# yuhogun0908/MISOnet

Measured on AMD Instinct MI355X. Metric: utterances/sec MISO1->MVDR->MISO3, 6-mic 16kHz 4s, higher is better.
Workload: dtype f32w; 1 GPU; BASELINE configs[3]: synthetic 6-mic 16 kHz 4 s, full MISO1x6 -> align -> MVDRx2 -> MISO3x2; batch_per_gpu=16, global_batch=16, frames=1001, freq_bins=129, parallelism=utterance-shard x1

## Files before the change

include/misonet.h:

```cpp
#ifndef MISONET_H_
#define MISONET_H_

#ifdef __cplusplus
extern "C" {
#endif

typedef struct misonet_net misonet_net;
typedef struct misonet_pipeline misonet_pipeline;
typedef void* misonet_stream;

enum {
  MISONET_OK = 0,
  MISONET_EINVAL = -1,
  MISONET_ESTATE = -2,
  MISONET_EHIP = -3,
  MISONET_ENOMEM = -4,
  MISONET_ENAN = -5
};

typedef struct {
  int in_ch;
  int out_ch;
  int en_ch[7];
  int de_ch[7];
  int n_freq;
  int tcn_norm;
} misonet_cfg;

const char* misonet_strerror(int code);
const char* misonet_last_error(void);
int misonet_version(void);

int misonet_net_create(const misonet_cfg* cfg, misonet_net** out);
int misonet_net_destroy(misonet_net* net);
int misonet_net_num_tensors(const misonet_net* net);
const char* misonet_net_tensor_name(const misonet_net* net, int i);
long long misonet_net_tensor_numel(const misonet_net* net, int i);
int misonet_net_set_tensor(misonet_net* net, const char* key, const float* host_data, long long numel);
int misonet_net_commit(misonet_net* net);

int misonet_net_set_precision(misonet_net* net, int mode);
int misonet_net_get_precision(const misonet_net* net);

long long misonet_net_workspace_bytes(const misonet_net* net, int n_samples, int n_frames);

int misonet_net_forward(misonet_net* net, int n_seg, const void* const* seg_dev, const int* seg_ch,
                        int B, int T, void* out_dev, void* ws_dev, long long ws_bytes, misonet_stream stream);
int misonet_net_check(misonet_net* net, const void* ws_dev, misonet_stream stream);

int misonet_net_keep_activations(misonet_net* net, int keep);
int misonet_net_buffer_plan(const misonet_net* net, int n_frames, int max_buffers, long long* offset_bytes,
                            long long* size_bytes, int* first_step, int* last_step);
int misonet_net_conv_plan(const misonet_net* net, int mode, int max_layers, int* kind);
int misonet_net_tap_shape(const misonet_net* net, const char* name, int* C, int* F);
int misonet_net_tap(misonet_net* net, const char* name, const void* ws_dev, int B, int T, float* dst_dev,
                    misonet_stream stream);

long long misonet_mvdr_workspace_bytes(int B, int F, int M);
int misonet_mvdr(const void* src_dev, const void* mix_dev, int B, int F, int M, int T, float epsi,
                 void* out_dev, void* ws_dev, long long ws_bytes, misonet_stream stream);
int misonet_mvdr_debug(const void* ws_dev, int B, int F, int M, void* steer_c128_dev, void* w_c128_dev,
                       misonet_stream stream);

typedef struct {
  int kind;
  int noise;
  double condition;
  int trace_normalize;
  float epsi;
  int ban;
  int ref_ch;
} misonet_bf_opts;
int misonet_bf_opts_default(misonet_bf_opts* opts);
long long misonet_beamform_workspace_bytes(int B, int F, int M, const misonet_bf_opts* opts);
int misonet_beamform(const void* src_dev, const void* mix_dev, int B, int F, int M, int T, const misonet_bf_opts* opts,
                     void* out_dev, void* ws_dev, long long ws_bytes, misonet_stream stream);
int misonet_beamform_debug(const void* ws_dev, int B, int F, int M, const misonet_bf_opts* opts, void* w_c128_dev,
                           double* lambda_dev, misonet_stream stream);

typedef struct {
  int taps;
  int delay;
  int iterations;
  double diag_load;
  double power_floor;
} misonet_wpe_opts;
int misonet_wpe_opts_default(misonet_wpe_opts* opts);
long long misonet_wpe_workspace_bytes(int B, int M, int T, int F, const misonet_wpe_opts* opts);
int misonet_wpe(const void* mix_dev, const float* power_dev, int B, int M, int T, int F, const misonet_wpe_opts* opts,
                void* out_dev, void* ws_dev, long long ws_bytes, misonet_stream stream);
int misonet_wpe_debug(const void* ws_dev, int B, int M, int F, const misonet_wpe_opts* opts, void* g_c128_dev, int* fail_dev,
                      misonet_stream stream);

typedef struct {
  int taps;
  int delay;
  double diag_load;
  double power_floor;
  int ref_ch;
} misonet_wpd_opts;
int misonet_wpd_opts_default(misonet_wpd_opts* opts);
long long misonet_wpd_workspace_bytes(int B, int F, int M, const misonet_wpd_opts* opts);
int misonet_wpd(const void* src_dev, const void* mix_dev, int B, int F, int M, int T, const misonet_wpd_opts* opts,
                void* out_dev, void* ws_dev, long long ws_bytes, misonet_stream stream);
int misonet_wpd_debug(const void* ws_dev, int B, int F, int M, const misonet_wpd_opts* opts, void* wbar_c128_dev, int* fail_dev,
                      misonet_stream stream);

typedef struct {
  int iterations;
  int prior;
  double diag_load;
  double prior_floor;
} misonet_cacgmm_opts;
int misonet_cacgmm_opts_default(misonet_cacgmm_opts* opts);
long long misonet_cacgmm_workspace_bytes(int B, int K, int F, int M);
int misonet_cacgmm(const void* mix_dev, const float* init_masks_dev, int B, int K, int F, int M, int T,
                   const misonet_cacgmm_opts* opts, float* masks_out_dev, void* images_out_dev, void* ws_dev, long long ws_bytes,
                   misonet_stream stream);
int misonet_cacgmm_debug(const void* ws_dev, int B, int K, int F, int M, void* bk_c128_dev, double* pi_dev, double* ll_dev,
                         int* fail_dev, misonet_stream stream);
int misonet_masks_from_estimates(const void* est_dev, const void* mix_dev, int B, int S, int F, int M, int T,
                                 float* masks_out_dev, misonet_stream stream);

typedef struct {
  int kind;
  int noise;
  int rtf;
  double mu;
  double diag_load;
  int ref_ch;
} misonet_jbf_opts;
int misonet_jbf_opts_default(misonet_jbf_opts* opts);
long long misonet_beamform_joint_workspace_bytes(int B, int S, int F, int M, const misonet_jbf_opts* opts);
int misonet_beamform_joint(const void* src_dev, const void* mix_dev, int B, int S, int F, int M, int T,
                           const misonet_jbf_opts* opts, void* out_dev, void* ws_dev, long long ws_bytes, misonet_stream stream);
int misonet_beamform_joint_debug(const void* ws_dev, int B, int S, int F, int M, const misonet_jbf_opts* opts, void* w_c128_dev,
                                 void* rtf_c128_dev, int* fail_dev, misonet_stream stream);

typedef struct {
  int iterations;
  int model;
  int channels;
  int ref_ch;
  double floor;
} misonet_iva_opts;
int misonet_iva_opts_default(misonet_iva_opts* opts);
long long misonet_auxiva_workspace_bytes(int B, int S, int K, int F, int M, int T);
int misonet_auxiva_resident_frames(int K);
int misonet_auxiva(const void* mix_dev, int B, int S, int F, int M, int T, const misonet_iva_opts* opts, void* images_out_dev,
                   int* order_out_dev, void* ws_dev, long long ws_bytes, misonet_stream stream);
int misonet_auxiva_debug(const void* ws_dev, int B, int K, int F, int M, int T, void* y_c128_dev, void* a_c128_dev,
                         void* evec_c128_dev, double* power_dev, int* fail_dev, misonet_stream stream);

long long misonet_pit_scratch_bytes(int B, int S, int F);
int misonet_pit_select(const void* anchor_dev, const void* cand_dev, int B, int S, int T, int F,
                       int* sel_dev, double* dist_dev, long long dist_bytes, misonet_stream stream);

long long misonet_css_scratch_bytes(int K, int S, int F);
int misonet_css_align(const void* est_dev, int K, int S, int T, int F, int hop_frames, const int* perm0_dev,
                      int* perm_dev, double* dist_dev, long long dist_bytes, misonet_stream stream);
int misonet_css_stitch(const float* y_dev, const int* perm_dev, int K, int S, int W, int hop, int first,
                       long long n_out, short* out_i16_dev, float* out_f32_dev, misonet_stream stream);

long long misonet_score_scratch_bytes(int B, int E, int R, long long n_or_F);
int misonet_score_wave(const void* est_dev, int est_is_i16, long long est_sb, long long est_ss, long long est_st,
                       const float* ref_dev, long long ref_sb, long long ref_ss, long long ref_st, int B, int E, int R,
                       long long n, const int* n_valid_dev, double* stats_dev, void* scratch_dev,
                       long long scratch_bytes, misonet_stream stream);
int misonet_score_spec(const void* est_dev, long long est_sb, long long est_ss, long long est_st, const void* ref_dev,
                       long long ref_sb, long long ref_ss, long long ref_st, int B, int E, int R, int T, int F,
                       double* pair_dev, int* perm_dev, double* upit_dev, void* scratch_dev, long long scratch_bytes,
                       misonet_stream stream);

long long misonet_bss_scratch_bytes(int B, int E, int R, long long n, int Q);
int misonet_bss_corr(const void* est_dev, int est_is_i16, long long est_sb, long long est_ss, long long est_st,
                     const float* ref_dev, long long ref_sb, long long ref_ss, long long ref_st, int B, int E, int R,
                     long long n, const int* n_valid_dev, int Q, double* Rrr_dev, double* Rre_dev, double* Eee_dev,
                     void* scratch_dev, long long scratch_bytes, misonet_stream stream);
int misonet_bss_solve(const double* Rrr_dev, const double* Rre_dev, const double* Eee_dev, int B, int E, int R, int Q,
                      double* T_dev, double* A_dev, int* info_dev, void* scratch_dev, long long scratch_bytes,
                      misonet_stream stream);

long long misonet_stoi_resampled_len(long long n, int fs);
int misonet_stoi_taps(int fs, double* taps_host);
long long misonet_stoi_scratch_bytes(int B, int NS, int R, long long n10);
int misonet_stoi_resample(const void* est_dev, int est_is_i16, long long est_sb, long long est_ss, long long est_st,
                          const float* ref_dev, long long ref_sb, long long ref_ss, long long ref_st, const float* mix_dev,
                          long long mix_sb, long long mix_st, int B, int E, int R, long long n, const int* n_valid_dev, int fs,
                          double* x10_dev, int* len10_dev, misonet_stream stream);
int misonet_stoi_measure(const double* x10_dev, const int* len10_dev, int B, int NS, int R, long long n10, double* out_dev,
                         int* frames_dev, void* scratch_dev, long long scratch_bytes, misonet_stream stream);

int misonet_resample_ratio(int fs_in, int fs_out, int* p, int* q);
long long misonet_resampled_len(long long n, int fs_in, int fs_out);
int misonet_resample_taps(int fs_in, int fs_out, double* out_host, int cap);
int misonet_resample_tile(void);
int misonet_resample(const void* src_dev, int src_kind, long long src_sb, long long src_sc, long long src_st, int B, int M,
                     long long n, const int* n_valid_dev, int fs_in, int fs_out, void* dst_dev, int dst_kind, long long dst_sb,
                     long long dst_sc, long long dst_st, misonet_stream stream);

long long misonet_resample_stream_carry(long long fs_in, long long fs_out);
long long misonet_resample_stream_state_bytes(int B, int M, long long fs_in, long long fs_out);
long long misonet_resample_stream_outputs(long long n_seen, long long n_new, int flush, long long fs_in, long long fs_out);
int misonet_resample_stream_tile(void);
int misonet_resample_stream_reset(void* state_dev, int B, int M, long long fs_in, long long fs_out, misonet_stream stream);
int misonet_resample_stream(const void* src_dev, int src_i16, long long src_sb, long long src_sc, long long src_st, int B, int M,
// ... 147 lines not shown
```

misonet_amd/_lib.py:

```python
from __future__ import annotations

import ctypes as C
import os

_HERE = os.path.dirname(os.path.abspath(__file__))
LIB_PATH = os.environ.get("MISONET_LIB_PATH") or os.path.join(_HERE, "libmisonet_hip.so")

OK, EINVAL, ESTATE, EHIP, ENOMEM, ENAN = 0, -1, -2, -3, -4, -5


class MisonetError(RuntimeError):
    def __init__(self, code, detail):
        super().__init__(f"libmisonet_hip error {code}: {detail}")
        self.code = code


class Cfg(C.Structure):
    _fields_ = [("in_ch", C.c_int), ("out_ch", C.c_int), ("en_ch", C.c_int * 7), ("de_ch", C.c_int * 7),
                ("n_freq", C.c_int), ("tcn_norm", C.c_int)]


class BfOpts(C.Structure):
    _fields_ = [("kind", C.c_int), ("noise", C.c_int), ("condition", C.c_double), ("trace_normalize", C.c_int),
                ("epsi", C.c_float), ("ban", C.c_int), ("ref_ch", C.c_int)]


class WpeOpts(C.Structure):
    _fields_ = [("taps", C.c_int), ("delay", C.c_int), ("iterations", C.c_int), ("diag_load", C.c_double),
                ("power_floor", C.c_double)]


class OwpeOpts(C.Structure):
    _fields_ = [("taps", C.c_int), ("delay", C.c_int), ("context", C.c_int), ("alpha", C.c_double),
                ("power_floor", C.c_double), ("init", C.c_double)]


class OivaOpts(C.Structure):
    _fields_ = [("model", C.c_int), ("ref_ch", C.c_int), ("alpha", C.c_double), ("floor", C.c_double), ("init", C.c_double)]


class ObfOpts(C.Structure):
    _fields_ = [("noise", C.c_int), ("ref_ch", C.c_int), ("alpha", C.c_double), ("mu", C.c_double), ("diag_load", C.c_double),
                ("epsi", C.c_double), ("init", C.c_double)]


class WpdOpts(C.Structure):
    _fields_ = [("taps", C.c_int), ("delay", C.c_int), ("diag_load", C.c_double), ("power_floor", C.c_double),
                ("ref_ch", C.c_int)]


class CacgmmOpts(C.Structure):
    _fields_ = [("iterations", C.c_int), ("prior", C.c_int), ("diag_load", C.c_double), ("prior_floor", C.c_double)]


class JbfOpts(C.Structure):
    _fields_ = [("kind", C.c_int), ("noise", C.c_int), ("rtf", C.c_int), ("mu", C.c_double), ("diag_load", C.c_double),
                ("ref_ch", C.c_int)]


class DoaOpts(C.Structure):
    _fields_ = [("kind", C.c_int), ("num_src", C.c_int), ("block", C.c_int), ("hop", C.c_int), ("f_lo", C.c_int),
                ("f_hi", C.c_int), ("min_sep", C.c_double)]


class IvaOpts(C.Structure):
    _fields_ = [("iterations", C.c_int), ("model", C.c_int), ("channels", C.c_int), ("ref_ch", C.c_int), ("floor", C.c_double)]


SIGNATURES = {
    "misonet_strerror": (C.c_char_p, [C.c_int]),
    "misonet_last_error": (C.c_char_p, []),
    "misonet_version": (C.c_int, []),
    "misonet_net_create": (C.c_int, [C.POINTER(Cfg), C.POINTER(C.c_void_p)]),
    "misonet_net_destroy": (C.c_int, [C.c_void_p]),
    "misonet_net_num_tensors": (C.c_int, [C.c_void_p]),
    "misonet_net_tensor_name": (C.c_char_p, [C.c_void_p, C.c_int]),
    "misonet_net_tensor_numel": (C.c_longlong, [C.c_void_p, C.c_int]),
    "misonet_net_set_tensor": (C.c_int, [C.c_void_p, C.c_char_p, C.c_void_p, C.c_longlong]),
    "misonet_net_commit": (C.c_int, [C.c_void_p]),
    "misonet_net_set_precision": (C.c_int, [C.c_void_p, C.c_int]),
    "misonet_net_get_precision": (C.c_int, [C.c_void_p]),
    "misonet_net_keep_activations": (C.c_int, [C.c_void_p, C.c_int]),
    "misonet_net_buffer_plan": (C.c_int, [C.c_void_p, C.c_int, C.c_int, C.POINTER(C.c_longlong), C.POINTER(C.c_longlong),
                                          C.POINTER(C.c_int), C.POINTER(C.c_int)]),
    "misonet_net_conv_plan": (C.c_int, [C.c_void_p, C.c_int, C.c_int, C.POINTER(C.c_int)]),
    "misonet_net_workspace_bytes": (C.c_longlong, [C.c_void_p, C.c_int, C.c_int]),
    "misonet_net_forward": (C.c_int, [C.c_void_p, C.c_int, C.POINTER(C.c_void_p), C.POINTER(C.c_int), C.c_int, C.c_int,
                                      C.c_void_p, C.c_void_p, C.c_longlong, C.c_void_p]),
    "misonet_net_check": (C.c_int, [C.c_void_p, C.c_void_p, C.c_void_p]),
    "misonet_net_tap_shape": (C.c_int, [C.c_void_p, C.c_char_p, C.POINTER(C.c_int), C.POINTER(C.c_int)]),
    "misonet_net_tap": (C.c_int, [C.c_void_p, C.c_char_p, C.c_void_p, C.c_int, C.c_int, C.c_void_p, C.c_void_p]),
    "misonet_mvdr_workspace_bytes": (C.c_longlong, [C.c_int, C.c_int, C.c_int]),
    "misonet_mvdr": (C.c_int, [C.c_void_p, C.c_void_p, C.c_int, C.c_int, C.c_int, C.c_int, C.c_float, C.c_void_p,
                               C.c_void_p, C.c_longlong, C.c_void_p]),
    "misonet_mvdr_debug": (C.c_int, [C.c_void_p, C.c_int, C.c_int, C.c_int, C.c_void_p, C.c_void_p, C.c_void_p]),
    "misonet_bf_opts_default": (C.c_int, [C.POINTER(BfOpts)]),
    "misonet_beamform_workspace_bytes": (C.c_longlong, [C.c_int, C.c_int, C.c_int, C.POINTER(BfOpts)]),
    "misonet_beamform": (C.c_int, [C.c_void_p, C.c_void_p, C.c_int, C.c_int, C.c_int, C.c_int, C.POINTER(BfOpts), C.c_void_p,
                                   C.c_void_p, C.c_longlong, C.c_void_p]),
    "misonet_beamform_debug": (C.c_int, [C.c_void_p, C.c_int, C.c_int, C.c_int, C.POINTER(BfOpts), C.c_void_p, C.c_void_p,
                                         C.c_void_p]),
    "misonet_pipeline_set_beamformer": (C.c_int, [C.c_void_p, C.POINTER(BfOpts)]),
    "misonet_wpe_opts_default": (C.c_int, [C.POINTER(WpeOpts)]),
    "misonet_wpe_workspace_bytes": (C.c_longlong, [C.c_int, C.c_int, C.c_int, C.c_int, C.POINTER(WpeOpts)]),
    "misonet_wpe": (C.c_int, [C.c_void_p, C.c_void_p, C.c_int, C.c_int, C.c_int, C.c_int, C.POINTER(WpeOpts), C.c_void_p,
                              C.c_void_p, C.c_longlong, C.c_void_p]),
    "misonet_wpe_debug": (C.c_int, [C.c_void_p, C.c_int, C.c_int, C.c_int, C.POINTER(WpeOpts), C.c_void_p, C.c_void_p,
                                    C.c_void_p]),
    "misonet_owpe_opts_default": (C.c_int, [C.POINTER(OwpeOpts)]),
    "misonet_owpe_state_bytes": (C.c_longlong, [C.c_int, C.c_int, C.c_int, C.POINTER(OwpeOpts)]),
    "misonet_owpe_lds_bytes": (C.c_int, [C.c_int, C.POINTER(OwpeOpts)]),
    "misonet_owpe_reset": (C.c_int, [C.c_void_p, C.c_int, C.c_int, C.c_int, C.POINTER(OwpeOpts), C.c_void_p]),
    "misonet_owpe": (C.c_int, [C.c_void_p, C.c_int, C.c_int, C.c_int, C.c_int, C.POINTER(OwpeOpts), C.c_void_p, C.c_void_p,
                               C.c_longlong, C.c_void_p]),
    "misonet_owpe_debug": (C.c_int, [C.c_void_p, C.c_int, C.c_int, C.c_int, C.POINTER(OwpeOpts), C.c_void_p, C.c_void_p,
                                     C.c_void_p, C.c_void_p, C.c_void_p]),
    "misonet_wpd_opts_default": (C.c_int, [C.POINTER(WpdOpts)]),
    "misonet_wpd_workspace_bytes": (C.c_longlong, [C.c_int, C.c_int, C.c_int, C.POINTER(WpdOpts)]),
    "misonet_wpd": (C.c_int, [C.c_void_p, C.c_void_p, C.c_int, C.c_int, C.c_int, C.c_int, C.POINTER(WpdOpts), C.c_void_p,
                              C.c_void_p, C.c_longlong, C.c_void_p]),
    "misonet_wpd_debug": (C.c_int, [C.c_void_p, C.c_int, C.c_int, C.c_int, C.POINTER(WpdOpts), C.c_void_p, C.c_void_p,
                                    C.c_void_p]),
    "misonet_pipeline_set_wpd": (C.c_int, [C.c_void_p, C.POINTER(WpdOpts)]),
    "misonet_cacgmm_opts_default": (C.c_int, [C.POINTER(CacgmmOpts)]),
    "misonet_cacgmm_workspace_bytes": (C.c_longlong, [C.c_int, C.c_int, C.c_int, C.c_int]),
    "misonet_cacgmm": (C.c_int, [C.c_void_p, C.c_void_p, C.c_int, C.c_int, C.c_int, C.c_int, C.c_int, C.POINTER(CacgmmOpts),
                                 C.c_void_p, C.c_void_p, C.c_void_p, C.c_longlong, C.c_void_p]),
    "misonet_cacgmm_debug": (C.c_int, [C.c_void_p, C.c_int, C.c_int, C.c_int, C.c_int, C.c_void_p, C.c_void_p, C.c_void_p,
                                       C.c_void_p, C.c_void_p]),
    "misonet_masks_from_estimates": (C.c_int, [C.c_void_p, C.c_void_p, C.c_int, C.c_int, C.c_int, C.c_int, C.c_int, C.c_void_p,
                                               C.c_void_p]),
    "misonet_pipeline_set_refine": (C.c_int, [C.c_void_p, C.POINTER(CacgmmOpts)]),
    "misonet_jbf_opts_default": (C.c_int, [C.POINTER(JbfOpts)]),
    "misonet_beamform_joint_workspace_bytes": (C.c_longlong, [C.c_int, C.c_int, C.c_int, C.c_int, C.POINTER(JbfOpts)]),
    "misonet_beamform_joint": (C.c_int, [C.c_void_p, C.c_void_p, C.c_int, C.c_int, C.c_int, C.c_int, C.c_int, C.POINTER(JbfOpts),
                                         C.c_void_p, C.c_void_p, C.c_longlong, C.c_void_p]),
    "misonet_beamform_joint_debug": (C.c_int, [C.c_void_p, C.c_int, C.c_int, C.c_int, C.c_int, C.POINTER(JbfOpts), C.c_void_p,
                                               C.c_void_p, C.c_void_p, C.c_void_p]),
    "misonet_pipeline_set_joint": (C.c_int, [C.c_void_p, C.POINTER(JbfOpts)]),
    "misonet_iva_opts_default": (C.c_int, [C.POINTER(IvaOpts)]),
    "misonet_auxiva_workspace_bytes": (C.c_longlong, [C.c_int, C.c_int, C.c_int, C.c_int, C.c_int, C.c_int]),
    "misonet_auxiva_resident_frames": (C.c_int, [C.c_int]),
    "misonet_auxiva": (C.c_int, [C.c_void_p, C.c_int, C.c_int, C.c_int, C.c_int, C.c_int, C.POINTER(IvaOpts), C.c_void_p,
                                 C.c_void_p, C.c_void_p, C.c_longlong, C.c_void_p]),
    "misonet_auxiva_debug": (C.c_int, [C.c_void_p, C.c_int, C.c_int, C.c_int, C.c_int, C.c_int, C.c_void_p, C.c_void_p,
                                       C.c_void_p, C.c_void_p, C.c_void_p, C.c_void_p]),
    "misonet_oiva_opts_default": (C.c_int, [C.POINTER(OivaOpts)]),
    "misonet_oiva_state_bytes": (C.c_longlong, [C.c_int, C.c_int, C.c_int]),
    "misonet_oiva_bins_per_pass": (C.c_int, [C.c_int]),
    "misonet_oiva_reset": (C.c_int, [C.c_void_p, C.c_int, C.c_int, C.c_int, C.POINTER(OivaOpts), C.c_void_p]),
    "misonet_oiva": (C.c_int, [C.c_void_p, C.c_int, C.c_int, C.c_int, C.c_int, C.POINTER(OivaOpts), C.c_void_p, C.c_void_p,
                               C.c_void_p, C.c_longlong, C.c_void_p]),
    "misonet_oiva_debug": (C.c_int, [C.c_void_p, C.c_int, C.c_int, C.c_int, C.c_void_p, C.c_void_p, C.c_void_p, C.c_void_p,
                                     C.c_void_p]),
    "misonet_obf_opts_default": (C.c_int, [C.POINTER(ObfOpts)]),
    "misonet_obf_state_bytes": (C.c_longlong, [C.c_int, C.c_int, C.c_int, C.c_int]),
    "misonet_obf_cells_per_block": (C.c_int, [C.c_int]),
    "misonet_obf_reset": (C.c_int, [C.c_void_p, C.c_int, C.c_int, C.c_int, C.c_int, C.POINTER(ObfOpts), C.c_void_p]),
    "misonet_obf": (C.c_int, [C.c_void_p, C.c_void_p, C.c_int, C.c_int, C.c_int, C.c_int, C.c_int, C.POINTER(ObfOpts), C.c_void_p,
                              C.c_void_p, C.c_longlong, C.c_void_p]),
    "misonet_obf_debug": (C.c_int, [C.c_void_p, C.c_int, C.c_int, C.c_int, C.c_int, C.c_void_p, C.c_void_p, C.c_void_p, C.c_void_p,
                                    C.c_void_p, C.c_void_p]),
    "misonet_pit_scratch_bytes": (C.c_longlong, [C.c_int, C.c_int, C.c_int]),
    "misonet_pit_select": (C.c_int, [C.c_void_p, C.c_void_p, C.c_int, C.c_int, C.c_int, C.c_int, C.c_void_p, C.c_void_p,
                                     C.c_longlong, C.c_void_p]),
    "misonet_css_scratch_bytes": (C.c_longlong, [C.c_int, C.c_int, C.c_int]),
    "misonet_css_align": (C.c_int, [C.c_void_p, C.c_int, C.c_int, C.c_int, C.c_int, C.c_int, C.c_void_p, C.c_void_p,
                                    C.c_void_p, C.c_longlong, C.c_void_p]),
    "misonet_css_stitch": (C.c_int, [C.c_void_p, C.c_void_p, C.c_int, C.c_int, C.c_int, C.c_int, C.c_int, C.c_longlong,
                                     C.c_void_p, C.c_void_p, C.c_void_p]),
    "misonet_score_scratch_bytes": (C.c_longlong, [C.c_int, C.c_int, C.c_int, C.c_longlong]),
    "misonet_score_wave": (C.c_int, [C.c_void_p, C.c_int, C.c_longlong, C.c_longlong, C.c_longlong, C.c_void_p, C.c_longlong,
                                     C.c_longlong, C.c_longlong, C.c_int, C.c_int, C.c_int, C.c_longlong, C.c_void_p,
                                     C.c_void_p, C.c_void_p, C.c_longlong, C.c_void_p]),
    "misonet_score_spec": (C.c_int, [C.c_void_p, C.c_longlong, C.c_longlong, C.c_longlong, C.c_void_p, C.c_longlong,
                                     C.c_longlong, C.c_longlong, C.c_int, C.c_int, C.c_int, C.c_int, C.c_int, C.c_void_p,
                                     C.c_void_p, C.c_void_p, C.c_void_p, C.c_longlong, C.c_void_p]),
    "misonet_bss_scratch_bytes": (C.c_longlong, [C.c_int, C.c_int, C.c_int, C.c_longlong, C.c_int]),
    "misonet_bss_corr": (C.c_int, [C.c_void_p, C.c_int, C.c_longlong, C.c_longlong, C.c_longlong, C.c_void_p, C.c_longlong,
                                   C.c_longlong, C.c_longlong, C.c_int, C.c_int, C.c_int, C.c_longlong, C.c_void_p, C.c_int,
                                   C.c_void_p, C.c_void_p, C.c_void_p, C.c_void_p, C.c_longlong, C.c_void_p]),
    "misonet_bss_solve": (C.c_int, [C.c_void_p, C.c_void_p, C.c_void_p, C.c_int, C.c_int, C.c_int, C.c_int, C.c_void_p,
                                    C.c_void_p, C.c_void_p, C.c_void_p, C.c_longlong, C.c_void_p]),
    "misonet_stoi_resampled_len": (C.c_longlong, [C.c_longlong, C.c_int]),
    "misonet_stoi_taps": (C.c_int, [C.c_int, C.POINTER(C.c_double)]),
    "misonet_stoi_scratch_bytes": (C.c_longlong, [C.c_int, C.c_int, C.c_int, C.c_longlong]),
    "misonet_stoi_resample": (C.c_int, [C.c_void_p, C.c_int, C.c_longlong, C.c_longlong, C.c_longlong, C.c_void_p,
                                        C.c_longlong, C.c_longlong, C.c_longlong, C.c_void_p, C.c_longlong, C.c_longlong,
                                        C.c_int, C.c_int, C.c_int, C.c_longlong, C.c_void_p, C.c_int, C.c_void_p, C.c_void_p,
                                        C.c_void_p]),
    "misonet_stoi_measure": (C.c_int, [C.c_void_p, C.c_void_p, C.c_int, C.c_int, C.c_int, C.c_longlong, C.c_void_p,
                                       C.c_void_p, C.c_void_p, C.c_longlong, C.c_void_p]),
    "misonet_resample_ratio": (C.c_int, [C.c_int, C.c_int, C.POINTER(C.c_int), C.POINTER(C.c_int)]),
    "misonet_resampled_len": (C.c_longlong, [C.c_longlong, C.c_int, C.c_int]),
    "misonet_resample_taps": (C.c_int, [C.c_int, C.c_int, C.POINTER(C.c_double), C.c_int]),
    "misonet_resample_tile": (C.c_int, []),
    "misonet_resample": (C.c_int, [C.c_void_p, C.c_int, C.c_longlong, C.c_longlong, C.c_longlong, C.c_int, C.c_int, C.c_longlong,
                                   C.c_void_p, C.c_int, C.c_int, C.c_void_p, C.c_int, C.c_longlong, C.c_longlong, C.c_longlong,
                                   C.c_void_p]),
    "misonet_resample_stream_carry": (C.c_longlong, [C.c_longlong, C.c_longlong]),
    "misonet_resample_stream_state_bytes": (C.c_longlong, [C.c_int, C.c_int, C.c_longlong, C.c_longlong]),
    "misonet_resample_stream_outputs": (C.c_longlong, [C.c_longlong, C.c_longlong, C.c_int, C.c_longlong, C.c_longlong]),
    "misonet_resample_stream_tile": (C.c_int, []),
    "misonet_resample_stream_reset": (C.c_int, [C.c_void_p, C.c_int, C.c_int, C.c_longlong, C.c_longlong, C.c_void_p]),
    "misonet_resample_stream": (C.c_int, [C.c_void_p, C.c_int, C.c_longlong, C.c_longlong, C.c_longlong, C.c_int, C.c_int,
                                          C.c_longlong, C.c_longlong, C.c_int, C.c_longlong, C.c_longlong, C.c_void_p, C.c_int,
                                          C.c_longlong, C.c_longlong, C.c_longlong, C.c_void_p, C.c_longlong, C.c_void_p]),
    "misonet_room_tile": (C.c_int, []),
    "misonet_room_rir_len": (C.c_longlong, [C.c_int, C.c_int, C.c_int, C.c_int]),
    "misonet_room_mix_len": (C.c_longlong, [C.c_longlong, C.c_int]),
    "misonet_room_rir": (C.c_int, [C.c_void_p, C.c_void_p, C.c_void_p, C.c_void_p, C.c_int, C.c_int, C.c_int, C.c_double,
                                   C.c_double, C.c_int, C.c_int, C.c_void_p, C.c_void_p, C.c_void_p]),
    "misonet_room_mix": (C.c_int, [C.c_void_p, C.c_longlong, C.c_longlong, C.c_longlong, C.c_void_p, C.c_void_p, C.c_int, C.c_int,
                                   C.c_int, C.c_longlong, C.c_int, C.c_longlong, C.c_void_p, C.c_void_p, C.c_void_p, C.c_void_p]),
    "misonet_doa_opts_default": (C.c_int, [C.POINTER(DoaOpts)]),
    "misonet_doa_tile": (C.c_int, []),
    "misonet_doa_bin_chunk": (C.c_int, []),
    "misonet_doa_blocks": (C.c_int, [C.c_int, C.c_int, C.c_int]),
    "misonet_doa_workspace_bytes": (C.c_longlong, [C.c_int, C.c_int, C.c_int, C.c_int, C.c_int, C.c_int, C.POINTER(DoaOpts)]),
    "misonet_doa": (C.c_int, [C.c_void_p, C.c_void_p, C.c_void_p, C.c_int, C.c_void_p, C.c_int, C.c_int, C.c_int, C.c_int,
                              C.c_int, C.c_int, C.c_double, C.POINTER(DoaOpts), C.c_void_p, C.c_void_p, C.c_void_p, C.c_void_p,
                              C.c_void_p, C.c_longlong, C.c_void_p]),
    "misonet_doa_debug": (C.c_int, [C.c_void_p, C.c_int, C.c_int, C.c_int, C.c_int, C.c_int, C.c_int, C.POINTER(DoaOpts),
                                    C.c_void_p, C.c_void_p, C.c_void_p, C.c_void_p]),
    "misonet_reverb_frames": (C.c_longlong, [C.c_longlong, C.c_int]),
    "misonet_reverb_scratch_bytes": (C.c_longlong, [C.c_int, C.c_int, C.c_int, C.c_longlong, C.c_int]),
    "misonet_reverb_measure": (C.c_int, [C.c_void_p, C.c_int, C.c_longlong, C.c_longlong, C.c_longlong, C.c_void_p,
                                         C.c_longlong, C.c_longlong, C.c_longlong, C.c_void_p, C.c_longlong, C.c_longlong,
                                         C.c_int, C.c_int, C.c_int, C.c_longlong, C.c_void_p, C.c_int, C.c_void_p, C.c_void_p,
                                         C.c_void_p, C.c_void_p, C.c_longlong, C.c_void_p]),
    "misonet_srmr_frames": (C.c_longlong, [C.c_longlong, C.c_int]),
    "misonet_srmr_scratch_bytes": (C.c_longlong, [C.c_int, C.c_int, C.c_longlong, C.c_int]),
    "misonet_srmr_chunk": (C.c_int, []),
    "misonet_srmr_measure": (C.c_int, [C.c_void_p, C.c_int, C.c_longlong, C.c_longlong, C.c_longlong, C.c_void_p, C.c_longlong,
                                       C.c_longlong, C.c_int, C.c_int, C.c_longlong, C.c_void_p, C.c_int, C.c_void_p, C.c_void_p,
                                       C.c_void_p, C.c_void_p, C.c_longlong, C.c_void_p]),
    "misonet_pipeline_create": (C.c_int, [C.c_void_p, C.c_void_p, C.c_int, C.c_int, C.c_int, C.c_float,
                                          C.POINTER(C.c_void_p)]),
# ... 62 lines not shown
```

misonet_amd/csrc/conv_select.hpp:

```cpp
#pragma once
#include "kernels.hpp"

#ifdef MISONET_EXPERIMENTS
#define MN_ALT_MODES 1
#else
#define MN_ALT_MODES 0
#endif

namespace mn {

constexpr int CONV_NMODES = 7;
inline bool conv_mode_built(int mode) {
  return mode == 0 || mode == 3 || mode == 5 || (MN_ALT_MODES && mode >= 1 && mode < CONV_NMODES);
}

enum class ConvKind : int {
  DIRECT = 0,
  W1D,
  FEW,
  WINO,
  X6_FIRST,
  X6,
  BF16,
  BF16_DMA,
  WINO6,
};
constexpr int CONV_NKIND = 9;

struct ConvShape {
  int Cin, Cout, Fin, Fout;
  int sf, padf, tr2, act;
  bool transposed;
  int ident_c;
  bool net_input;
  int in_oct, out_oct;
};
inline ConvShape conv_shape(const ConvArgs& a, bool net_input = false) {
  return {a.Cin, a.Cout, a.Fin, a.Fout, a.sf, a.padf, a.tr2, a.act, a.padf == 2, a.ident_c, net_input, a.in_oct, a.out_oct};
}

bool conv_w1d_ok(const ConvShape& s);
bool conv_few_ok(const ConvShape& s);
bool conv_wino_ok(const ConvShape& s);
bool conv_x6_first_ok(const ConvShape& s);
bool conv_wino6_ok(const ConvShape& s);

inline ConvKind conv_select(const ConvShape& s, int mode) {
  const bool planar = mode == 0 || mode == 5 || mode == 6;
  if (s.out_oct == 3 && conv_x6_first_ok(s)) return ConvKind::X6_FIRST;
  if (s.in_oct == 3) return ConvKind::X6;
#if MN_ALT_MODES
  if (s.in_oct) return ConvKind::BF16_DMA;
  if (mode == 1 || mode == 2) return ConvKind::BF16;
  if (mode == 6 && conv_wino6_ok(s)) return ConvKind::WINO6;
#endif
  if (planar && conv_few_ok(s)) return ConvKind::FEW;
  if (mode == 5 && conv_wino_ok(s)) return ConvKind::WINO;
  if (mode == 5 && conv_w1d_ok(s)) return ConvKind::W1D;
  return ConvKind::DIRECT;
}

struct ConvWeights {
  const float* W;
  int Cin, Cout;
  bool transposed;
  int cop, ncg;
};
long long conv_image_floats(ConvKind k, const ConvWeights& c);
void conv_image_pack(ConvKind k, const ConvWeights& c, float* img);
inline long long conv_wino_ww16_at(int Cin, int Cout) { return (long long)((Cout + 31) / 32) * (Cin / 8) * 16 * 8 * 32; }
float conv_f16_wscale(const float* W, long long n);

}
```

misonet_amd/csrc/conv_weights.hip:

```cpp
#include "conv_select.hpp"

#include <math.h>
#include <cmath>
#include <algorithm>
#include <string.h>

namespace mn {

static inline float tap(const ConvWeights& c, int co, int ci, int kt, int kf) {
  return c.transposed ? c.W[(((long long)ci * c.Cout + co) * 3 + (2 - kt)) * 3 + (2 - kf)]
                      : c.W[(((long long)co * c.Cin + ci) * 3 + kt) * 3 + kf];
}
static const double WINO_G[4][3] = {{1, 0, 0}, {0.5, 0.5, 0.5}, {0.5, -0.5, 0.5}, {0, 0, 1}};
static inline double wino_u(const ConvWeights& c, int co, int ci, int xi, int nu) {
  double u = 0.0;
  for (int kt = 0; kt < 3; ++kt)
    for (int kf = 0; kf < 3; ++kf) u += WINO_G[xi][kf] * WINO_G[nu][kt] * (double)tap(c, co, ci, kt, kf);
  return u;
}

static void direct_image(const ConvWeights& c, float* w) {
  const int nchunk = (c.Cin + CK - 1) / CK, COP = c.cop;
  for (int cg = 0; cg < c.ncg; ++cg)
    for (int kc = 0; kc < nchunk; ++kc)
      for (int kt = 0; kt < 3; ++kt)
        for (int kf = 0; kf < 3; ++kf)
          for (int cil = 0; cil < CK; ++cil)
            for (int col = 0; col < COP; ++col) {
              const int ci = kc * CK + cil, co = cg * COP + col;
              w[((((long long)cg * nchunk + kc) * 9 + (kt * 3 + kf)) * CK + cil) * COP + col] =
                  (ci < c.Cin && co < c.Cout) ? tap(c, co, ci, kt, kf) : 0.f;
            }
}

static inline unsigned short f32_to_bf16_rne(float f) {
  unsigned int u;
  memcpy(&u, &f, 4);
  u += 0x7fffu + ((u >> 16) & 1u);
  return (unsigned short)(u >> 16);
}
static inline float bf16_to_f32(unsigned short h) {
  unsigned int u = (unsigned int)h << 16;
  float f;
  memcpy(&f, &u, 4);
  return f;
}

float conv_f16_wscale(const float* W, long long n) {
  float m = 0.f;
  for (long long i = 0; i < n; ++i) m = std::max(m, fabsf(W[i]));
  return (m > 0.f && std::isfinite(m)) ? exp2f(floorf(log2f(64.f / m))) : 1.f;
}

static void bf16_image(const ConvWeights& c, float* dst, bool pieces) {
  const int nchunk = (c.Cin + 15) / 16;
  const int COP = 32;
  const int ncg16 = (c.Cout + 31) / 32;
  unsigned short* w = reinterpret_cast<unsigned short*>(dst);
  const long long img = 9LL * 2 * COP * 8;
  for (int cg = 0; cg < ncg16; ++cg)
    for (int kc = 0; kc < nchunk; ++kc)
      for (int kt = 0; kt < 3; ++kt)
        for (int kf = 0; kf < 3; ++kf)
          for (int h = 0; h < 2; ++h)
            for (int col = 0; col < COP; ++col)
              for (int e = 0; e < 8; ++e) {
                const int ci = kc * 16 + 8 * h + e, co = cg * COP + col;
                const float v = (ci < c.Cin && co < c.Cout) ? tap(c, co, ci, kt, kf) : 0.f;
                const long long idx = ((((long long)(kt * 3 + kf)) * 2 + h) * COP + col) * 8 + e;
                if (pieces) {
                  const unsigned short hi = f32_to_bf16_rne(v);
                  const long long base = ((long long)cg * nchunk + kc) * 2 * img;
                  w[base + idx] = hi;
                  w[base + img + idx] = f32_to_bf16_rne(v - bf16_to_f32(hi));
                } else {
                  dst[((long long)cg * nchunk + kc) * img + idx] = v;
                }
              }
}

static void wf6_image(const ConvWeights& c, float* wf) {
  const int nchunk = (c.Cin + 7) / 8;
  const int ncg = (c.Cout + 31) / 32;
  for (int cg = 0; cg < ncg; ++cg)
    for (int kc = 0; kc < nchunk; ++kc)
      for (int kt = 0; kt < 3; ++kt)
        for (int kf = 0; kf < 3; ++kf)
          for (int col = 0; col < 32; ++col)
            for (int e = 0; e < 8; ++e) {
              const int ci = kc * 8 + e, co = cg * 32 + col;
              wf[((((long long)cg * nchunk + kc) * 9 + (kt * 3 + kf)) * 32 + col) * 8 + e] =
                  (ci < c.Cin && co < c.Cout) ? tap(c, co, ci, kt, kf) : 0.f;
            }
}

static void w6s_image(const ConvWeights& c, float* dst) {
  const int nchunk = (c.Cin + 7) / 8;
  unsigned short* img = reinterpret_cast<unsigned short*>(dst);
  for (int kc = 0; kc < nchunk; ++kc)
    for (int kt = 0; kt < 3; ++kt)
      for (int kf = 0; kf < 3; ++kf)
        for (int co = 0; co < 32; ++co)
          for (int e = 0; e < 8; ++e) {
            const int ci = kc * 8 + e;
            const float v = (ci < c.Cin && co < c.Cout) ? tap(c, co, ci, kt, kf) : 0.f;
            const unsigned short h = f32_to_bf16_rne(v);
            const float r1 = v - bf16_to_f32(h);
            const unsigned short m = f32_to_bf16_rne(r1);
            const unsigned short l = f32_to_bf16_rne(r1 - bf16_to_f32(m));
            const unsigned short part[3] = {h, m, l};
            for (int p = 0; p < 3; ++p) {
              const long long unit = kt < 2 ? ((kf * 3 + p) * 2 + kt) * 32 + co : 576 + (kf * 3 + p) * 32 + co;
              img[((long long)kc * 864 + unit) * 8 + e] = part[p];
            }
          }
}

static void few_image(const ConvWeights& c, float* img) {
  for (int ci = 0; ci < c.Cin; ++ci)
    for (int kt = 0; kt < 3; ++kt)
      for (int kf = 0; kf < 3; ++kf)
        for (int co = 0; co < 4; ++co) img[((long long)ci * 9 + (kt * 3 + kf)) * 4 + co] = co < c.Cout ? tap(c, co, ci, kt, kf) : 0.f;
}

static void w1d_image(const ConvWeights& c, float* img) {
  const int nchunk = (c.Cin + CK - 1) / CK, ncg = (c.Cout + 31) / 32;
  for (int cg = 0; cg < ncg; ++cg)
    for (int kc = 0; kc < nchunk; ++kc)
      for (int nu = 0; nu < 4; ++nu)
        for (int kf = 0; kf < 3; ++kf)
          for (int cil = 0; cil < CK; ++cil)
            for (int col = 0; col < 32; ++col) {
              const int ci = kc * CK + cil, co = cg * 32 + col;
              double u = 0.0;
              if (ci < c.Cin && co < c.Cout)
                for (int kt = 0; kt < 3; ++kt) u += WINO_G[nu][kt] * (double)tap(c, co, ci, kt, kf);
              img[((((long long)cg * nchunk + kc) * 12 + (nu * 3 + kf)) * CK + cil) * 32 + col] = (float)u;
            }
}

static inline bool wino_minus(int xi, int nu) { return (nu == 2) != ((nu == 3) != (xi == 3)); }
static void wino_image(const ConvWeights& c, float* img) {
  const int nchunk = c.Cin / 8, ncg = (c.Cout + 31) / 32;
  for (int cg = 0; cg < ncg; ++cg)
    for (int kc = 0; kc < nchunk; ++kc)
      for (int cil = 0; cil < 8; ++cil)
        for (int col = 0; col < 32; ++col) {
          const int ci = kc * 8 + cil, co = cg * 32 + col;
          for (int pos = 0; pos < 16; ++pos) {
            const int xi = pos >> 2, nu = pos & 3;
            const double u = co < c.Cout ? wino_u(c, co, ci, xi, nu) : 0.0;
            img[(((((long long)cg * nchunk + kc) * 4 + (pos >> 2)) * 8 + cil) * 32 + col) * 4 + (pos & 3)] = (float)(wino_minus(xi, nu) ? -u : u);
          }
        }
}
static void wino_image16(const ConvWeights& c, int co0, float* img) {
  const int nchunk = c.Cin / 8;
  for (int kc = 0; kc < nchunk; ++kc)
    for (int cil = 0; cil < 8; ++cil)
      for (int col = 0; col < 16; ++col) {
        const int ci = kc * 8 + cil, co = co0 + col;
        for (int pos = 0; pos < 16; ++pos) {
          const int xi = pos >> 2, nu = pos & 3;
          const double u = wino_u(c, co, ci, xi, nu);
          const int s = cil >> 2, kk = cil & 3;
          img[((((((long long)kc * 2 + s) * 4 + (pos >> 2)) * 4 + kk) * 16 + col) * 4) + (pos & 3)] = (float)(wino_minus(xi, nu) ? -u : u);
        }
      }
}

static void wino6_image(const ConvWeights& c, float* dst) {
  const int nk = (c.Cin + 15) / 16, ncg = (c.Cout + 31) / 32;
  unsigned short* img = reinterpret_cast<unsigned short*>(dst);
  auto top16 = [](float x) { unsigned u; memcpy(&u, &x, 4); return (unsigned short)(u >> 16); };
  for (int cg = 0; cg < ncg; ++cg)
    for (int kk = 0; kk < nk; ++kk)
      for (int pos = 0; pos < 16; ++pos)
        for (int col = 0; col < 32; ++col)
          for (int cil = 0; cil < 16; ++cil) {
            const int ci = kk * 16 + cil, co = cg * 32 + col, xi = pos >> 2, nu = pos & 3;
            const float v = (float)((co < c.Cout && ci < c.Cin) ? wino_u(c, co, ci, xi, nu) : 0.0);
            unsigned vb; memcpy(&vb, &v, 4);
            unsigned hb = vb & 0xffff0000u, wb = vb & 0xffffff00u;
            float h, w; memcpy(&h, &hb, 4); memcpy(&w, &wb, 4);
            const float m = w - h, l = v - w;
            const int lane = col + 32 * (cil >> 3), j = cil & 7;
            const long long q = (((long long)cg * nk + kk) * 4 + xi) * (3 * 4 * 64 * 8);
            img[q + ((long long)(nu * 3 + 0) * 64 + lane) * 8 + j] = top16(h);
            img[q + ((long long)(nu * 3 + 1) * 64 + lane) * 8 + j] = top16(m);
            img[q + ((long long)(nu * 3 + 2) * 64 + lane) * 8 + j] = top16(l);
          }
}

long long conv_image_floats(ConvKind k, const ConvWeights& c) {
  const long long g32 = (c.Cout + 31) / 32, k8 = (c.Cin + 7) / 8, k16 = (c.Cin + 15) / 16;
  switch (k) {
    case ConvKind::DIRECT: return (long long)c.ncg * ((c.Cin + CK - 1) / CK) * 9 * CK * c.cop;
    case ConvKind::W1D: return g32 * ((c.Cin + CK - 1) / CK) * 12 * CK * 32;
    case ConvKind::FEW: return (long long)c.Cin * 36;
    case ConvKind::WINO: return conv_wino_ww16_at(c.Cin, c.Cout) + ((c.Cout & 31) == 16 ? (long long)(c.Cin / 8) * 2048 : 0);
    case ConvKind::X6_FIRST: return k8 * 864 * 4;
    case ConvKind::X6: return g32 * k8 * 9 * 32 * 8;
    case ConvKind::BF16: return g32 * k16 * 2 * 9 * 2 * 32 * 8 / 2;
    case ConvKind::BF16_DMA: return g32 * k16 * 9 * 2 * 32 * 8;
    case ConvKind::WINO6: return g32 * k16 * (16 * 3 * 64 * 16 / 4);
  }
  return 0;
}

void conv_image_pack(ConvKind k, const ConvWeights& c, float* img) {
  switch (k) {
    case ConvKind::DIRECT: direct_image(c, img); break;
    case ConvKind::W1D: w1d_image(c, img); break;
    case ConvKind::FEW: few_image(c, img); break;
    case ConvKind::WINO:
      wino_image(c, img);
      if ((c.Cout & 31) == 16) wino_image16(c, c.Cout - 16, img + conv_wino_ww16_at(c.Cin, c.Cout));
      break;
    case ConvKind::X6_FIRST: w6s_image(c, img); break;
    case ConvKind::X6: wf6_image(c, img); break;
#if MN_ALT_MODES
    case ConvKind::BF16: bf16_image(c, img, true); break;
    case ConvKind::BF16_DMA: bf16_image(c, img, false); break;
    case ConvKind::WINO6: wino6_image(c, img); break;
#else
    default: break;
#endif
  }
}

}
```

misonet_amd/csrc/conv_wino.hip:

```cpp
#include "conv_select.hpp"
#include "conv_epilogue.hpp"
#include "wino_regs.hpp"
#include <stdio.h>
#include <stdlib.h>
#include <utility>

namespace mn {

typedef float wf16 __attribute__((ext_vector_type(16)));
typedef float wf4 __attribute__((ext_vector_type(4)));
typedef float wf2 __attribute__((ext_vector_type(2)));
typedef unsigned int wu2 __attribute__((ext_vector_type(2)));
#define MN_WLDS(p) ((__attribute__((address_space(3))) void*)(p))

constexpr int WCK = 8;
constexpr int WTT = 64;
constexpr int WFT = 8;
constexpr int WNR = 10;
constexpr int WTW = 66;
constexpr int WIN_FLOATS = WCK * WNR * WTW;
constexpr int WW_FLOATS = 16 * WCK * 32;
constexpr int WSTAGE_FLOATS = WIN_FLOATS + WW_FLOATS;
constexpr int WNSTAGE = 3;
constexpr int WNRM_MAX = 192;
constexpr int WCO_MAX = 64;

template <int P, bool Z = false>
__device__ __forceinline__ void wino_mfma(float uu, float vv) {
  if (Z) asm volatile("v_mfma_f32_32x32x2_f32 a[%0:%1], %2, %3, 0" ::"n"(16 * P), "n"(16 * P + 15), "v"(uu), "v"(vv) : W_ACLOB);
  else asm volatile("v_mfma_f32_32x32x2_f32 a[%0:%1], %2, %3, a[%0:%1]" ::"n"(16 * P), "n"(16 * P + 15), "v"(uu), "v"(vv) : W_ACLOB);
}
template <int B, bool Z = false>
__device__ __forceinline__ void wino_mfma16(float uu, float vv) {
  if (Z) asm volatile("v_mfma_f32_16x16x4_f32 a[%0:%1], %2, %3, 0" ::"n"(4 * B), "n"(4 * B + 3), "v"(uu), "v"(vv) : W_ACLOB);
  else asm volatile("v_mfma_f32_16x16x4_f32 a[%0:%1], %2, %3, a[%0:%1]" ::"n"(4 * B), "n"(4 * B + 3), "v"(uu), "v"(vv) : W_ACLOB);
}
__device__ __forceinline__ wf2 pk_add(wf2 a, wf2 b) { wf2 d; asm volatile("v_pk_add_f32 %0, %1, %2" : "=v"(d) : "v"(a), "v"(b)); return d; }
__device__ __forceinline__ wf2 pk_sub(wf2 a, wf2 b) { wf2 d; asm volatile("v_pk_add_f32 %0, %1, %2 neg_lo:[0,1] neg_hi:[0,1]" : "=v"(d) : "v"(a), "v"(b)); return d; }
__device__ __forceinline__ wf2 pk_t01(wf2 a, wf2 b) { wf2 d; asm volatile("v_pk_add_f32 %0, %1, %2 op_sel:[0,0] op_sel_hi:[1,0] neg_lo:[0,1] neg_hi:[0,0]" : "=v"(d) : "v"(a), "v"(b)); return d; }
__device__ __forceinline__ wf2 pk_t23(wf2 a, wf2 b) { wf2 d; asm volatile("v_pk_add_f32 %0, %1, %2 op_sel:[1,0] op_sel_hi:[1,1] neg_lo:[0,1] neg_hi:[0,1]" : "=v"(d) : "v"(a), "v"(b)); return d; }
__device__ __forceinline__ wf2 pk_spm(wf2 a) { wf2 d; asm volatile("v_pk_add_f32 %0, %1, %1 op_sel:[0,1] op_sel_hi:[0,1] neg_lo:[0,0] neg_hi:[0,1]" : "=v"(d) : "v"(a)); return d; }
__device__ __forceinline__ wf2 pk_add_nh(wf2 a, wf2 b) { wf2 d; asm volatile("v_pk_add_f32 %0, %1, %2 neg_lo:[0,0] neg_hi:[0,1]" : "=v"(d) : "v"(a), "v"(b)); return d; }
__device__ __forceinline__ wf2 pk_mul(wf2 a, wf2 b) { wf2 d; asm volatile("v_pk_mul_f32 %0, %1, %2" : "=v"(d) : "v"(a), "v"(b)); return d; }
__device__ __forceinline__ wf2 pk_fma(wf2 a, wf2 b, wf2 c) { wf2 d; asm volatile("v_pk_fma_f32 %0, %1, %2, %3" : "=v"(d) : "v"(a), "v"(b), "v"(c)); return d; }
__device__ __forceinline__ float exp2_ws(float x) {
  float r;
  asm volatile("v_exp_f32 %0, %1\n\ts_nop 0" : "=v"(r) : "v"(x));
  return r;
}
__device__ __forceinline__ float elu_pick(float y, float neg, float pos) {
  return __builtin_bit_cast(int, y) < 0 ? neg : pos;
}
template <int OFF>
__device__ __forceinline__ void lds_write_f32(unsigned addr, float v) {
  asm volatile("ds_write_b32 %0, %1 offset:%2" ::"v"(addr), "v"(v), "n"(OFF) : "memory");
}
__device__ __forceinline__ wf2 pk_nrm(wf2 x, wf2 nr) { wf2 d; asm volatile("v_pk_fma_f32 %0, %1, %2, %2 op_sel:[0,0,1] op_sel_hi:[1,0,1]" : "=v"(d) : "v"(x), "v"(nr)); return d; }
constexpr int WRAW_FLOATS = WCK * WNR * WTT + 256;
constexpr unsigned WRAW_B = (unsigned)(WNSTAGE * WSTAGE_FLOATS) * 4u;
constexpr unsigned WNRM_B = WRAW_B + 2u * WRAW_FLOATS * 4u;
constexpr unsigned WZERO_B = WNRM_B + 2u * WNRM_MAX * 8u;
constexpr unsigned WRED_B = WZERO_B + WNRM_MAX * 8u;
constexpr unsigned WDUMMY_B = WRED_B + 4u * 64u * 4u;
constexpr unsigned WBIAS_B = WDUMMY_B + 64u * 4u;
constexpr size_t WINO_LDS = WBIAS_B + WCO_MAX * 24;
static_assert(WINO_LDS <= 160 * 1024, "one workgroup per CU: at most 160 KB of LDS");

template <int DBG, bool G16 = false>
__global__ __launch_bounds__(256, 1) void conv3x3_wino_f32(const ConvArgs a) {
  extern __shared__ __align__(16) float smem[];
  char* const smem_c = reinterpret_cast<char*>(smem);
  wf2* s_nrm = reinterpret_cast<wf2*>(smem_c + WNRM_B);
  wf2* s_zero = reinterpret_cast<wf2*>(smem_c + WZERO_B);

  const int tid = threadIdx.x;
  const int lane = tid & 63;
  const int wave = __builtin_amdgcn_readfirstlane(tid >> 6);
  const int half = lane >> 5, l31 = lane & 31;
  const int kk = lane >> 4, nn = lane & 15;
  const int T = a.T, Tp = a.Tp, F = a.Fin, Cin = a.Cin;
  const int nchunk = Cin / WCK;
  constexpr unsigned WIMG_B = G16 ? 2u * 4u * 4u * 16u * 16u : (unsigned)(WW_FLOATS * 4);

  const unsigned tps = (unsigned)(a.ntx * a.nty * a.ncg);
  unsigned q0, qstep, Q, xcd_id = 0;
  if (a.xcd) {
    xcd_id = blockIdx.x & 7u;
    q0 = blockIdx.x >> 3;
    qstep = gridDim.x >> 3;
    Q = (unsigned)(a.nsamp >> 3) * tps;
  } else {
    q0 = blockIdx.x;
    qstep = gridDim.x;
    Q = (unsigned)a.nsamp * tps;
  }
  if (q0 >= Q) return;
  const unsigned ntile = (Q - q0 + qstep - 1) / qstep;
  for (int i = tid; i < WNRM_MAX; i += 256) s_zero[i] = wf2{0.f, 0.f};
  if (tid < WCO_MAX) {
    const float b = tid < a.ncg * 32 ? a.bias[tid] : 0.f;
    const float c = elu_fast(b);
    wf2* tb = reinterpret_cast<wf2*>(smem_c + WBIAS_B + tid * 24);
    tb[0] = wf2{b, b}; tb[1] = wf2{-c, -c}; tb[2] = wf2{-1.f - c, -1.f - c};
  }

  const unsigned row_e = (unsigned)Tp;
  const unsigned plane_b = (unsigned)F * row_e * 4u;

  const int sq = tid & 15, scr = tid >> 4;
  int sch[5];
#pragma unroll
  for (int i = 0; i < 5; ++i) sch[i] = (scr + 16 * i) / WNR;
  const bool hrole = tid < 2 * WCK * WNR;
  const int hit = hrole ? tid >> 1 : 0, hside = tid & 1;
  const int hch = hit / WNR, hrow = hit - hch * WNR;
  const unsigned lds0 = (unsigned)(unsigned long long)MN_WLDS(smem);
  constexpr unsigned STAGE_B = (unsigned)WSTAGE_FLOATS * 4u, STEP_B = (unsigned)((G16 ? 4 : 2) * WNR * WTW) * 4u;
  const unsigned dbase = G16 ? lds0 + (unsigned)((kk * WNR + 2 * wave) * WTW + 2 * nn) * 4u
                             : lds0 + (unsigned)((half * WNR + 2 * wave) * WTW + 2 * l31) * 4u;
  unsigned d1 = launder(dbase + STEP_B), d2 = launder(dbase + 2 * STEP_B), d3 = launder(dbase + 3 * STEP_B);
  unsigned d0n = launder(dbase + STAGE_B);
  unsigned uc = launder(lds0 + (unsigned)WIN_FLOATS * 4u + (unsigned)(G16 ? kk * 16 + nn : half * 32 + l31) * 16u);
  unsigned un = launder(uc + STAGE_B);
  unsigned cn = launder(lds0 + STAGE_B + (unsigned)(scr * WTW + 1 + 4 * sq) * 4u);
  unsigned hn = launder(lds0 + (hrole ? STAGE_B + (unsigned)(hit * WTW + (hside ? WTT + 1 : 0)) * 4u : WDUMMY_B + (unsigned)(tid & 63) * 4u));
#define W_LP(TYPE, ADDR) (reinterpret_cast<__attribute__((address_space(3))) TYPE*>(ADDR))
  const unsigned rofs0 = lds0 + WRAW_B + (unsigned)(scr * WTT + 4 * sq) * 4u;
  const unsigned rhofs0 = lds0 + WRAW_B + (unsigned)(WCK * WNR * WTT + tid) * 4u;
  const unsigned rdma0 = WRAW_B + (unsigned)wave * 1024u;
  const unsigned rhdma0 = WRAW_B + (unsigned)(WCK * WNR * WTT) * 4u + (unsigned)wave * 256u;
  const unsigned wdma0 = (unsigned)(WIN_FLOATS * 4) + (unsigned)wave * 1024u;
  const __amdgpu_buffer_rsrc_t rs_w = make_rsrc_e(reinterpret_cast<unsigned long long>(a.ww),
                                                   (unsigned)(a.ncg * nchunk) * WIMG_B);
  unsigned wvo[4];
#pragma unroll
  for (int j = 0; j < 4; ++j) wvo[j] = (unsigned)(tid + 256 * (G16 ? (j & 1) : j)) * 16u;

  unsigned ql = q0;
  int kl = 0;
  int Ln = -1, Lpar = 1, Lcg = 0;
  int lslot = 0;
  unsigned Lgoff[5], Lhoff = 0;
  unsigned Lnr[6];
  bool Lfull = false;
  unsigned Lmask = 0;
  __amdgpu_buffer_rsrc_t rs_l;
  unsigned Cnr[6];
  bool Cfull = false;
  unsigned Cmask = 0;
  unsigned Dwso = 0;
  int cslot = 0;
#pragma unroll
  for (int i = 0; i < 6; ++i) { Lnr[i] = lds0 + WZERO_B; Cnr[i] = lds0 + WZERO_B; }

#define W_DECODE(Q, TT_, FT_, N_, CG_)                                                                \
  {                                                                                                   \
    const unsigned q_ = __builtin_amdgcn_readfirstlane(Q);                                            \
    const unsigned j_ = q_ / tps;                                                                     \
    unsigned r_ = q_ - j_ * tps;                                                                      \
    N_ = (int)(a.xcd ? j_ * 8u + xcd_id : j_);                                                        \
    CG_ = (int)(r_ % (unsigned)a.ncg);                                                                \
    r_ /= (unsigned)a.ncg;                                                                            \
    TT_ = (int)(r_ % (unsigned)a.ntx);                                                                \
    FT_ = (int)(r_ / (unsigned)a.ntx);                                                                \
  }

#define W_LOAD_SETUP(Q)                                                                               \
  {                                                                                                   \
    int tt_, ft_, n_, cg_;                                                                            \
    W_DECODE(Q, tt_, ft_, n_, cg_)                                                                    \
    const int t0_ = tt_ * WTT, fin0_ = ft_ * WFT - 1;                                                 \
    if (n_ != Ln) {                             \
      Ln = n_;                                                                                        \
      Lpar ^= 1;                                                                                      \
      for (int c = tid; c < Cin; c += 256) {                                                          \
        float mean = 0.f, rstd = 1.f;                                                                 \
        if (c >= a.ident_c) {                                                                         \
          const dstat_t* st_ = a.in_stats + ((long long)n_ * a.in_sstride + a.in_c0 + c) * (2 * DS_NL); \
          const double cnt = (double)F * (double)T;                                                   \
          const double m = dstat_read(st_) / cnt;                                                     \
          double var = dstat_read(st_ + DS_NL) / cnt - m * m;                                         \
          var = var > 0.0 ? var : 0.0;                                                                \
          mean = (float)m;                                                                            \
          rstd = (float)(1.0 / sqrt(var + (double)IN_EPS));                                           \
        }                                                                                             \
        s_nrm[Lpar * WNRM_MAX + c] = wf2{rstd, -mean * rstd};                                         \
      }                                                                                               \
      const float* in_n_ = a.in + (long long)n_ * a.in_bstride + (long long)a.in_c0 * F * Tp;         \
      rs_l = make_rsrc_e(reinterpret_cast<unsigned long long>(in_n_), (unsigned)Cin * plane_b);       \
    }                                                                                                 \
    Lcg = cg_;                                                                                        \
    const int tg_ = t0_ + 4 * sq;                                                                     \
    const int tge_ = tg_ + 4 <= Tp ? tg_ : Tp - 4;                                                    \
    Lfull = t0_ + WTT <= T;                                                                           \
    Lmask = (tg_ < T ? 1u : 0u) | (tg_ + 1 < T ? 2u : 0u) | (tg_ + 2 < T ? 4u : 0u) | (tg_ + 3 < T ? 8u : 0u); \
    _Pragma("unroll") for (int i = 0; i < 5; ++i) {                                                   \
      int fin = fin0_ + (scr + 16 * i) - sch[i] * WNR;                                                \
      Lnr[i] = lds0 + ((fin >= 0 && fin < F) ? WNRM_B + (unsigned)(Lpar * WNRM_MAX + sch[i]) * 8u : WZERO_B); \
      fin = fin < 0 ? 0 : (fin >= F ? F - 1 : fin);                                                   \
      Lgoff[i] = (unsigned)sch[i] * plane_b + (unsigned)((fin * (int)row_e + tge_) * 4);              \
    }                                                                                                 \
    {                                                                                                 \
      const int htg_ = hside ? t0_ + WTT : t0_ - 1;                                                   \
      int fin = fin0_ + hrow;                                                                         \
      const bool hok_ = hrole && fin >= 0 && fin < F && htg_ >= 0 && htg_ < T;                        \
      Lnr[5] = lds0 + (hok_ ? WNRM_B + (unsigned)(Lpar * WNRM_MAX + hch) * 8u : WZERO_B);             \
      fin = fin < 0 ? 0 : (fin >= F ? F - 1 : fin);                                                   \
      const int th_ = (htg_ < 0 || htg_ >= T) ? 0 : htg_;    \
      Lhoff = (unsigned)hch * plane_b + (unsigned)((fin * (int)row_e + th_) * 4);                     \
    }                                                                                                 \
  }

#define W_LATCH                                                                                       \
  {                                                                                                   \
    Dwso = (unsigned)(Lcg * nchunk + kl) * WIMG_B;                                                    \
  }
#define W_ADVANCE                                                                                     \
  {                                                                                                   \
    lslot ^= 1;                                                                                       \
    if (++kl == nchunk) {                                                                             \
      if (ql + qstep < Q) { kl = 0; ql += qstep; W_LOAD_SETUP(ql) }                                             \
      else kl = nchunk - 1;                     \
    }                                                                                                 \
  }

  wf4 rwa, rwb;
  float rh = 0.f;
  wf2 nra, nrb;
  wf2 cva[2], cvb[2];
  float chv = 0.f;
  unsigned rofs = rofs0, rhofs = rhofs0;

#define W_CB ((unsigned)kl * (unsigned)WCK * plane_b)
#define W_ISSUE_I(I)                                                                                  \
  __builtin_amdgcn_raw_ptr_buffer_load_lds(rs_l, MN_WLDS(smem_c + rdma0 + lslot * (WRAW_FLOATS * 4) + (I) * 4096), 16, Lgoff[I], W_CB, 0, 0);
#define W_ISSUE_H                                                                                     \
  __builtin_amdgcn_raw_ptr_buffer_load_lds(rs_l, MN_WLDS(smem_c + rhdma0 + lslot * (WRAW_FLOATS * 4)), 4, Lhoff, W_CB, 0, 0);
#define W_ISSUE_W(J, ST, WSO)                                                                         \
  __builtin_amdgcn_raw_ptr_buffer_load_lds(rs_w, MN_WLDS(smem_c + (ST) * (WSTAGE_FLOATS * 4) + wdma0 + (G16 ? ((J) & 1) : (J)) * 4096), 16, wvo[J], WSO, 0, 0);
#define W_WSO_L ((unsigned)(Lcg * nchunk + kl) * WIMG_B)
#define W_VMCNT(N) asm volatile("s_waitcnt vmcnt(" #N ")" ::: "memory");
#define W_NR(DST, I) DST = *W_LP(const wf2, Cnr[I]);
#define W_RR(DST, I) DST = *W_LP(const wf4, rofs + (I) * 4096);
#define W_RRH rh = *W_LP(const float, rhofs);
#define W_CC(CV, RW, NR)                                                                              \
  {                                                                                                   \
    CV[0] = pk_nrm(wf2{RW.x, RW.y}, NR);                                                              \
    CV[1] = pk_nrm(wf2{RW.z, RW.w}, NR);                                                              \
    if (RAG) {                                                                                        \
      CV[0].x = (Cmask & 1u) ? CV[0].x : 0.f; CV[0].y = (Cmask & 2u) ? CV[0].y : 0.f;                 \
      CV[1].x = (Cmask & 4u) ? CV[1].x : 0.f; CV[1].y = (Cmask & 8u) ? CV[1].y : 0.f;                 \
    }                                                                                                 \
  }
#define W_CCH(NR) chv = fmaf(rh, NR.x, NR.y);
#define W_DSW(ADDR, VAL, OFF) asm volatile("ds_write_b32 %0, %1 offset:%2" ::"v"(ADDR), "v"(VAL), "n"(OFF) : "memory");
#define W_CW(CV, I)                                                                                   \
  {                                                                                                   \
    W_DSW(cn, CV[0].x, (I) * (16 * WTW * 4))                                                          \
    W_DSW(cn, CV[0].y, (I) * (16 * WTW * 4) + 4)                                                      \
    W_DSW(cn, CV[1].x, (I) * (16 * WTW * 4) + 8)                                                      \
    W_DSW(cn, CV[1].y, (I) * (16 * WTW * 4) + 12)                                                     \
  }
#define W_CWH W_DSW(hn, chv, 0)
#define W_BARRIER { asm volatile("s_waitcnt lgkmcnt(0)" ::: "memory"); __builtin_amdgcn_s_barrier(); asm volatile("" ::: "memory"); }

  wf2 dd16[2][4][2];
  wf2 vp16[2][4][2];
  wf2 dd[4][2];
  wf4 u[4];
  wf2 vp[4][2];
#define W_FD(I0, DREG)                                                                                \
  {                                                                                                   \
    const unsigned si_ = DREG;                                                                        \
    dd[I0][0] = *W_LP(const wf2, si_ + (I0) * (WTW * 4));                                             \
    dd[I0][1] = *W_LP(const wf2, si_ + (I0) * (WTW * 4) + 8);                                         \
    dd[I0 + 1][0] = *W_LP(const wf2, si_ + ((I0) + 1) * (WTW * 4));                                   \
    dd[I0 + 1][1] = *W_LP(const wf2, si_ + ((I0) + 1) * (WTW * 4) + 8);                               \
  }
#define W_FU(Q, UREG, S) u[Q] = *W_LP(const wf4, UREG + ((S) * 64 + (Q) * 256) * 16);
#define W_TRANSFORM                                                                                   \
  if (!(DBG & 4)) {                                                                                   \
    const wf2 c0a = pk_sub(dd[0][0], dd[2][0]), c0b = pk_sub(dd[0][1], dd[2][1]);                     \
    const wf2 c1a = pk_add(dd[1][0], dd[2][0]), c1b = pk_add(dd[1][1], dd[2][1]);                     \
    const wf2 c2a = pk_sub(dd[2][0], dd[1][0]), c2b = pk_sub(dd[2][1], dd[1][1]);                     \
    const wf2 c3a = pk_sub(dd[1][0], dd[3][0]), c3b = pk_sub(dd[1][1], dd[3][1]);                     \
    vp[0][0] = pk_t01(c0a, c0b); vp[0][1] = pk_t23(c0a, c0b);                                         \
    vp[1][0] = pk_t01(c1a, c1b); vp[1][1] = pk_t23(c1a, c1b);                                         \
    vp[2][0] = pk_t01(c2a, c2b); vp[2][1] = pk_t23(c2a, c2b);                                         \
    vp[3][0] = pk_t01(c3a, c3b); vp[3][1] = pk_t23(c3a, c3b);                                         \
  }

#define W_SB __builtin_amdgcn_sched_barrier(0);
#ifdef MISONET_EXPERIMENTS
  unsigned long long* const tl_buf = (blockIdx.x == 8 && wave == 1) ? a.dbg_buf : nullptr;
  int tl_n = 0;
#define W_STAMP(ID) if (tl_buf && tl_n < 250) { if (lane == 0) { tl_buf[2 * tl_n] = (ID); tl_buf[2 * tl_n + 1] = __builtin_readcyclecounter(); } ++tl_n; }
#else
#define W_STAMP(ID)
#endif
#define W_MF(P, CS) wino_mfma<P, (POST == 2 && (CS) == 0)>(u[(P) >> 2][(P) & 3], vp[(P) >> 2][((P) & 3) >> 1][(P) & 1]);
#define W_NONE
#define W_X(...) if (!(DBG & (1 | 32))) { __VA_ARGS__ }
#define W_XL(...) if (!(DBG & (1 | 16))) { __VA_ARGS__ }
#define W_XW(...) if (!(DBG & (1 | 8))) { __VA_ARGS__ }
#define W_STEP(CS, FD_, FU_, FS, X1, X2, X3, XB, X4, X5, X6, X7, X8, X9, X10, X11, X13, X14, XG)      \
  W_MF(0, CS) W_FU(3, uc, CS) W_SB                                                                    \
  W_MF(1, CS) X1 W_SB                                                                                 \
  W_MF(2, CS) X2 W_SB                                                                                 \
  W_MF(3, CS) X3 W_SB                                                                                 \
  XB                                                                                                  \
  W_MF(4, CS) W_FU(0, FU_, FS) X4 W_SB                                                                \
  W_MF(5, CS) W_FD(0, FD_) X5 W_SB                                                                    \
  W_MF(6, CS) W_FD(2, FD_) X6 W_SB                                                                    \
  W_MF(7, CS) X7 W_SB                                                                                 \
  W_MF(8, CS) W_FU(1, FU_, FS) X8 W_SB                                                                \
  W_MF(9, CS) X9 W_SB                                                                                 \
  W_MF(10, CS) X10 W_SB                                                                               \
  W_MF(11, CS) X11 W_SB                                                                               \
  W_MF(12, CS) W_FU(2, FU_, FS) W_SB                                                                  \
  W_MF(13, CS) X13 W_SB                                                                               \
  W_MF(14, CS) X14 W_SB                                                                               \
  W_MF(15, CS) W_SB                                                                                   \
  W_TRANSFORM XG W_SB

  constexpr int W_NDMA_W = 4, W_NDMA_I = 6, W_NSTORE = 16;
  static_assert(W_NDMA_W * 256 * 16 == WW_FLOATS * 4, "U image = 4 pieces of 256 threads x 16 bytes");
  static_assert(5 * 256 * 16 == WCK * WNR * WTT * 4 && 2 * WCK * WNR <= 256, "raw input = 5 pieces of 256 x 16 bytes + one 4-byte halo piece");
  static_assert(W_NDMA_W + W_NDMA_I == 10 && W_NDMA_I == 6 && 10 + W_NSTORE == 26 && 6 + W_NSTORE == 22,
                "the s_waitcnt vmcnt immediates of W_CHUNK_ (10 / 26 in step 0, 6 / 22 in front of the barrier)");
#define W_BK_S1  \
  const bool nxt0_ = (kc + 2 == nchunk);                                                              \
  Cfull = nxt0_ ? Lfull : Cfull;                                                                      \
  Dwso = (unsigned)(Lcg * nchunk + kl) * WIMG_B;
#define W_BK_S2  \
  lslot ^= 1; ++kl;
#define W_BK_S3                                                \
  const unsigned dl_n_ = (ph3 == 1) ? 0u - 2u * STAGE_B : STAGE_B;       \
  ph3 = ph3 == 2 ? 0 : ph3 + 1;                                                                       \
  post = post > 0 ? post - 1 : 0;                                                                     \
  cslot ^= 1;                                                                                         \
  stnn = ph3 == 0 ? 2 : ph3 - 1;                            \
  const unsigned rsl_ = cslot ? (unsigned)(WRAW_FLOATS * 4) : 0u;
#define W_BK_V                                                                                        \
  if (__builtin_expect(nxt0_, 0)) {                                                                   \
    _Pragma("unroll") for (int i = 0; i < 6; ++i) Cnr[i] = Lnr[i];                                    \
    Cmask = Lmask;                                                                                    \
  } else {                                                                                            \
    _Pragma("unroll") for (int i = 0; i < 6; ++i) Cnr[i] += (unsigned)(WCK * 8);                      \
  }                                                                                                   \
  d1 = d0n + STEP_B; d2 = d0n + 2 * STEP_B; d3 = d0n + 3 * STEP_B;                                    \
  uc = un;                                                                                            \
  d0n += dl_n_; un += dl_n_; cn += dl_n_;                                                             \
  hn += hrole ? dl_n_ : 0u;                                                                           \
  rofs = rofs0 + rsl_; rhofs = rhofs0 + rsl_;
#define W_CHUNK_                                                                                      \
  W_STEP(0, d1, uc, 1, W_NONE, W_NONE, W_NONE, W_NONE, W_NONE, W_NONE, W_NONE,                        \
         W_X(W_STAMP(1) if (POST) { W_VMCNT(26) } else { W_VMCNT(10) } W_STAMP(2) W_RR(rwa, 0)), W_NONE, W_X(W_RR(rwb, 1)), W_X(W_NR(nra, 0)), W_X(W_NR(nrb, 1)), W_NONE, W_NONE, \
         W_X(W_CC(cva, rwa, nra) W_CC(cvb, rwb, nrb)))                                                \
  W_STEP(1, d2, uc, 2, W_X(W_CW(cva, 0)), W_X(W_CW(cvb, 1)), W_NONE, W_NONE, W_NONE, W_NONE, W_NONE,  \
         W_X(W_RR(rwa, 2)), W_NONE, W_X(W_RR(rwb, 3)), W_X(W_NR(nra, 2)), W_X(W_NR(nrb, 3)), W_NONE, W_NONE,  \
         W_X(W_CC(cva, rwa, nra) W_CC(cvb, rwb, nrb)))                                                \
  W_STEP(2, d3, uc, 3, W_X(W_CW(cva, 2)), W_X(W_CW(cvb, 3)), W_NONE, W_NONE, W_NONE, W_NONE, W_NONE,  \
         W_X(W_RR(rwa, 4)), W_NONE, W_X(W_RRH), W_X(W_NR(nra, 4)), W_X(W_NR(nrb, 5)), W_NONE, W_NONE, \
         W_X(W_CC(cva, rwa, nra) W_CCH(nrb)))                                                         \
  W_STEP(3, d0n, un, 0, W_X(W_CW(cva, 4)), W_X(W_CWH), W_NONE,                                        \
         W_STAMP(3) W_XW(if (POST == 2) { W_VMCNT(22) } else { W_VMCNT(6) }) W_STAMP(4) W_BARRIER W_STAMP(5), \
         W_XW(W_ISSUE_W(0, stnn, Dwso)), W_XW(W_ISSUE_W(1, stnn, Dwso)), W_XW(W_ISSUE_W(2, stnn, Dwso)), W_XW(W_ISSUE_W(3, stnn, Dwso)), \
         W_XL(W_ISSUE_I(0)), W_XL(W_ISSUE_I(1)), W_XL(W_ISSUE_I(2)), W_XL(W_ISSUE_I(3)), W_XL(W_ISSUE_I(4)),  \
         W_XL(W_ISSUE_H) W_BK_S1 W_BK_S2 W_BK_S3, W_BK_V)

#define W_FD16(G, I0, DREG)                                                                           \
  {                                                                                                   \
    const unsigned si_ = (DREG) + (G) * 128u;                                                         \
    dd16[G][I0][0] = *W_LP(const wf2, si_ + (I0) * (WTW * 4));                                        \
    dd16[G][I0][1] = *W_LP(const wf2, si_ + (I0) * (WTW * 4) + 8);                                    \
    dd16[G][I0 + 1][0] = *W_LP(const wf2, si_ + ((I0) + 1) * (WTW * 4));                              \
    dd16[G][I0 + 1][1] = *W_LP(const wf2, si_ + ((I0) + 1) * (WTW * 4) + 8);                          \
  }
#define W_FU16(Q, UREG, S) u[Q] = *W_LP(const wf4, UREG + ((S) * 4 + (Q)) * 1024);
#define W_TRANSFORM16(G)                                                                              \
  {                                                                                                   \
    const wf2 c0a = pk_sub(dd16[G][0][0], dd16[G][2][0]), c0b = pk_sub(dd16[G][0][1], dd16[G][2][1]); \
    const wf2 c1a = pk_add(dd16[G][1][0], dd16[G][2][0]), c1b = pk_add(dd16[G][1][1], dd16[G][2][1]); \
    const wf2 c2a = pk_sub(dd16[G][2][0], dd16[G][1][0]), c2b = pk_sub(dd16[G][2][1], dd16[G][1][1]); \
    const wf2 c3a = pk_sub(dd16[G][1][0], dd16[G][3][0]), c3b = pk_sub(dd16[G][1][1], dd16[G][3][1]); \
    vp16[G][0][0] = pk_t01(c0a, c0b); vp16[G][0][1] = pk_t23(c0a, c0b);                               \
    vp16[G][1][0] = pk_t01(c1a, c1b); vp16[G][1][1] = pk_t23(c1a, c1b);                               \
    vp16[G][2][0] = pk_t01(c2a, c2b); vp16[G][2][1] = pk_t23(c2a, c2b);                               \
    vp16[G][3][0] = pk_t01(c3a, c3b); vp16[G][3][1] = pk_t23(c3a, c3b);                               \
  }
#define W_MF16(I, CS) wino_mfma16<(I), (POST == 2 && (CS) == 0)>(u[(I) >> 3][((I) >> 1) & 3], vp16[(I) & 1][(I) >> 3][(((I) >> 1) & 3) >> 1][((I) >> 1) & 1]);
#define W_S16(I, CS, ...) W_MF16(I, CS) __VA_ARGS__ W_SB
#define W_CHUNK16_                                                                                    \
    \
  W_S16(0, 0, W_FU16(3, uc, 0))                                                                       \
  W_S16(1, 0, W_X(if (POST) { W_VMCNT(26) } else { W_VMCNT(10) } W_RR(rwa, 0)))                       \
  W_S16(2, 0, W_X(W_RR(rwb, 1)))                                                                      \
  W_S16(3, 0, W_X(W_NR(nra, 0)))                                                                      \
  W_S16(4, 0, W_X(W_NR(nrb, 1)))                                                                      \
  W_S16(5, 0) W_S16(6, 0)                                                                             \
  W_S16(7, 0, W_X(W_CC(cva, rwa, nra) W_CC(cvb, rwb, nrb)))                                           \
  W_S16(8, 0, W_FU16(0, uc, 1) W_X(W_CW(cva, 0)))                                                     \
  W_S16(9, 0, W_X(W_CW(cvb, 1)))                                                                      \
  W_S16(10, 0, W_FD16(0, 0, d1) W_X(W_RR(rwa, 2)))                                                    \
  W_S16(11, 0, W_FD16(0, 2, d1) W_X(W_RR(rwb, 3)))                                                    \
  W_S16(12, 0, W_FD16(1, 0, d1) W_X(W_NR(nra, 2)))                                                    \
  W_S16(13, 0, W_FD16(1, 2, d1) W_X(W_NR(nrb, 3)))                                                    \
  W_S16(14, 0) W_S16(15, 0)                                                                           \
  W_S16(16, 0, W_FU16(1, uc, 1))                                                                      \
  W_S16(17, 0) W_S16(18, 0)                                                                           \
  W_S16(19, 0, W_X(W_CC(cva, rwa, nra) W_CC(cvb, rwb, nrb)))                                          \
  W_S16(20, 0, W_X(W_CW(cva, 2)))                                                                     \
  W_S16(21, 0, W_X(W_CW(cvb, 3)))                                                                     \
  W_S16(22, 0, W_X(W_RR(rwa, 4)))                                                                     \
  W_S16(23, 0, W_X(W_RRH))                                                                            \
  W_S16(24, 0, W_FU16(2, uc, 1) W_X(W_NR(nra, 4)))                                                    \
  W_S16(25, 0, W_X(W_NR(nrb, 5)))                                                                     \
  W_S16(26, 0) W_S16(27, 0) W_S16(28, 0) W_S16(29, 0) W_S16(30, 0) W_S16(31, 0)                       \
  W_TRANSFORM16(0) W_TRANSFORM16(1) W_X(W_CC(cva, rwa, nra) W_CCH(nrb)) W_SB                          \
   \
  W_S16(0, 1, W_FU16(3, uc, 1) W_X(W_CW(cva, 4)))                                                     \
  W_S16(1, 1, W_X(W_CWH))                                                                             \
  W_S16(2, 1) W_S16(3, 1)                                                                             \
  W_XW(if (POST == 2) { W_VMCNT(22) } else { W_VMCNT(6) }) W_BARRIER                                  \
  W_S16(4, 1, W_XW(W_ISSUE_W(0, stnn, Dwso)))                                                         \
  W_S16(5, 1, W_XW(W_ISSUE_W(1, stnn, Dwso)))                                                         \
  W_S16(6, 1, W_XW(W_ISSUE_W(2, stnn, Dwso)))                                                         \
  W_S16(7, 1, W_XW(W_ISSUE_W(3, stnn, Dwso)))                                                         \
  W_S16(8, 1, W_FU16(0, un, 0) W_XL(W_ISSUE_I(0)))                                                    \
  W_S16(9, 1, W_XL(W_ISSUE_I(1)))                                                                     \
  W_S16(10, 1, W_FD16(0, 0, d0n) W_XL(W_ISSUE_I(2)))                                                  \
  W_S16(11, 1, W_FD16(0, 2, d0n) W_XL(W_ISSUE_I(3)))                                                  \
  W_S16(12, 1, W_FD16(1, 0, d0n) W_XL(W_ISSUE_I(4)))                                                  \
  W_S16(13, 1, W_FD16(1, 2, d0n) W_XL(W_ISSUE_H))                                                     \
  W_S16(14, 1) W_S16(15, 1)                                                                           \
  W_S16(16, 1, W_FU16(1, un, 0))                                                                      \
  W_S16(17, 1) W_S16(18, 1) W_S16(19, 1) W_S16(20, 1) W_S16(21, 1) W_S16(22, 1) W_S16(23, 1)          \
  W_S16(24, 1, W_FU16(2, un, 0))                                                                      \
  W_S16(25, 1) W_S16(26, 1) W_S16(27, 1) W_S16(28, 1) W_S16(29, 1)                                    \
  W_S16(30, 1, W_BK_S1 W_BK_S2 W_BK_S3)                                                               \
  W_S16(31, 1)                                                                                        \
  W_TRANSFORM16(0) W_TRANSFORM16(1) W_BK_V W_SB
#define W_BODY_ if constexpr (G16) { W_CHUNK16_ } else { W_CHUNK_ }

  constexpr bool RAG = true;
  W_LOAD_SETUP(ql)
#pragma unroll
  for (int i = 0; i < 6; ++i) Cnr[i] = Lnr[i];
  Cmask = Lmask; Cfull = Lfull;
  __syncthreads();
  W_ISSUE_W(0, 0, W_WSO_L) W_ISSUE_W(1, 0, W_WSO_L) W_ISSUE_W(2, 0, W_WSO_L) W_ISSUE_W(3, 0, W_WSO_L)
  W_ISSUE_I(0) W_ISSUE_I(1) W_ISSUE_I(2) W_ISSUE_I(3) W_ISSUE_I(4) W_ISSUE_H
  W_LATCH
  W_ADVANCE
  W_ISSUE_W(0, 1, W_WSO_L) W_ISSUE_W(1, 1, W_WSO_L) W_ISSUE_W(2, 1, W_WSO_L) W_ISSUE_W(3, 1, W_WSO_L)
  W_ISSUE_I(0) W_ISSUE_I(1) W_ISSUE_I(2) W_ISSUE_I(3) W_ISSUE_I(4) W_ISSUE_H
  W_LATCH
  W_ADVANCE
  W_VMCNT(0)
  cn -= STAGE_B;
  if (hrole) hn -= STAGE_B;
  W_RR(rwa, 0) W_NR(nra, 0) W_CC(cva, rwa, nra) W_CW(cva, 0)
  W_RR(rwa, 1) W_NR(nra, 1) W_CC(cva, rwa, nra) W_CW(cva, 1)
  W_RR(rwa, 2) W_NR(nra, 2) W_CC(cva, rwa, nra) W_CW(cva, 2)
  W_RR(rwa, 3) W_NR(nra, 3) W_CC(cva, rwa, nra) W_CW(cva, 3)
  W_RR(rwa, 4) W_NR(nra, 4) W_CC(cva, rwa, nra) W_CW(cva, 4)
  W_RRH W_NR(nrb, 5) W_CCH(nrb) W_CWH
#pragma unroll
  for (int i = 0; i < 6; ++i) Cnr[i] += (unsigned)(WCK * 8);
  cn += STAGE_B;
  if (hrole) hn += STAGE_B;
  asm volatile("s_waitcnt lgkmcnt(0)" ::: "memory");
  W_ISSUE_I(0) W_ISSUE_I(1) W_ISSUE_I(2) W_ISSUE_I(3) W_ISSUE_I(4) W_ISSUE_H
  W_LATCH
  W_ADVANCE
  cslot = 1;
  rofs = rofs0 + WRAW_FLOATS * 4;
  rhofs = rhofs0 + WRAW_FLOATS * 4;
  W_BARRIER
  if constexpr (G16) {
    W_FD16(0, 0, dbase) W_FD16(0, 2, dbase) W_FD16(1, 0, dbase) W_FD16(1, 2, dbase) W_FU16(0, uc, 0) W_FU16(1, uc, 0) W_FU16(2, uc, 0)
    W_TRANSFORM16(0) W_TRANSFORM16(1)
  } else {
    W_FD(0, dbase) W_FD(2, dbase) W_FU(0, uc, 0) W_FU(1, uc, 0) W_FU(2, uc, 0)
    W_TRANSFORM
  }
  wfor<256>([&](auto i) __attribute__((always_inline)) { agpr_zero<decltype(i)::value>(); });
  asm volatile("s_nop 4");

  unsigned qc = q0;
  int kc = 0;
  int ph3 = 0;
  int post = 0;
  const unsigned G = ntile * (unsigned)nchunk;
  int stnn = 2;
  for (unsigned g = 0; g < G; ++g) {
    if (Cfull) {
      constexpr bool RAG = false;
      if (post == 0) { constexpr int POST = 0; W_BODY_ } else if (post == 1) { constexpr int POST = 1; W_BODY_ } else { constexpr int POST = 2; W_BODY_ }
    } else {
      constexpr bool RAG = true;
      if (post == 0) { constexpr int POST = 0; W_BODY_ } else if (post == 1) { constexpr int POST = 1; W_BODY_ } else { constexpr int POST = 2; W_BODY_ }
    }
    if (++kc == nchunk) {
      asm volatile("s_nop 15\n\ts_nop 7");
      W_STAMP(10)
      if (!(DBG & 2)) {
      int tt_, ft_, n, cg;
      W_DECODE(qc, tt_, ft_, n, cg)
      const int t0 = tt_ * WTT, f0 = ft_ * WFT;
      const int cbase = cg * 32;
      const int fa = f0 + 2 * wave;
      const bool r0ok = fa < F, r1ok = fa + 1 < F;
      const unsigned P4 = (unsigned)F * (unsigned)Tp * 4u;
      const float* ob_ = a.out + (long long)n * a.out_bstride + (long long)a.out_c0 * F * Tp;
      const __amdgpu_buffer_rsrc_t rs_out = make_rsrc_e(reinterpret_cast<unsigned long long>(ob_), (unsigned)a.Cout * P4);
      const unsigned red_a = lds0 + WRED_B;
      wf2 l2e = {1.44269504088896341f, 1.44269504088896341f};
      asm volatile("" : "+v"(l2e));
      auto epi_item = [&](auto getm, unsigned tabp, unsigned voff, bool evl, const wf2& mt, const wf2& mb, float& o1, float& o2) __attribute__((always_inline)) {
        const wf2 bb = *W_LP(const wf2, tabp);
        wf2 E[4];
        wfor<4>([&](auto xc) __attribute__((always_inline)) {
          constexpr int x = decltype(xc)::value;
          const float m0 = getm(xc, std::integral_constant<int, 0>{}), m1 = getm(xc, std::integral_constant<int, 1>{});
          const float m2 = getm(xc, std::integral_constant<int, 2>{}), m3 = getm(xc, std::integral_constant<int, 3>{});
          E[x] = wf2{m1 + m2, m1 - m2} + wf2{m0, m3};
        });
        wf2 yt = (E[0] + E[1]) + (E[2] + bb);
        wf2 yb = (E[1] - E[2]) + (bb + E[3]);
        if (!(DBG & 256)) {
          const wf2 ncr = *W_LP(const wf2, tabp + 8), nc1 = *W_LP(const wf2, tabp + 16);
          const wf2 xt = yt * l2e, xb = yb * l2e;
          const wf2 et = wf2{__builtin_amdgcn_exp2f(xt.x), __builtin_amdgcn_exp2f(xt.y)} + nc1;
          const wf2 eb = wf2{__builtin_amdgcn_exp2f(xb.x), __builtin_amdgcn_exp2f(xb.y)} + nc1;
          const wf2 at = yt + ncr, ab = yb + ncr;
          yt = wf2{elu_pick(yt.x, et.x, at.x), elu_pick(yt.y, et.y, at.y)};
          yb = wf2{elu_pick(yb.x, eb.x, ab.x), elu_pick(yb.y, eb.y, ab.y)};
        }
        if (!(DBG & 64)) {
          const float n00 = dpp_get<0xB1>(yt.x), n01 = dpp_get<0xB1>(yt.y), n10 = dpp_get<0xB1>(yb.x), n11 = dpp_get<0xB1>(yb.y);
          const wf4 o = {evl ? yt.x : n10, evl ? yt.y : n11, evl ? n00 : yb.x, evl ? n01 : yb.y};
          __builtin_amdgcn_raw_buffer_store_b128(__builtin_bit_cast(u32x4_t, o), rs_out, (DBG & 512) ? 0x80000000u : voff, 0, 2);
        }
        const wf2 zt = yt * mt, zb = yb * mb;
        const wf2 zs = zt + zb, zq = __builtin_elementwise_fma(zb, zb, zt * zt);
        o1 = zs.x + zs.y;
        o2 = zq.x + zq.y;
      };
      auto dummy_store = [&]() __attribute__((always_inline)) {
        if (!(DBG & 64)) __builtin_amdgcn_raw_buffer_store_b128(u32x4_t{0u, 0u, 0u, 0u}, rs_out, 0x80000000u, 0, 2);
      };
      if constexpr (G16) {
        const bool ev = (nn & 1) == 0;
        const unsigned tab16 = launder(lds0 + WBIAS_B + (unsigned)(cbase + 4 * kk) * 24u);
        float s1g[8], s2g[8];
        wfor<2>([&](auto gc) __attribute__((always_inline)) {
          constexpr int g = decltype(gc)::value;
          const int t = t0 + 2 * (nn + 16 * g);
          const bool c0ok = t < T, c1ok = t + 1 < T;
          const unsigned vbase = (unsigned)(fa * Tp + t) * 4u + (unsigned)(cbase + 4 * kk) * P4;
          const unsigned vo_x = ev ? ((r0ok && c0ok) ? vbase : 0x80000000u)
                                   : ((r1ok && t - 2 < T) ? vbase + (unsigned)Tp * 4u - 8u : 0x80000000u);
          wf2 mt = {(r0ok && c0ok) ? 1.f : 0.f, (r0ok && c1ok) ? 1.f : 0.f}, mb = {(r1ok && c0ok) ? 1.f : 0.f, (r1ok && c1ok) ? 1.f : 0.f};
          asm volatile("" : "+v"(mt), "+v"(mb));
          wfor<4>([&](auto rc) __attribute__((always_inline)) {
            constexpr int r = decltype(rc)::value;
            epi_item([&](auto xc, auto nc) __attribute__((always_inline)) { return agpr_get<((4 * decltype(xc)::value + decltype(nc)::value) * 2 + g) * 4 + r>(); },
                     tab16 + r * 24, vo_x + (unsigned)r * P4, ev, mt, mb, s1g[4 * g + r], s2g[4 * g + r]);
          });
        });
        wfor<8>([&](auto) __attribute__((always_inline)) { dummy_store(); });
        W_STAMP(11)
        if (!(DBG & 128)) {
          wfor<4>([&](auto rc) __attribute__((always_inline)) {
            constexpr int r = decltype(rc)::value;
            float x1 = s1g[r] + s1g[4 + r], x2 = s2g[r] + s2g[4 + r];
            x1 += dpp_get<0xB1>(x1); x2 += dpp_get<0xB1>(x2);
            x1 += dpp_get<0x4E>(x1); x2 += dpp_get<0x4E>(x2);
            x1 += dpp_get<0x141>(x1); x2 += dpp_get<0x141>(x2);
            x1 += dpp_get<0x140>(x1); x2 += dpp_get<0x140>(x2);
            if (nn == 0) {
              const unsigned ra_ = red_a + (unsigned)((wave * 32 + 4 * kk + r) * 2) * 4u;
              lds_write_f32<0>(ra_, x1);
              lds_write_f32<4>(ra_, x2);
            }
          });
        }
      } else {
      const int t = t0 + 2 * l31;
      const bool c0ok = t < T, c1ok = t + 1 < T;
      const unsigned vbase = (unsigned)(fa * Tp + t) * 4u + (unsigned)(4 * half) * P4;
      const bool ev = (l31 & 1) == 0;
      const unsigned vo_x = ev ? ((r0ok && c0ok) ? vbase : 0x80000000u)
                               : ((r1ok && t - 2 < T) ? vbase + (unsigned)Tp * 4u - 8u : 0x80000000u);
      const unsigned tab_a = launder(lds0 + WBIAS_B + (unsigned)(cbase + 4 * half) * 24u);
      wf2 mt = {(r0ok && c0ok) ? 1.f : 0.f, (r0ok && c1ok) ? 1.f : 0.f}, mb = {(r1ok && c0ok) ? 1.f : 0.f, (r1ok && c1ok) ? 1.f : 0.f};
      asm volatile("" : "+v"(mt), "+v"(mb));
      float s1[16], s2[16];
      const int nquad = (a.Cout - cbase + 7) >> 3;
      wfor<4>([&](auto qc_) __attribute__((always_inline)) {
        constexpr int qd = decltype(qc_)::value;
        if (__builtin_expect(qd >= nquad, 0)) {
          wfor<4>([&](auto r4) __attribute__((always_inline)) {
            constexpr int r = 4 * qd + decltype(r4)::value;
            dummy_store();
            s1[r] = 0.f; s2[r] = 0.f;
          });
          return;
        }
        wfor<4>([&](auto r4) __attribute__((always_inline)) {
          constexpr int r = 4 * qd + decltype(r4)::value;
          constexpr int kr = (r & 3) + 8 * (r >> 2);
          epi_item([&](auto xc, auto nc) __attribute__((always_inline)) { return agpr_get<(4 * decltype(xc)::value + decltype(nc)::value) * 16 + r>(); },
                   tab_a + kr * 24, vo_x + (unsigned)(cbase + kr) * P4, ev, mt, mb, s1[r], s2[r]);
        });
      });
      W_STAMP(11)
      if (!(DBG & 128)) {
        const float x1 = reduce16_halfwave(s1, lane);
        const float x2 = reduce16_halfwave(s2, lane);
        if ((lane & 16) == 0) {
          const int q = lane & 15;
          const int co_l = (q & 3) + 8 * (q >> 2) + 4 * half;
          W_DSW(red_a + (unsigned)((wave * 32 + co_l) * 2) * 4u, x1, 0)
          W_DSW(red_a + (unsigned)((wave * 32 + co_l) * 2) * 4u, x2, 4)
        }
      }
      }
      if (!(DBG & 128)) {
        W_BARRIER
        if (lane < 16) {
          const int pr = wave * 16 + lane;
          const int co_l = pr >> 1, which = pr & 1;
          const int co = cbase + co_l;
          if (co < a.Cout) {
            float tot = 0.f;
            for (int w = 0; w < 4; ++w)
              if (f0 + 2 * w < F) tot += *W_LP(const float, red_a + (unsigned)((w * 32 + co_l) * 2 + which) * 4u);
            dstat_add(a.out_stats + (((long long)n * a.out_sstride + a.out_c0 + co) * 2 + which) * DS_NL, (double)tot);
          }
        }
      }
      }
      W_STAMP(12)
      if (DBG & (2 | 64)) {
        wfor<256>([&](auto i) __attribute__((always_inline)) { agpr_zero<decltype(i)::value>(); });
        asm volatile("s_nop 4");
      }
      W_STAMP(13)
      kc = 0;
      qc += qstep;
      post = (DBG & (2 | 64)) ? 0 : 2;
    }
    if (kl == nchunk) {
      if (ql + qstep < Q) { kl = 0; ql += qstep; W_LOAD_SETUP(ql) }
      else kl = nchunk - 1;
    }
  }
}

bool conv_wino_ok(const ConvShape& s) {
  return s.act && s.Cin >= 3 * WCK && s.Cout <= WCO_MAX && s.sf == 1 && s.padf == 1 && !s.tr2 && s.Fin == s.Fout && (s.Cin % WCK) == 0 && s.Cin <= WNRM_MAX && !s.in_oct &&
         !s.out_oct;
}

#ifdef MISONET_EXPERIMENTS
static int wino_dbg_env() {
  static const int v = exp_env("MISONET_WINO_DBG", 0);
  return v;
}
#endif

hipError_t conv_wino_init() {
  hipError_t e = hipFuncSetAttribute(reinterpret_cast<const void*>(&conv3x3_wino_f32<0>), hipFuncAttributeMaxDynamicSharedMemorySize,
                                     (int)WINO_LDS);
  if (e == hipSuccess)
    e = hipFuncSetAttribute(reinterpret_cast<const void*>(&conv3x3_wino_f32<0, true>), hipFuncAttributeMaxDynamicSharedMemorySize, (int)WINO_LDS);
#ifdef MISONET_EXPERIMENTS
#define W_ATTR(D) if (e == hipSuccess) e = hipFuncSetAttribute(reinterpret_cast<const void*>(&conv3x3_wino_f32<D>), hipFuncAttributeMaxDynamicSharedMemorySize, (int)WINO_LDS);
  W_ATTR(1) W_ATTR(2) W_ATTR(3) W_ATTR(4) W_ATTR(7) W_ATTR(10) W_ATTR(18) W_ATTR(34) W_ATTR(64) W_ATTR(128) W_ATTR(256) W_ATTR(448) W_ATTR(512)
#undef W_ATTR
#endif
  return e;
}

static hipError_t launch_wino_groups(ConvArgs a, int n_samples, hipStream_t s, bool g16);

hipError_t launch_conv_wino(const ConvArgs& a_in, int n_samples, hipStream_t s) {
  if (!conv_wino_ok(conv_shape(a_in)) || !a_in.ww) return hipErrorInvalidValue;
  if ((a_in.Cout & 31) == 16 && a_in.ww16 != nullptr) {
    const int c32 = a_in.Cout - 16;
    if (c32 > 0) {
      ConvArgs a = a_in;
      a.Cout = c32;
      const hipError_t e = launch_wino_groups(a, n_samples, s, false);
      if (e != hipSuccess) return e;
    }
    ConvArgs b = a_in;
    b.Cout = 16;
    b.out_c0 = a_in.out_c0 + c32;
    b.bias = a_in.bias + c32;
    b.ww = a_in.ww16;
    return launch_wino_groups(b, n_samples, s, true);
  }
  return launch_wino_groups(a_in, n_samples, s, false);
}

static hipError_t launch_wino_groups(ConvArgs a, int n_samples, hipStream_t s, bool g16) {
  a.cop = 32;
  a.ncg = g16 ? 1 : (a.Cout + 31) / 32;
  const int cus = device_cus();
  if (cus <= 0) return hipErrorInvalidDevice;
  (void)conv_grid(a, n_samples, WTT, WFT, (n_samples % 8 == 0 && cus % 8 == 0) ? conv_xcd_env() : 0);
  const long long tiles = (long long)n_samples * a.ntx * a.nty * a.ncg;
  const unsigned grid = (unsigned)(tiles < cus ? tiles : cus);
  const dim3 g(a.xcd ? (unsigned)cus : grid);
  if (g16) {
    hipLaunchKernelGGL((conv3x3_wino_f32<0, true>), g, dim3(256), WINO_LDS, s, a);
    return hipGetLastError();
  }
#ifdef MISONET_EXPERIMENTS
  {
    static const int tl_cin = exp_env("MISONET_WINO_TIMELINE", 0);
    static unsigned long long* tl_dev = nullptr;
    static int tl_done = 0;
    if (tl_cin && a.Cin == tl_cin && a.Fin == 63 && n_samples == 96 && tl_done < 2) {
      if (!tl_dev) (void)hipMalloc(reinterpret_cast<void**>(&tl_dev), 512 * 8);
      (void)hipMemsetAsync(tl_dev, 0, 512 * 8, s);
      a.dbg_buf = tl_dev;
      hipLaunchKernelGGL(conv3x3_wino_f32<0>, g, dim3(256), WINO_LDS, s, a);
      (void)hipStreamSynchronize(s);
      unsigned long long h[512];
      (void)hipMemcpy(h, tl_dev, sizeof(h), hipMemcpyDeviceToHost);
      if (++tl_done == 2) {
        fprintf(stderr, "[wino timeline] Cin=%d nchunk=%d: id, cycles since previous stamp\n", a.Cin, a.Cin / 8);
        for (int i = 0; i < 250 && h[2 * i]; ++i)
          fprintf(stderr, "  %2llu %8lld\n", h[2 * i], i ? (long long)(h[2 * i + 1] - h[2 * i - 1]) : 0ll);
      }
      return hipGetLastError();
    }
  }
  switch (wino_dbg_env()) {
#define W_CASE(D) case D: hipLaunchKernelGGL(conv3x3_wino_f32<D>, g, dim3(256), WINO_LDS, s, a); return hipGetLastError();
    W_CASE(1) W_CASE(2) W_CASE(3) W_CASE(4) W_CASE(7) W_CASE(10) W_CASE(18) W_CASE(34) W_CASE(64) W_CASE(128) W_CASE(256) W_CASE(448) W_CASE(512)
#undef W_CASE
    default: break;
  }
#endif
  hipLaunchKernelGGL(conv3x3_wino_f32<0>, g, dim3(256), WINO_LDS, s, a);
  return hipGetLastError();
}

}
```

misonet_amd/csrc/kernels.hpp:

```cpp
#pragma once
#include <hip/hip_runtime.h>
#include <stdint.h>
#include <stdlib.h>
#include "det_stats.hpp"
#include "sig_view.hpp"

namespace mn {

constexpr int CK = 8;
constexpr int TT = 128;
constexpr int TW = 136;
constexpr int FT = 4;
constexpr float IN_EPS = 1e-5f;
constexpr float GLN_EPS = 1e-8f;

#ifdef MISONET_EXPERIMENTS
inline int exp_env(const char* name, int dflt) { const char* e = getenv(name); return e ? atoi(e) : dflt; }
#else
constexpr int exp_env(const char*, int dflt) { return dflt; }
#endif

inline int round_up(int x, int m) { return (x + m - 1) / m * m; }
inline int frames_pitch(int T) { return round_up(T, 32); }

struct ConvArgs {
  const float* in;
  const dstat_t* in_stats;
  float* out;
  dstat_t* out_stats;
  const float* w;
  const float* bias;
  const unsigned short* w16;
  const void* ww6;
  const float* wsm;
  const float* ww16;
  const float* w1d;
  const float* ww;
  long long in_bstride;
  long long out_bstride;
  int in_sstride, out_sstride;
  int in_c0, Cin, Fin;
  int ident_c;
  int out_c0, Cout, Fout;
  int T, Tp;
  int sf;
  int padf;
  int tr2;
  int act;
  int NR;
  int ncg;
  int cop;
  int in_oct, out_oct;
  float wscale, descale;
  const void* wps;
  long long wps_nstride;
  const float* btab;
  long long btab_nstride;
  int xcd;
  int ntx, nty, nsamp;
  unsigned long long* dbg_buf;
  int dbg;
};
struct ConvTile { int t_tile, f_tile, n, cg; bool valid; };
__device__ __forceinline__ ConvTile conv_tile(const ConvArgs& a) {
  ConvTile r;
  if (a.xcd) {
    const unsigned id = blockIdx.x;
    const unsigned xcd = id & 7u, k = id >> 3;
    const unsigned per = (unsigned)(a.ntx * a.nty * a.ncg);
    const unsigned grp = k / per;
    unsigned tile = k - grp * per;
    r.n = (int)(grp * 8u + xcd);
    r.t_tile = (int)(tile % (unsigned)a.ntx);
    tile /= (unsigned)a.ntx;
    r.cg = (int)(tile % (unsigned)a.ncg);
    r.f_tile = (int)(tile / (unsigned)a.ncg);
    r.valid = r.n < a.nsamp;
  } else {
    r.t_tile = blockIdx.x; r.f_tile = blockIdx.y;
    r.n = blockIdx.z / a.ncg; r.cg = blockIdx.z - r.n * a.ncg;
    r.valid = true;
  }
  return r;
}
inline dim3 conv_grid(ConvArgs& a, int n_samples, int tt, int ft, int xcd) {
  a.ntx = (a.T + tt - 1) / tt; a.nty = (a.Fout + ft - 1) / ft; a.nsamp = n_samples; a.xcd = xcd;
  if (xcd) return dim3((unsigned)(8 * ((n_samples + 7) / 8) * a.ntx * a.nty * a.ncg), 1, 1);
  return dim3(a.ntx, a.nty, n_samples * a.ncg);
}
int conv_xcd_env();
int device_cus();
int conv_cop(int Cout);
int conv_rows(int sf, int tr2);
hipError_t launch_conv(const ConvArgs& a, int n_samples, hipStream_t s);
hipError_t launch_conv_w1d(const ConvArgs& a, int n_samples, hipStream_t s);
hipError_t conv_init();
hipError_t launch_conv_wino(const ConvArgs& a, int n_samples, hipStream_t s);
hipError_t conv_wino_init();
hipError_t launch_conv_few(const ConvArgs& a, int n_samples, hipStream_t s);
hipError_t conv_few_init();
hipError_t launch_conv_wino6(const ConvArgs& a, int n_samples, hipStream_t s);
hipError_t conv_wino6_init();
hipError_t launch_conv_bf16(const ConvArgs& a, int n_samples, hipStream_t s);
hipError_t conv_bf16_init();
hipError_t launch_conv_bf16_dma(const ConvArgs& a, int n_samples, hipStream_t s);
hipError_t launch_conv_wprep(const ConvArgs& a, const float* wf, int n_samples, hipStream_t s);
hipError_t conv_bf16_dma_init();
hipError_t launch_conv_bf16x6(const ConvArgs& a, int n_samples, hipStream_t s);
hipError_t launch_conv_wprep6(const ConvArgs& a, const float* wf6, int n_samples, hipStream_t s);
hipError_t conv_bf16x6_init();
long long conv_bf16x6_wps_bytes(int Cin, int Cout);
hipError_t launch_conv_x6_first(const ConvArgs& a, const void* wimg, int n_samples, hipStream_t s);

int tcn_part_slots(int T);
hipError_t launch_tcn_prepare(const float* raw, long long raw_bstride, int raw_c0, const dstat_t* raw_stats, int raw_sstride,
                              float* x, double2* x_part, int C, int T, int Tp, int n_samples, hipStream_t s,
                              int raw_oct3 = 0);
hipError_t launch_tcn_dw(const float* x, const double2* x_part, int x_np, const float* wdw , const float* prelu ,
                         float* d, double2* gln_part , int C, int T, int Tp, int dilation, int n_samples, hipStream_t s,
                         int norm_kind = 0, const float* nsc = nullptr, const float* nsh = nullptr, const float2* fstat = nullptr);
hipError_t launch_tcn_cln_stats(const float* x, float2* fstat, int C, int T, int Tp, int n_samples, hipStream_t s);
hipError_t launch_tcn_pw(const float* d, const double2* gln_part, const float* gamma, const float* beta,
                         const float* wpw , const float* residual ,
                         float* y, long long y_bstride, int y_c0, double2* y_part , int C, int T, int Tp,
                         int n_samples, hipStream_t s,
                         int y_oct3_cbuf = 0, int x6 = 0);

hipError_t launch_pack(const float2* src, int B, int Mseg, int T, int F, float* dst, long long dst_bstride, int Tp,
                       int c_re, int c_im, int nshift, hipStream_t s);
hipError_t launch_unpack(const float* src, long long src_bstride, int Tp, int S, int T, int F, float2* dst, int n_samples,
                         int* nan_flag, hipStream_t s);
hipError_t launch_export(const float* src, long long src_bstride, int c0, int C, int Fq, int T, int Tp,
                         const dstat_t* stats, int sstride, int ident_c, float* dst, int n_samples, hipStream_t s,
                         int oct = 0);
hipError_t launch_unpack_ex(const float* src, long long src_bstride, int Tp, int S, int T, int F, int c_re0, int c_im0, int mode,
                            int M, const int* sel, float2* dst, int n_out, int* nan_flag, hipStream_t s);
hipError_t launch_compose_sel(const int* shift_sel, const int* clean_sel, int B, int M, int S, int* out, hipStream_t s);
hipError_t launch_assemble3(const float* in1, long long in1_bstride, const float* out1, long long out1_bstride,
                            const int* sel, int B, int M, int S, int ref_ch, int F, int Tp, float* in3,
                            long long in3_bstride, hipStream_t s);

hipError_t launch_stft_pack(const float* wav, int B, int L, int Mw, int T, const float* twid, float* dst,
                            long long dst_bstride, int Tp, int F, int c_re, int c_im, int nshift, hipStream_t s);
hipError_t stft_init();
void stft_build_twiddles(float* tw);
int stft_twiddle_count();
hipError_t launch_istft(const void* spec, int N, int T, const float* itw, short* out_i16, float* out_f32, hipStream_t s);
hipError_t istft_init();
void istft_build_twiddles(float* tw);
int istft_twiddle_count();
long long stft_stream_state_bytes(long long BM);
long long istft_stream_state_bytes(long long R);
hipError_t stft_stream_init();
hipError_t launch_stft_stream(const float* wav, int B, int n, int Mw, int Tn, int off0, int update, const float* twid,
                              float2* out, float* tail, hipStream_t s);
hipError_t launch_istft_stream(const void* spec, int R, int Tn, int lead, int fr0, int H, int update, const float* itw,
                               short* out_i16, float* out_f32, void* carry, hipStream_t s);

struct CView {
  const float* re; const float* im;
  long long sb, sf, sm; int st;
};
enum { BF_MVDR = 0, BF_SOUDEN = 1, BF_GEV = 2 };
struct MvdrArgs {
  CView mix;
  const float* est;
  long long est_bstride;
  const int* sel;
  CView src;
  int S;
  int B, F, M, T, Tp;
  float epsi;
  int kind = BF_MVDR;
  int noise_mix = 0;
  int trace_norm = 0;
  int ban = 0;
  int bf_ref = 0;
  double condition = 0.0;
};
long long mvdr_ws_bytes(int B, int S, int F, int M);
long long bf_ws_bytes(int B, int S, int F, int M, int kind);
struct COut { float* re; float* im; long long ob, os, ot, of; };
hipError_t launch_mvdr(const MvdrArgs& a, const COut& out, void* ws, hipStream_t s);
hipError_t launch_mvdr_debug(const void* ws, int B, int S, int F, int M, double* steer, double* w, hipStream_t s);
hipError_t launch_bf_debug(const void* ws, int B, int S, int F, int M, double* w, double* lam, hipStream_t s);

struct PitArgs {
  CView a, b;
// ... 229 lines not shown
```

misonet_amd/csrc/net.hip:

```cpp
#include "net.hpp"

#include <math.h>
#include <cmath>
#include <algorithm>
#include <stdarg.h>
#include <stdio.h>
#include <stdlib.h>
#include <string.h>

using namespace mn;

static thread_local char g_err[512] = "";
int mn::fail(int code, const char* fmt, ...) {
  va_list ap;
  va_start(ap, fmt);
  vsnprintf(g_err, sizeof(g_err), fmt, ap);
  va_end(ap);
  return code;
}

Prof mn::g_profs[MAX_DEV];
std::atomic<int> mn::g_prof_any{0};

static int find_tensor(const misonet_net* n, const std::string& name) {
// ... 117 lines not shown
      snprintf(nm, sizeof(nm), "decoders.%d.0", i);
      add_dense(n, n->dec, nm, buf, cin, cin / 2, cin, 0, B_X2 + (i - 2), 0);
      snprintf(nm, sizeof(nm), i == 6 ? "decoders.%d.1.deconv2d" : "decoders.%d.1.net.0", i);
      n->dec.push_back(make_conv(n, nm, B_X2 + (i - 2), 0, cin, 0, obuf, 0, cout, i == 6 ? 1 : 2, 0, true, i == 6 ? 0 : 1));
    } else {
      snprintf(nm, sizeof(nm), "decoders.%d.0.net.0", i);
      n->dec.push_back(make_conv(n, nm, buf, 0, cin, i == 0 ? de[0] : 0, obuf, 0, cout, i == 0 ? 1 : 2, 0, true, 1));
    }
  }
  for (int r = 0; r < 2; ++r)
    for (int x = 0; x < 7; ++x) {
      TcnBlock tb;
      tb.dilation = 1 << x;
      for (int h = 0; h < 2; ++h) {
        if (c.tcn_norm) {
          snprintf(nm, sizeof(nm), "TCN.temporal_conv_net.%d.%d.net.%d", r, x, h == 0 ? 0 : 3);
          const std::string q(nm);
          if (c.tcn_norm == 3) {
            tb.h[h].on[0] = add_tensor(n, q + ".weight", 128);
            tb.h[h].on[1] = add_tensor(n, q + ".bias", 128);
            tb.h[h].on[2] = add_tensor(n, q + ".running_mean", 128);
            tb.h[h].on[3] = add_tensor(n, q + ".running_var", 128);
          } else {
            tb.h[h].on[0] = add_tensor(n, q + ".gamma", 128);
            tb.h[h].on[1] = add_tensor(n, q + ".beta", 128);
          }
        }
        snprintf(nm, sizeof(nm), "TCN.temporal_conv_net.%d.%d.net.%d.net", r, x, h == 0 ? 2 : 5);
        const std::string p(nm);
        tb.h[h].dw = add_tensor(n, p + ".0.weight", 128 * 3);
        tb.h[h].prelu = add_tensor(n, p + ".1.weight", 1);
        tb.h[h].gamma = add_tensor(n, p + ".2.gamma", 128);
        tb.h[h].beta = add_tensor(n, p + ".2.beta", 128);
        tb.h[h].pw = add_tensor(n, p + ".3.weight", 128 * 128);
      }
      n->tcn.push_back(tb);
    }
  n->taps.push_back({"enc0_conv", B_E0, 0, en[0], false});
  for (int b = 0; b < 7; ++b) {
    snprintf(nm, sizeof(nm), "enc%d", b);
    n->taps.push_back({nm, B_D0 + (6 - b), de[6 - b], en[b], true});
  }
  n->taps.push_back({"tcn_out", B_D0, 0, 128, false});
  for (int i = 0; i < 6; ++i) {
    snprintf(nm, sizeof(nm), "dec%d", i);
    n->taps.push_back({nm, B_D0 + i + 1, 0, de[i + 1], true});
  }
  n->taps.push_back({"dec6", B_OUT, 0, c.out_ch, false});
  static const int x6first_env = exp_env("MISONET_X6_FIRST", 1);
  for (std::vector<ConvL>* v : {&n->enc, &n->dec})
    for (ConvL& l : *v)
      for (int mode = 0; mode < CONV_NMODES; ++mode) {
        const ConvShape sh = {l.Cin, l.Cout, n->bufs[l.in_buf].F, n->bufs[l.out_buf].F, l.sf, l.padf, l.tr2, l.act, l.transposed,
                              l.ident_c, l.in_buf == B_IN, buf_oct(mode, l.in_buf), buf_oct(mode, l.out_buf)};
        l.kind[mode] = conv_mode_built(mode) ? conv_select(sh, mode) : ConvKind::DIRECT;
        if (l.kind[mode] == ConvKind::X6_FIRST && !x6first_env) l.kind[mode] = ConvKind::DIRECT;
      }
  return MISONET_OK;
}

static inline long long buf_floats(const misonet_net* n, int Tp, int b) {
  const long long e = (long long)n->bufs[b].C * n->bufs[b].F * Tp;
  return buf_oct(n, b) == 3 ? e + e / 2 : e;
}
long long mn::bstride(const misonet_net* n, const Layout& L, int b) {
  if (b == B_IN && L.in_ext_off >= 0) return L.in_ext_bstride;
  return b >= B_TXA ? buf_floats(n, L.Tp, b) : L.sample_stride;
}

static void buf_lifetime(int b, int& t0, int& t1) {
  if (b == B_IN) { t0 = 0; t1 = 16; }
  else if (b >= B_E0 && b <= B_E4) { t0 = t1 = 1 + (b - B_E0); }
  else if (b >= B_D0 && b <= B_D6) { const int i = b - B_D0; t0 = 7 - i; t1 = 9 + i; }
  else if (b >= B_X2 && b <= B_X6) { t0 = t1 = 9 + 2 + (b - B_X2); }
  else { t0 = 15; t1 = 16; }
}

Layout mn::make_layout(const misonet_net* n, int N, int T, bool ext_in) {
  Layout L;
  L.N = N; L.T = T; L.Tp = frames_pitch(T);
  long long so = 0;
  for (int b = 0; b < NBUF; ++b) {
    L.stats_off[b] = so;
    so += (long long)N * n->bufs[b].C * 2 * DS_NL;
  }
  const long long tslots = tcn_part_slots(T);
  so = (so + 1) & ~1LL;
  L.tcn_xs = so;  so += 15LL * N * 128 * tslots * 2;
  L.tcn_ps = so;  so += 14LL * N * 128 * tslots * 2;
  L.tcn_gln = so; so += 28LL * N * 32 * 2;
  L.stats_doubles = so;
  L.data_base = align_up(256 + so * 8, 256);
  {
    struct Rect { int b, t0, t1; long long off, size; };
    std::vector<Rect> placed;
    std::vector<int> order;
    for (int b = 0; b < B_TXA; ++b)
      if (!(ext_in && b == B_IN)) order.push_back(b);
    L.data_off[B_IN] = 0;
    std::sort(order.begin(), order.end(), [&](int x, int y) {
      const long long sx = buf_floats(n, L.Tp, x), sy = buf_floats(n, L.Tp, y);
      return sx != sy ? sx > sy : x < y;
    });
    long long top = 0;
    for (int b : order) {
      Rect r;
      r.b = b;
      r.size = align_up(buf_floats(n, L.Tp, b), 64);
      buf_lifetime(b, r.t0, r.t1);
      if (n->keep_taps) { r.t0 = 0; r.t1 = 16; }
      std::vector<long long> cand(1, 0);
      for (const Rect& q : placed)
        if (q.t0 <= r.t1 && r.t0 <= q.t1) cand.push_back(q.off + q.size);
      std::sort(cand.begin(), cand.end());
      for (long long o : cand) {
        bool ok = true;
        for (const Rect& q : placed)
          if (q.t0 <= r.t1 && r.t0 <= q.t1 && o < q.off + q.size && q.off < o + r.size) { ok = false; break; }
        if (ok) { r.off = o; break; }
      }
      placed.push_back(r);
      L.data_off[b] = r.off;
      top = std::max(top, r.off + r.size);
    }
    L.sample_stride = top;
  }
  long long d = (long long)N * L.sample_stride;
  for (int b = B_TXA; b < NBUF; ++b) {
    L.data_off[b] = d;
    d += align_up((long long)N * buf_floats(n, L.Tp, b), 64);
  }
  long long wmax = 0, cmax = 0;
  auto scan = [&](const std::vector<ConvL>& v) {
    for (const ConvL& c : v) {
      const long long g = (c.Cout + 31) / 32, k = (c.Cin + 15) / 16;
      wmax = std::max(wmax, g * k * (2LL * 9 * 2 * 32 * 16));
      wmax = std::max(wmax, conv_bf16x6_wps_bytes((c.Cin + 7) / 8 * 8, c.Cout));
      cmax = std::max(cmax, g * 32);
    }
  };
  scan(n->enc); scan(n->dec);
  L.wps_base = align_up(L.data_base + d * 4, 256);
  L.wps_nstride = wmax;
  L.btab_base = align_up(L.wps_base + wmax * N, 256);
  L.btab_nstride = cmax * 9 * 4;
  L.fstat_base = align_up(L.btab_base + L.btab_nstride * 4 * N, 256);
  L.total_bytes = L.fstat_base + (n->cfg.tcn_norm == 2 ? (long long)N * L.Tp * 8 : 0);
  return L;
}

static inline dstat_t* stats_base(void* ws) { return reinterpret_cast<dstat_t*>(reinterpret_cast<char*>(ws) + 256); }
static inline dstat_t* stats_ptr(const Layout& L, void* ws, int b) { return stats_base(ws) + L.stats_off[b]; }

static int run_conv(const misonet_net* n, const Layout& L, void* ws, const ConvL& c, hipStream_t s, int n0 = 0, int nb = -1) {
  const ConvKind kind = c.kind[n->precision];
  if (nb < 0) nb = L.N;
  ConvArgs a = {};
  a.in_bstride = bstride(n, L, c.in_buf);
  a.out_bstride = bstride(n, L, c.out_buf);
  a.in_sstride = n->bufs[c.in_buf].C;
  a.out_sstride = n->bufs[c.out_buf].C;
  a.in = buf_ptr(L, ws, c.in_buf) + (long long)n0 * a.in_bstride;
  a.out = buf_ptr(L, ws, c.out_buf) + (long long)n0 * a.out_bstride;
  a.in_stats = stats_ptr(L, ws, c.in_buf) + (long long)n0 * a.in_sstride * 2 * DS_NL;
  a.out_stats = stats_ptr(L, ws, c.out_buf) + (long long)n0 * a.out_sstride * 2 * DS_NL;
  a.bias = n->w_dev + c.b_off;
  a.in_c0 = c.in_c0; a.Cin = c.Cin; a.Fin = n->bufs[c.in_buf].F; a.ident_c = c.ident_c;
  a.out_c0 = c.out_c0; a.Cout = c.Cout; a.Fout = n->bufs[c.out_buf].F;
  a.T = L.T; a.Tp = L.Tp;
  a.sf = c.sf; a.padf = c.padf; a.tr2 = c.tr2; a.act = c.act;
  a.in_oct = buf_oct(n, c.in_buf);
  a.out_oct = buf_oct(n, c.out_buf);
  a.cop = kind == ConvKind::DIRECT ? c.cop : 32;
  a.ncg = (c.Cout + a.cop - 1) / a.cop;
  a.wscale = a.descale = 1.f;
  static const int sync_dbg = exp_env("MISONET_SYNC_DEBUG", 0);
  struct SyncDbg {
    hipStream_t s; const ConvArgs& a; int on;
    ~SyncDbg() {
      if (!on) return;
      fprintf(stderr, "[conv] Cin=%d Cout=%d Fin=%d Fout=%d T=%d in_oct=%d out_oct=%d mode=%d ... ", a.Cin, a.Cout, a.Fin, a.Fout,
              a.T, a.in_oct, a.out_oct, a.tr2 ? 2 : (a.sf == 2 ? 1 : 0));
      const hipError_t e = hipStreamSynchronize(s);
      fprintf(stderr, "%s\n", hipGetErrorString(e));
    }
  } sync_guard{s, a, sync_dbg};
  auto prep = [&](hipError_t (*launch_wprep)(const ConvArgs&, const float*, int, hipStream_t)) {
    a.wps = reinterpret_cast<char*>(ws) + L.wps_base + (long long)n0 * L.wps_nstride;
    a.wps_nstride = L.wps_nstride;
    a.btab = reinterpret_cast<float*>(reinterpret_cast<char*>(ws) + L.btab_base) + (long long)n0 * L.btab_nstride;
    a.btab_nstride = L.btab_nstride;
    ProfScope pw(s, PK_OTHER);
    return launch_wprep(a, c.img(n->w_dev, kind), nb, s);
  };
  hipError_t e = hipSuccess;
  switch (kind) {
    case ConvKind::DIRECT: { a.w = c.img(n->w_dev, kind); ProfScope ps(s, PK_CONV); e = launch_conv(a, nb, s); } break;
    case ConvKind::W1D: { a.w1d = c.img(n->w_dev, kind); ProfScope ps(s, PK_CONV); e = launch_conv_w1d(a, nb, s); } break;
    case ConvKind::FEW: { a.wsm = c.img(n->w_dev, kind); ProfScope ps(s, PK_CONV); e = launch_conv_few(a, nb, s); } break;
    case ConvKind::WINO: {
      a.ww = c.img(n->w_dev, kind);
      if ((c.Cout & 31) == 16) a.ww16 = a.ww + conv_wino_ww16_at(c.Cin, c.Cout);
      ProfScope ps(s, PK_CONV);
      e = launch_conv_wino(a, nb, s);
    } break;
    case ConvKind::X6_FIRST: { ProfScope ps(s, PK_CONV); e = launch_conv_x6_first(a, c.img(n->w_dev, kind), nb, s); } break;
    case ConvKind::X6:
      e = prep(launch_conv_wprep6);
      if (e == hipSuccess) { ProfScope ps(s, PK_CONV); e = launch_conv_bf16x6(a, nb, s); }
      break;
#if MN_ALT_MODES
    case ConvKind::BF16: {
      a.w16 = reinterpret_cast<const unsigned short*>(c.img(n->w_dev, kind));
      ProfScope ps(s, PK_CONV);
      e = launch_conv_bf16(a, nb, s);
    } break;
    case ConvKind::BF16_DMA:
      if (a.in_oct == 4) { a.wscale = c.wscale; a.descale = 1.f / c.wscale; }
      e = prep(launch_conv_wprep);
      if (e == hipSuccess) { ProfScope ps(s, PK_CONV); e = launch_conv_bf16_dma(a, nb, s); }
      break;
    case ConvKind::WINO6: { a.ww6 = c.img(n->w_dev, kind); ProfScope ps(s, PK_CONV); e = launch_conv_wino6(a, nb, s); } break;
#endif
    default: e = hipErrorInvalidValue; break;
  }
  if (e == hipErrorInvalidValue)
    return fail(MISONET_EINVAL, "conv kernel kind %d refuses the layer Cin=%d Cout=%d Fin=%d Fout=%d sf=%d padf=%d tr2=%d act=%d in_oct=%d out_oct=%d (mode %d)",
                (int)kind, a.Cin, a.Cout, a.Fin, a.Fout, a.sf, a.padf, a.tr2, a.act, a.in_oct, a.out_oct, n->precision);
  HIPCHK(e);
  return MISONET_OK;
}

static unsigned layout_stamp(const misonet_net* n, const Layout& L) {
  unsigned h = 2166136261u;
  auto mix = [&](unsigned long long v) { for (int i = 0; i < 8; ++i) { h ^= (unsigned)(v & 0xff); h *= 16777619u; v >>= 8; } };
  mix(n->keep_taps ? 1 : 0); mix((unsigned)n->precision); mix((unsigned)L.N); mix((unsigned)L.T); mix((unsigned long long)L.total_bytes);
  return h | 1u;
}

int mn::forward_planar(misonet_net* n, const Layout& L, void* ws, hipStream_t s) {
  HIPCHK(hipMemsetAsync(ws, 0, (size_t)(256 + L.tcn_xs * 8), s));
  HIPCHK(hipMemsetD32Async(reinterpret_cast<hipDeviceptr_t>(reinterpret_cast<char*>(ws) + 8), (int)layout_stamp(n, L), 1, s));
  static const int sub_env = exp_env("MISONET_SUBBATCH", 0);
  auto run_stack = [&](const std::vector<ConvL>& v) -> int {
    if (sub_env <= 0) {
      for (const ConvL& c : v) { int r = run_conv(n, L, ws, c, s); if (r) return r; }
      return MISONET_OK;
    }
    size_t i = 0;
    while (i < v.size()) {
      const int Fg = n->bufs[v[i].out_buf].F;
      size_t j = i;
      while (j < v.size() && n->bufs[v[j].out_buf].F == Fg) ++j;
      int sb = sub_env * (127 / (Fg > 0 ? Fg : 1));
      if (sb < 1) sb = 1;
      for (int n0 = 0; n0 < L.N; n0 += sb) {
        const int nb = (L.N - n0) < sb ? (L.N - n0) : sb;
        for (size_t k = i; k < j; ++k) { int r = run_conv(n, L, ws, v[k], s, n0, nb); if (r) return r; }
      }
      i = j;
    }
    return MISONET_OK;
  };
  { int r = run_stack(n->enc); if (r) return r; }
  {
    ProfScope ps_tcn(s, PK_TCN);
    const int N = L.N, T = L.T, Tp = L.Tp;
    double2* xs = reinterpret_cast<double2*>(stats_base(ws) + L.tcn_xs);
    double2* ps = reinterpret_cast<double2*>(stats_base(ws) + L.tcn_ps);
    double2* gl = reinterpret_cast<double2*>(stats_base(ws) + L.tcn_gln);
    const int tslots = tcn_part_slots(T);
    const long long per = (long long)N * 128 * tslots;
    const long long gper = (long long)N * 32;
    float* xa = buf_ptr(L, ws, B_TXA);
    float* xb = buf_ptr(L, ws, B_TXB);
    float* td = buf_ptr(L, ws, B_TD);
    float* tp = buf_ptr(L, ws, B_TP);
    const int skip_c0 = n->cfg.de_ch[0];
    HIPCHK(launch_tcn_prepare(buf_ptr(L, ws, B_D0), bstride(n, L, B_D0), skip_c0, stats_ptr(L, ws, B_D0),
                              n->bufs[B_D0].C, xa, xs, 128, T, Tp, N, s, buf_oct(n, B_D0) == 3));
    float* cur = xa;
    float* nxt = xb;
    static const int tcn_x6_env = exp_env("MISONET_TCN_X6", 1);
    const int tcn_x6 = (n->precision == 3 && tcn_x6_env) ? 1 : 0;
    for (int k = 0; k < 14; ++k) {
      const TcnBlock& tb = n->tcn[k];
      const float* W = n->w_dev;
      const int nk = n->cfg.tcn_norm;
      float2* fstat = reinterpret_cast<float2*>(reinterpret_cast<char*>(ws) + L.fstat_base);
      if (nk == 2) HIPCHK(launch_tcn_cln_stats(cur, fstat, 128, T, Tp, N, s));
      HIPCHK(launch_tcn_dw(cur, xs + k * per, k == 0 ? 1 : tslots, W + tb.h[0].o_dw, W + tb.h[0].o_prelu, td, gl + (2 * k) * gper,
                           128, T, Tp, tb.dilation, N, s, nk, W + tb.h[0].o_nsc, W + tb.h[0].o_nsh, fstat));
      HIPCHK(launch_tcn_pw(td, gl + (2 * k) * gper, W + tb.h[0].o_gamma, W + tb.h[0].o_beta, W + tb.h[0].o_pw,
                           nullptr, tp, 128LL * Tp, 0, ps + k * per, 128, T, Tp, N, s, 0, tcn_x6));
      if (nk == 2) HIPCHK(launch_tcn_cln_stats(tp, fstat, 128, T, Tp, N, s));
      HIPCHK(launch_tcn_dw(tp, ps + k * per, tslots, W + tb.h[1].o_dw, W + tb.h[1].o_prelu, td,
                           gl + (2 * k + 1) * gper, 128, T, Tp, tb.dilation, N, s, nk, W + tb.h[1].o_nsc, W + tb.h[1].o_nsh, fstat));
      const bool last = (k == 13);
      float* y = last ? buf_ptr(L, ws, B_D0) : nxt;
      HIPCHK(launch_tcn_pw(td, gl + (2 * k + 1) * gper, W + tb.h[1].o_gamma, W + tb.h[1].o_beta,
                           W + tb.h[1].o_pw, cur, y, last ? bstride(n, L, B_D0) : 128LL * Tp, 0,
                           xs + (k + 1) * per, 128, T, Tp, N, s, (last && buf_oct(n, B_D0) == 3) ? n->bufs[B_D0].C : 0, tcn_x6));
      float* t = cur; cur = nxt; nxt = t;
    }
  }
  { int r = run_stack(n->dec); if (r) return r; }
  return MISONET_OK;
}

extern "C" {

const char* misonet_strerror(int code) {
  switch (code) {
    case MISONET_OK: return "ok";
    case MISONET_EINVAL: return "invalid argument / unsupported geometry";
    case MISONET_ESTATE: return "invalid call order or missing tensor";
    case MISONET_EHIP: return "HIP runtime error";
    case MISONET_ENOMEM: return "workspace too small";
    case MISONET_ENAN: return "NaN in network output";
    default: return "unknown error";
  }
}
const char* misonet_last_error(void) { return g_err; }
int misonet_version(void) { return 660; }

int misonet_net_create(const misonet_cfg* cfg, misonet_net** out) {
  if (!cfg || !out) return fail(MISONET_EINVAL, "null argument");
  misonet_net* n = new misonet_net();
  n->cfg = *cfg;
  int r = build_plan(n);
  if (r) { delete n; return r; }
  *out = n;
  return MISONET_OK;
}

int misonet_net_destroy(misonet_net* n) {
  if (!n) return MISONET_OK;
  if (n->w_dev) (void)hipFree(n->w_dev);
  delete n;
  return MISONET_OK;
}

int misonet_net_num_tensors(const misonet_net* n) { return n ? (int)n->tensors.size() : 0; }
const char* misonet_net_tensor_name(const misonet_net* n, int i) {
  if (!n || i < 0 || i >= (int)n->tensors.size()) return nullptr;
  return n->tensors[i].name.c_str();
}
long long misonet_net_tensor_numel(const misonet_net* n, int i) {
  if (!n || i < 0 || i >= (int)n->tensors.size()) return -1;
  return n->tensors[i].numel;
}

int misonet_net_set_tensor(misonet_net* n, const char* key, const float* host, long long numel) {
  if (!n || !key || !host) return fail(MISONET_EINVAL, "null argument");
  const int i = find_tensor(n, key);
  if (i < 0) return fail(MISONET_EINVAL, "unexpected state_dict key '%s'", key);
  if (n->tensors[i].numel != numel)
    return fail(MISONET_EINVAL, "size mismatch for '%s': expected %lld elements, got %lld", key, n->tensors[i].numel, numel);
  n->tensors[i].host.assign(host, host + numel);
  n->tensors[i].set = true;
  n->committed = false;
  return MISONET_OK;
}

static std::atomic<int> g_wino_state[MAX_DEV] = {};
static std::mutex g_wino_mu;
static int wino_selftest() {
  const int d = cur_dev();
  int st = g_wino_state[d].load(std::memory_order_acquire);
  if (st) return st;
  std::lock_guard<std::mutex> lk(g_wino_mu);
  st = g_wino_state[d].load(std::memory_order_acquire);
  if (st) return st;
  const int Cin = 40, Cout = 48, F = 11, T = 70, Tp = frames_pitch(T), N = 2;
  std::vector<float> W((size_t)Cout * Cin * 9), bias(Cout), x((size_t)N * Cin * F * Tp);
  unsigned rng = 12345u;
  auto rnd = [&rng]() { rng = rng * 1664525u + 1013904223u; return (float)((int)(rng >> 9) - (1 << 22)) * (1.f / (1 << 22)); };
  for (float& v : W) v = 0.1f * rnd();
  for (float& v : bias) v = 0.3f * rnd();
  for (float& v : x) v = rnd();
  const ConvWeights cw = {W.data(), Cin, Cout, false, 64, 1};
  std::vector<float> wd((size_t)conv_image_floats(ConvKind::DIRECT, cw)), ww((size_t)conv_image_floats(ConvKind::WINO, cw));
  conv_image_pack(ConvKind::DIRECT, cw, wd.data());
  conv_image_pack(ConvKind::WINO, cw, ww.data());
  const size_t out_n = (size_t)N * Cout * F * Tp, st_n = (size_t)N * Cout * 2 * DS_NL;
  float *dx = nullptr, *dwd = nullptr, *dww = nullptr, *db = nullptr, *dy = nullptr;
  dstat_t* dst = nullptr;
  auto release = [&]() { (void)hipFree(dx); (void)hipFree(dwd); (void)hipFree(dww); (void)hipFree(db); (void)hipFree(dy); (void)hipFree(dst); };
  bool ok = hipMalloc(reinterpret_cast<void**>(&dx), x.size() * 4) == hipSuccess && hipMalloc(reinterpret_cast<void**>(&dwd), wd.size() * 4) == hipSuccess &&
            hipMalloc(reinterpret_cast<void**>(&dww), ww.size() * 4) == hipSuccess &&
            hipMalloc(reinterpret_cast<void**>(&db), 128 * 4) == hipSuccess &&
            hipMalloc(reinterpret_cast<void**>(&dy), 2 * out_n * 4) == hipSuccess && hipMalloc(reinterpret_cast<void**>(&dst), 2 * st_n * 8) == hipSuccess;
  std::vector<float> y(2 * out_n);
  std::vector<dstat_t> sv(2 * st_n);
  if (ok) {
    std::vector<float> b128(128, 0.f);
    std::copy(bias.begin(), bias.end(), b128.begin());
    ok = hipMemcpy(dx, x.data(), x.size() * 4, hipMemcpyHostToDevice) == hipSuccess &&
         hipMemcpy(dwd, wd.data(), wd.size() * 4, hipMemcpyHostToDevice) == hipSuccess &&
         hipMemcpy(dww, ww.data(), ww.size() * 4, hipMemcpyHostToDevice) == hipSuccess &&
         hipMemcpy(db, b128.data(), 128 * 4, hipMemcpyHostToDevice) == hipSuccess &&
         hipMemset(dy, 0, 2 * out_n * 4) == hipSuccess && hipMemset(dst, 0, 2 * st_n * 8) == hipSuccess;
  }
  if (ok) {
    ConvArgs a = {};
    a.in = dx; a.in_stats = nullptr; a.w = dwd; a.bias = db; a.ww = dww; a.ww16 = dww + conv_wino_ww16_at(Cin, Cout);
    a.in_bstride = (long long)Cin * F * Tp; a.out_bstride = (long long)Cout * F * Tp;
    a.in_sstride = Cin; a.out_sstride = Cout;
    a.in_c0 = 0; a.Cin = Cin; a.Fin = F; a.ident_c = Cin;
    a.out_c0 = 0; a.Cout = Cout; a.Fout = F; a.T = T; a.Tp = Tp;
    a.sf = 1; a.padf = 1; a.tr2 = 0; a.act = 1; a.ncg = 1; a.cop = 64;
    a.wscale = a.descale = 1.f;
    a.out = dy; a.out_stats = dst;
    ok = launch_conv_wino(a, N, nullptr) == hipSuccess;
    a.ww = nullptr; a.ww16 = nullptr; a.out = dy + out_n; a.out_stats = dst + st_n;
    ok = ok && launch_conv(a, N, nullptr) == hipSuccess && hipDeviceSynchronize() == hipSuccess &&
         hipMemcpy(y.data(), dy, 2 * out_n * 4, hipMemcpyDeviceToHost) == hipSuccess &&
         hipMemcpy(sv.data(), dst, 2 * st_n * 8, hipMemcpyDeviceToHost) == hipSuccess;
  }
  release();
  if (ok) {
    double worst = 0.0, scale = 0.0;
    for (int nn = 0; nn < N; ++nn)
      for (int c = 0; c < Cout; ++c)
        for (int f = 0; f < F; ++f)
          for (int t = 0; t < T; ++t) {
            const size_t i = (((size_t)nn * Cout + c) * F + f) * Tp + t;
            worst = std::max(worst, (double)fabsf(y[i] - y[out_n + i]));
            scale = std::max(scale, (double)fabsf(y[out_n + i]));
          }
    ok = std::isfinite(worst) && scale > 0.0 && worst <= 2e-5 * scale;
    for (size_t i = 0; ok && i < st_n / DS_NL; ++i) {
      auto rd = [](const dstat_t* p) { long long L[DS_NL]; for (int k = 0; k < DS_NL; ++k) L[k] = (long long)p[k]; return dstat_combine(L); };
      const double a1 = rd(sv.data() + i * DS_NL), a2 = rd(sv.data() + st_n + i * DS_NL);
      ok = std::isfinite(a1) && fabs(a1 - a2) <= 1e-4 * (fabs(a2) + 1.0);
    }
    if (!ok) fprintf(stderr, "[misonet] conv3x3_wino_f32 self-check FAILED on device %d (max |diff| %.3e of %.3e): mode f32w disabled\n", d, worst, scale);
  }
  st = ok ? 1 : 2;
  g_wino_state[d].store(st, std::memory_order_release);
  return st;
}

int misonet_net_commit(misonet_net* n) {
  if (!n) return fail(MISONET_EINVAL, "null argument");
  for (const Tensor& t : n->tensors)
    if (!t.set) return fail(MISONET_ESTATE, "missing state_dict key '%s'", t.name.c_str());
  long long off = 0;
  auto take = [&off](long long nfl) { long long o = off; off += (nfl + 63) / 64 * 64; return o; };
  auto conv_weights = [n](const ConvL& c) { return ConvWeights{n->tensors[c.wt].host.data(), c.Cin, c.Cout, c.transposed, c.cop, c.ncg}; };
  for (std::vector<ConvL>* v : {&n->enc, &n->dec})
    for (ConvL& c : *v) {
      std::fill(c.img_off, c.img_off + CONV_NKIND, -1LL);
      c.img_off[(int)ConvKind::DIRECT] = take(conv_image_floats(ConvKind::DIRECT, conv_weights(c)));
      c.b_off = take((long long)c.ncg * c.cop);
      for (int mode = 0; mode < CONV_NMODES; ++mode) {
        long long& o = c.img_off[(int)c.kind[mode]];
        if (conv_mode_built(mode) && o < 0) o = take(conv_image_floats(c.kind[mode], conv_weights(c)));
      }
    }
  for (TcnBlock& tb : n->tcn)
    for (int h = 0; h < 2; ++h) {
      tb.h[h].o_dw = take(128 * 3);
      tb.h[h].o_prelu = take(1);
      tb.h[h].o_gamma = take(128);
      tb.h[h].o_beta = take(128);
      tb.h[h].o_pw = take(128 * 128);
      tb.h[h].o_nsc = take(128);
      tb.h[h].o_nsh = take(128);
    }
  std::vector<float> arena((size_t)off, 0.f);
  for (std::vector<ConvL>* v : {&n->enc, &n->dec})
    for (ConvL& c : *v) {
      for (int k = 0; k < CONV_NKIND; ++k)
        if (c.img_off[k] >= 0) conv_image_pack((ConvKind)k, conv_weights(c), arena.data() + c.img_off[k]);
      const std::vector<float>& Bv = n->tensors[c.bt].host;
      for (int co = 0; co < c.ncg * c.cop; ++co) arena[c.b_off + co] = co < c.Cout ? Bv[co] : 0.f;
      if (MN_ALT_MODES) c.wscale = conv_f16_wscale(n->tensors[c.wt].host.data(), n->tensors[c.wt].numel);
    }
  for (const TcnBlock& tb : n->tcn)
    for (int h = 0; h < 2; ++h) {
      const TcnHalf& H = tb.h[h];
      memcpy(arena.data() + H.o_dw, n->tensors[H.dw].host.data(), 128 * 3 * sizeof(float));
      arena[H.o_prelu] = n->tensors[H.prelu].host[0];
      memcpy(arena.data() + H.o_gamma, n->tensors[H.gamma].host.data(), 128 * sizeof(float));
      memcpy(arena.data() + H.o_beta, n->tensors[H.beta].host.data(), 128 * sizeof(float));
      if (n->cfg.tcn_norm == 3) {
        const float *w = n->tensors[H.on[0]].host.data(), *b = n->tensors[H.on[1]].host.data(),
                    *rm = n->tensors[H.on[2]].host.data(), *rv = n->tensors[H.on[3]].host.data();
        for (int ch = 0; ch < 128; ++ch) {
          const float sc = w[ch] / sqrtf(rv[ch] + 1e-5f);
          arena[H.o_nsc + ch] = sc;
          arena[H.o_nsh + ch] = b[ch] - rm[ch] * sc;
        }
      } else if (n->cfg.tcn_norm) {
        memcpy(arena.data() + H.o_nsc, n->tensors[H.on[0]].host.data(), 128 * sizeof(float));
        memcpy(arena.data() + H.o_nsh, n->tensors[H.on[1]].host.data(), 128 * sizeof(float));
      }
      const std::vector<float>& P = n->tensors[H.pw].host;
      for (int co = 0; co < 128; ++co)
        for (int ci = 0; ci < 128; ++ci) arena[H.o_pw + (long long)ci * 128 + co] = P[(long long)co * 128 + ci];
    }
  if (n->w_dev) { (void)hipFree(n->w_dev); n->w_dev = nullptr; }
  HIPCHK(hipMalloc(reinterpret_cast<void**>(&n->w_dev), arena.size() * sizeof(float)));
  HIPCHK(hipMemcpy(n->w_dev, arena.data(), arena.size() * sizeof(float), hipMemcpyHostToDevice));
  HIPCHK(conv_init());
  HIPCHK(conv_wino_init());
  HIPCHK(conv_few_init());
#ifdef MISONET_EXPERIMENTS
  if (!exp_env("MISONET_WINO_DBG", 0))
#endif
  if (wino_selftest() != 1 && n->precision == 5)
    return fail(MISONET_ESTATE, "the f32w kernel failed its self-check on this device (see stderr): use mode 0 (f32) or 3 (bf16x6)");
#if MN_ALT_MODES
  HIPCHK(conv_wino6_init());
  HIPCHK(conv_bf16_init());
  HIPCHK(conv_bf16_dma_init());
#endif
  HIPCHK(conv_bf16x6_init());
  { int rf = misonet_frontend_init(); if (rf) return rf; }
  n->committed = true;
  return MISONET_OK;
}

int misonet_net_set_precision(misonet_net* n, int mode) {
  if (!n) return fail(MISONET_EINVAL, "null argument");
  if (mode < 0 || mode >= CONV_NMODES || !conv_mode_built(mode))
    return fail(MISONET_EINVAL, "precision mode must be 0 (f32), 3 (bf16x6) or 5 (f32w: f32 with the dense-block convs in Winograd form)%s",
                MN_ALT_MODES ? "; experiment build: also 1 / 2 (bf16x3), 4 (f16x3), 6 (bf16x6w)"
                             : "; modes 1, 2, 4, 6 exist only in the experiment build (make exp)");
  if (mode == 5 && g_wino_state[cur_dev()].load(std::memory_order_acquire) == 2)
    return fail(MISONET_ESTATE, "the f32w kernel failed its self-check on this device: mode 5 is disabled (use 0 or 3)");
  n->precision = mode;
  return MISONET_OK;
}
int misonet_net_get_precision(const misonet_net* n) { return n ? n->precision : -1; }

int misonet_net_buffer_plan(const misonet_net* n, int n_frames, int max_buffers, long long* offset_bytes,
                            long long* size_bytes, int* first_step, int* last_step) {
  if (!n || n_frames <= 0 || !offset_bytes || !size_bytes || !first_step || !last_step) return fail(MISONET_EINVAL, "null argument");
  const Layout L = make_layout(n, 1, n_frames);
  int k = 0;
  for (int b = 0; b < B_TXA && k < max_buffers; ++b, ++k) {
    offset_bytes[k] = L.data_off[b] * 4;
    size_bytes[k] = buf_floats(n, L.Tp, b) * 4;
    buf_lifetime(b, first_step[k], last_step[k]);
    if (n->keep_taps) { first_step[k] = 0; last_step[k] = 16; }
  }
  return k;
}

int misonet_net_conv_plan(const misonet_net* n, int mode, int max_layers, int* kind) {
  if (!n || !kind) return fail(MISONET_EINVAL, "null argument");
  if (mode < 0 || mode >= CONV_NMODES || !conv_mode_built(mode)) return fail(MISONET_EINVAL, "precision mode %d is not in this build", mode);
  int k = 0;
  for (const std::vector<ConvL>* v : {&n->enc, &n->dec})
    for (const ConvL& c : *v)
      if (k < max_layers) kind[k++] = (int)c.kind[mode];
  return k;
}

int misonet_net_keep_activations(misonet_net* n, int keep) {
  if (!n) return fail(MISONET_EINVAL, "null argument");
  n->keep_taps = keep != 0;
  return MISONET_OK;
}

long long misonet_net_workspace_bytes(const misonet_net* n, int n_samples, int n_frames) {
  if (!n || n_samples <= 0 || n_frames <= 0) return -1;
  return make_layout(n, n_samples, n_frames).total_bytes;
}

int misonet_net_forward(misonet_net* n, int n_seg, const void* const* seg_dev, const int* seg_ch, int B, int T,
                        void* out_dev, void* ws, long long ws_bytes, misonet_stream stream) {
  if (!n || !seg_dev || !seg_ch || !out_dev || !ws) return fail(MISONET_EINVAL, "null argument");
  if (!n->committed) return fail(MISONET_ESTATE, "misonet_net_commit has not been called");
  if (B <= 0 || T <= 0) return fail(MISONET_EINVAL, "B and T must be positive");
  int tot = 0;
  for (int i = 0; i < n_seg; ++i) tot += seg_ch[i];
  if (2 * tot != n->cfg.in_ch) return fail(MISONET_EINVAL, "input segments give %d complex channels, network expects %d", tot, n->cfg.in_ch / 2);
  const Layout L = make_layout(n, B, T);
  if (ws_bytes < L.total_bytes) return fail(MISONET_ENOMEM, "workspace %lld < %lld bytes", ws_bytes, L.total_bytes);
  hipStream_t s = reinterpret_cast<hipStream_t>(stream);
  int c0 = 0;
  for (int i = 0; i < n_seg; ++i) {
    HIPCHK(launch_pack(reinterpret_cast<const float2*>(seg_dev[i]), B, seg_ch[i], T, n->cfg.n_freq, buf_ptr(L, ws, B_IN),
                       bstride(n, L, B_IN), L.Tp, c0, tot + c0, 1, s));
    c0 += seg_ch[i];
  }
  int r = forward_planar(n, L, ws, s);
  if (r) return r;
  HIPCHK(launch_unpack(buf_ptr(L, ws, B_OUT), bstride(n, L, B_OUT), L.Tp, n->S, T, n->cfg.n_freq,
                       reinterpret_cast<float2*>(out_dev), B, reinterpret_cast<int*>(ws), s));
  return MISONET_OK;
}

int misonet_net_check(misonet_net* n, const void* ws, misonet_stream stream) {
  if (!n || !ws) return fail(MISONET_EINVAL, "null argument");
  int flag = 0;
  HIPCHK(hipMemcpyAsync(&flag, ws, sizeof(int), hipMemcpyDeviceToHost, reinterpret_cast<hipStream_t>(stream)));
  HIPCHK(hipStreamSynchronize(reinterpret_cast<hipStream_t>(stream)));
  if (flag) return fail(MISONET_ENAN, "NaN in network output");
  return MISONET_OK;
}

int misonet_net_tap_shape(const misonet_net* n, const char* name, int* C, int* F) {
  if (!n || !name) return fail(MISONET_EINVAL, "null argument");
  for (const Tap& t : n->taps)
    if (t.name == name) {
      if (C) *C = t.C;
      if (F) *F = n->bufs[t.buf].F;
      return MISONET_OK;
    }
  return fail(MISONET_EINVAL, "unknown tap '%s'", name);
}

int misonet_net_tap(misonet_net* n, const char* name, const void* ws, int B, int T, float* dst, misonet_stream stream) {
  if (!n || !name || !ws || !dst) return fail(MISONET_EINVAL, "null argument");
  const Layout L = make_layout(n, B, T);
  for (const Tap& t : n->taps)
    if (t.name == name) {
      if (!n->keep_taps && t.buf != B_OUT)
        return fail(MISONET_ESTATE, "tap '%s': activation buffers share memory; call misonet_net_keep_activations(net, 1) "
                                    "before the forward", name);
      {
        unsigned stamp = 0;
        hipStream_t s_ = reinterpret_cast<hipStream_t>(stream);
        HIPCHK(hipMemcpyAsync(&stamp, reinterpret_cast<const char*>(ws) + 8, sizeof(stamp), hipMemcpyDeviceToHost, s_));
        HIPCHK(hipStreamSynchronize(s_));
        if (stamp != layout_stamp(n, L))
          return fail(MISONET_ESTATE, "tap '%s': the forward in this workspace ran with another buffer plan / mode / shape "
                                      "(keep_activations, precision, B or T changed since); run the forward again", name);
      }
      void* w = const_cast<void*>(ws);
      HIPCHK(launch_export(buf_ptr(L, w, t.buf), bstride(n, L, t.buf), t.c0, t.C, n->bufs[t.buf].F, T, L.Tp,
                           t.normalised ? stats_ptr(L, w, t.buf) : nullptr, n->bufs[t.buf].C, 0, dst, B,
                           reinterpret_cast<hipStream_t>(stream), buf_oct(n, t.buf) >= 3 ? buf_oct(n, t.buf) : (buf_oct(n, t.buf) ? 2 : 0)));
      return MISONET_OK;
    }
  return fail(MISONET_EINVAL, "unknown tap '%s'", name);
}

int misonet_profile_begin(int max_launches) {
  if (max_launches <= 0) return fail(MISONET_EINVAL, "max_launches must be positive");
  Prof& pr = g_profs[cur_dev()];
  while (pr.pool.size() < (size_t)max_launches * 2) {
    hipEvent_t e;
    HIPCHK(hipEventCreate(&e));
    pr.pool.push_back(e);
  }
  pr.used = 0;
  pr.recs.clear();
  pr.overflow = false;
  if (!pr.on) g_prof_any.fetch_add(1);
  pr.on = true;
  return MISONET_OK;
}
int misonet_profile_end(double* ms_by_kind, long long* launches_by_kind) {
  Prof& pr = g_profs[cur_dev()];
  if (pr.on) g_prof_any.fetch_sub(1);
  pr.on = false;
  if (!ms_by_kind || !launches_by_kind) return fail(MISONET_EINVAL, "null argument");
  for (int k = 0; k < PK_N; ++k) { ms_by_kind[k] = 0.0; launches_by_kind[k] = 0; }
  for (const ProfRec& r : pr.recs) {
    HIPCHK(hipEventSynchronize(r.e1));
    float ms = 0.f;
    HIPCHK(hipEventElapsedTime(&ms, r.e0, r.e1));
    ms_by_kind[r.kind] += ms;
    launches_by_kind[r.kind] += 1;
  }
  if (pr.overflow) return fail(MISONET_ENOMEM, "profile event pool exhausted");
  return MISONET_OK;
}

int misonet_event_create(void** ev) {
  hipEvent_t e;
  HIPCHK(hipEventCreate(&e));
  *ev = e;
  return MISONET_OK;
}
int misonet_event_record(void* ev, misonet_stream stream) {
  HIPCHK(hipEventRecord(reinterpret_cast<hipEvent_t>(ev), reinterpret_cast<hipStream_t>(stream)));
  return MISONET_OK;
}
int misonet_event_elapsed_ms(void* start, void* stop, float* ms) {
  HIPCHK(hipEventSynchronize(reinterpret_cast<hipEvent_t>(stop)));
  HIPCHK(hipEventElapsedTime(ms, reinterpret_cast<hipEvent_t>(start), reinterpret_cast<hipEvent_t>(stop)));
  return MISONET_OK;
}
int misonet_event_destroy(void* ev) {
  HIPCHK(hipEventDestroy(reinterpret_cast<hipEvent_t>(ev)));
  return MISONET_OK;
}

}
```

Baseline: 151.6 utt/s.

## Add one-pass Winograd kernel variant for 48-output-channel conv layers

Adds a one-pass Winograd f32 conv path for layers with 48 output channels. It uses a wider time tile of 32 and all three 16-channel output groups in one workgroup, with its own packed weight image and LDS geometry. Before, these layers needed a 32-channel launch plus a separate 16-channel pass; now they can run in one launch with no repeated input staging. It adds a self-check against the direct kernel and falls back to the two-launch dispatch if the check fails. It also adds a standalone dense-layer test entry point.

New measurement: 153.0 utt/s (median of 6 runs). About the same (+0.9%).

```diff
diff --git a/include/misonet.h b/include/misonet.h
--- a/include/misonet.h
+++ b/include/misonet.h
@@ -52,6 +52,10 @@
 int misonet_net_buffer_plan(const misonet_net* net, int n_frames, int max_buffers, long long* offset_bytes,
                             long long* size_bytes, int* first_step, int* last_step);
 int misonet_net_conv_plan(const misonet_net* net, int mode, int max_layers, int* kind);
+
+int misonet_conv_dense_layer(int path, int n_samples, int c_in, int c_out, int n_freq, int n_frames, const float* w_host,
+                             const float* bias_host, const float* x_dev, float* y_dev, unsigned long long* stats_dev,
+                             misonet_stream stream);
 int misonet_net_tap_shape(const misonet_net* net, const char* name, int* C, int* F);
 int misonet_net_tap(misonet_net* net, const char* name, const void* ws_dev, int B, int T, float* dst_dev,
                     misonet_stream stream);
diff --git a/misonet_amd/_lib.py b/misonet_amd/_lib.py
--- a/misonet_amd/_lib.py
+++ b/misonet_amd/_lib.py
@@ -84,6 +84,7 @@
     "misonet_net_buffer_plan": (C.c_int, [C.c_void_p, C.c_int, C.c_int, C.POINTER(C.c_longlong), C.POINTER(C.c_longlong),
                                           C.POINTER(C.c_int), C.POINTER(C.c_int)]),
     "misonet_net_conv_plan": (C.c_int, [C.c_void_p, C.c_int, C.c_int, C.POINTER(C.c_int)]),
+    "misonet_conv_dense_layer": (C.c_int, [C.c_int] * 6 + [C.c_void_p] * 6),
     "misonet_net_workspace_bytes": (C.c_longlong, [C.c_void_p, C.c_int, C.c_int]),
     "misonet_net_forward": (C.c_int, [C.c_void_p, C.c_int, C.POINTER(C.c_void_p), C.POINTER(C.c_int), C.c_int, C.c_int,
                                       C.c_void_p, C.c_void_p, C.c_longlong, C.c_void_p]),
diff --git a/misonet_amd/csrc/conv_select.hpp b/misonet_amd/csrc/conv_select.hpp
--- a/misonet_amd/csrc/conv_select.hpp
+++ b/misonet_amd/csrc/conv_select.hpp
@@ -69,6 +69,10 @@
 long long conv_image_floats(ConvKind k, const ConvWeights& c);
 void conv_image_pack(ConvKind k, const ConvWeights& c, float* img);
 inline long long conv_wino_ww16_at(int Cin, int Cout) { return (long long)((Cout + 31) / 32) * (Cin / 8) * 16 * 8 * 32; }
+inline int conv_wino_onepass_ncg(int Cout) { return Cout == 48 ? 3 : 0; }
+inline long long conv_wino_wwop_at(int Cin, int Cout) {
+  return conv_wino_ww16_at(Cin, Cout) + ((Cout & 31) == 16 ? (long long)(Cin / 8) * 2048 : 0);
+}
 float conv_f16_wscale(const float* W, long long n);
 
 }
diff --git a/misonet_amd/csrc/conv_weights.hip b/misonet_amd/csrc/conv_weights.hip
--- a/misonet_amd/csrc/conv_weights.hip
+++ b/misonet_amd/csrc/conv_weights.hip
@@ -168,6 +168,20 @@
         }
       }
 }
+static void wino_image_onepass(const ConvWeights& c, int ncg, float* img) {
+  const int nchunk = c.Cin / 8;
+  for (int kc = 0; kc < nchunk; ++kc)
+    for (int cil = 0; cil < 8; ++cil)
+      for (int co = 0; co < 16 * ncg; ++co) {
+        const int ci = kc * 8 + cil, cg = co >> 4, col = co & 15;
+        for (int pos = 0; pos < 16; ++pos) {
+          const int xi = pos >> 2, nu = pos & 3;
+          const double u = co < c.Cout ? wino_u(c, co, ci, xi, nu) : 0.0;
+          const int s = cil >> 2, kk = cil & 3;
+          img[(((((((long long)kc * 2 + s) * 4 + (pos >> 2)) * ncg + cg) * 4 + kk) * 16 + col) * 4) + (pos & 3)] = (float)(wino_minus(xi, nu) ? -u : u);
+        }
+      }
+}
 
 static void wino6_image(const ConvWeights& c, float* dst) {
   const int nk = (c.Cin + 15) / 16, ncg = (c.Cout + 31) / 32;
@@ -198,7 +212,7 @@
     case ConvKind::DIRECT: return (long long)c.ncg * ((c.Cin + CK - 1) / CK) * 9 * CK * c.cop;
     case ConvKind::W1D: return g32 * ((c.Cin + CK - 1) / CK) * 12 * CK * 32;
     case ConvKind::FEW: return (long long)c.Cin * 36;
-    case ConvKind::WINO: return conv_wino_ww16_at(c.Cin, c.Cout) + ((c.Cout & 31) == 16 ? (long long)(c.Cin / 8) * 2048 : 0);
+    case ConvKind::WINO: return conv_wino_wwop_at(c.Cin, c.Cout) + (long long)conv_wino_onepass_ncg(c.Cout) * (c.Cin / 8) * 2048;
     case ConvKind::X6_FIRST: return k8 * 864 * 4;
     case ConvKind::X6: return g32 * k8 * 9 * 32 * 8;
     case ConvKind::BF16: return g32 * k16 * 2 * 9 * 2 * 32 * 8 / 2;
@@ -216,6 +230,7 @@
     case ConvKind::WINO:
       wino_image(c, img);
       if ((c.Cout & 31) == 16) wino_image16(c, c.Cout - 16, img + conv_wino_ww16_at(c.Cin, c.Cout));
+      if (conv_wino_onepass_ncg(c.Cout)) wino_image_onepass(c, conv_wino_onepass_ncg(c.Cout), img + conv_wino_wwop_at(c.Cin, c.Cout));
       break;
     case ConvKind::X6_FIRST: w6s_image(c, img); break;
     case ConvKind::X6: wf6_image(c, img); break;
diff --git a/misonet_amd/csrc/conv_wino.hip b/misonet_amd/csrc/conv_wino.hip
--- a/misonet_amd/csrc/conv_wino.hip
+++ b/misonet_amd/csrc/conv_wino.hip
@@ -66,9 +66,42 @@
 constexpr size_t WINO_LDS = WBIAS_B + WCO_MAX * 24;
 static_assert(WINO_LDS <= 160 * 1024, "one workgroup per CU: at most 160 KB of LDS");
 
-template <int DBG, bool G16 = false>
-__global__ __launch_bounds__(256, 1) void conv3x3_wino_f32(const ConvArgs a) {
+template <int NCG>
+struct WGeo {
+  static constexpr bool OP = NCG > 0;
+  static constexpr int TT = OP ? 32 : mn::WTT;
+  static constexpr int TW = TT + 2;
+  static constexpr int SQN = TT / 4;
+  static constexpr int SCRN = 256 / SQN;
+  static constexpr int NIT = OP ? 3 : 5;
+  static constexpr int IN_FLOATS = OP ? NIT * SCRN * TW : WCK * WNR * TW;
+  static constexpr int IMG_FLOATS = OP ? 2048 * NCG : WW_FLOATS;
+  static constexpr int STAGE_FLOATS = IN_FLOATS + IMG_FLOATS;
+  static constexpr int RAWI_FLOATS = OP ? NIT * 1024 : WCK * WNR * TT;
+  static constexpr int RAW_FLOATS = RAWI_FLOATS + 256;
+  static constexpr int RED_CO = OP ? 64 : 32;
+  static constexpr unsigned RAW_B = (unsigned)(WNSTAGE * STAGE_FLOATS) * 4u;
+  static constexpr unsigned NRM_B = RAW_B + 2u * RAW_FLOATS * 4u;
+  static constexpr unsigned ZERO_B = NRM_B + 2u * WNRM_MAX * 8u;
+  static constexpr unsigned RED_B = ZERO_B + WNRM_MAX * 8u;
+  static constexpr unsigned DUMMY_B = RED_B + 4u * RED_CO * 2u * 4u;
+  static constexpr unsigned BIAS_B = DUMMY_B + 64u * 4u;
+  static constexpr size_t LDS = BIAS_B + WCO_MAX * 24;
+  static_assert(NIT * SCRN >= WCK * WNR && (IN_FLOATS % 4) == 0, "the pieces cover the chunk's items; the U image starts 16-byte aligned");
+  static_assert(LDS <= 160 * 1024, "one workgroup per CU: at most 160 KB of LDS");
+};
+static_assert(WGeo<0>::LDS == WINO_LDS && WGeo<0>::BIAS_B == WBIAS_B && WGeo<0>::RAW_B == WRAW_B, "NCG = 0 is the map above");
+constexpr int WOP_NCG = 3;
+
+template <int DBG, bool G16, int NCG>
+__device__ __forceinline__ void wino_body(const ConvArgs& a) {
   extern __shared__ __align__(16) float smem[];
+  using Geo = WGeo<NCG>;
+  constexpr bool OP = Geo::OP;
+  static_assert(!(OP && G16), "the one-pass body is its own operand path");
+  constexpr int WTT = Geo::TT, WTW = Geo::TW, WSCRN = Geo::SCRN, WNIT = Geo::NIT;
+  constexpr int WIN_FLOATS = Geo::IN_FLOATS, WSTAGE_FLOATS = Geo::STAGE_FLOATS, WRAWI_FLOATS = Geo::RAWI_FLOATS, WRAW_FLOATS = Geo::RAW_FLOATS;
+  constexpr unsigned WRAW_B = Geo::RAW_B, WNRM_B = Geo::NRM_B, WZERO_B = Geo::ZERO_B, WRED_B = Geo::RED_B, WDUMMY_B = Geo::DUMMY_B, WBIAS_B = Geo::BIAS_B;
   char* const smem_c = reinterpret_cast<char*>(smem);
   wf2* s_nrm = reinterpret_cast<wf2*>(smem_c + WNRM_B);
   wf2* s_zero = reinterpret_cast<wf2*>(smem_c + WZERO_B);
@@ -80,7 +113,7 @@
   const int kk = lane >> 4, nn = lane & 15;
   const int T = a.T, Tp = a.Tp, F = a.Fin, Cin = a.Cin;
   const int nchunk = Cin / WCK;
-  constexpr unsigned WIMG_B = G16 ? 2u * 4u * 4u * 16u * 16u : (unsigned)(WW_FLOATS * 4);
+  constexpr unsigned WIMG_B = OP ? (unsigned)(Geo::IMG_FLOATS * 4) : G16 ? 2u * 4u * 4u * 16u * 16u : (unsigned)(WW_FLOATS * 4);
 
   const unsigned tps = (unsigned)(a.ntx * a.nty * a.ncg);
   unsigned q0, qstep, Q, xcd_id = 0;
@@ -98,7 +131,7 @@
   const unsigned ntile = (Q - q0 + qstep - 1) / qstep;
   for (int i = tid; i < WNRM_MAX; i += 256) s_zero[i] = wf2{0.f, 0.f};
   if (tid < WCO_MAX) {
-    const float b = tid < a.ncg * 32 ? a.bias[tid] : 0.f;
+    const float b = tid < (OP ? a.Cout : a.ncg * 32) ? a.bias[tid] : 0.f;
     const float c = elu_fast(b);
     wf2* tb = reinterpret_cast<wf2*>(smem_c + WBIAS_B + tid * 24);
     tb[0] = wf2{b, b}; tb[1] = wf2{-c, -c}; tb[2] = wf2{-1.f - c, -1.f - c};
@@ -107,28 +140,28 @@
   const unsigned row_e = (unsigned)Tp;
   const unsigned plane_b = (unsigned)F * row_e * 4u;
 
-  const int sq = tid & 15, scr = tid >> 4;
+  const int sq = tid & (Geo::SQN - 1), scr = tid / Geo::SQN;
   int sch[5];
 #pragma unroll
-  for (int i = 0; i < 5; ++i) sch[i] = (scr + 16 * i) / WNR;
+  for (int i = 0; i < WNIT; ++i) sch[i] = (scr + WSCRN * i) / WNR;
   const bool hrole = tid < 2 * WCK * WNR;
   const int hit = hrole ? tid >> 1 : 0, hside = tid & 1;
   const int hch = hit / WNR, hrow = hit - hch * WNR;
   const unsigned lds0 = (unsigned)(unsigned long long)MN_WLDS(smem);
-  constexpr unsigned STAGE_B = (unsigned)WSTAGE_FLOATS * 4u, STEP_B = (unsigned)((G16 ? 4 : 2) * WNR * WTW) * 4u;
-  const unsigned dbase = G16 ? lds0 + (unsigned)((kk * WNR + 2 * wave) * WTW + 2 * nn) * 4u
+  constexpr unsigned STAGE_B = (unsigned)WSTAGE_FLOATS * 4u, STEP_B = (unsigned)((G16 || OP ? 4 : 2) * WNR * WTW) * 4u;
+  const unsigned dbase = (G16 || OP) ? lds0 + (unsigned)((kk * WNR + 2 * wave) * WTW + 2 * nn) * 4u
                              : lds0 + (unsigned)((half * WNR + 2 * wave) * WTW + 2 * l31) * 4u;
   unsigned d1 = launder(dbase + STEP_B), d2 = launder(dbase + 2 * STEP_B), d3 = launder(dbase + 3 * STEP_B);
   unsigned d0n = launder(dbase + STAGE_B);
-  unsigned uc = launder(lds0 + (unsigned)WIN_FLOATS * 4u + (unsigned)(G16 ? kk * 16 + nn : half * 32 + l31) * 16u);
+  unsigned uc = launder(lds0 + (unsigned)WIN_FLOATS * 4u + (unsigned)((G16 || OP) ? kk * 16 + nn : half * 32 + l31) * 16u);
   unsigned un = launder(uc + STAGE_B);
   unsigned cn = launder(lds0 + STAGE_B + (unsigned)(scr * WTW + 1 + 4 * sq) * 4u);
   unsigned hn = launder(lds0 + (hrole ? STAGE_B + (unsigned)(hit * WTW + (hside ? WTT + 1 : 0)) * 4u : WDUMMY_B + (unsigned)(tid & 63) * 4u));
 #define W_LP(TYPE, ADDR) (reinterpret_cast<__attribute__((address_space(3))) TYPE*>(ADDR))
   const unsigned rofs0 = lds0 + WRAW_B + (unsigned)(scr * WTT + 4 * sq) * 4u;
-  const unsigned rhofs0 = lds0 + WRAW_B + (unsigned)(WCK * WNR * WTT + tid) * 4u;
+  const unsigned rhofs0 = lds0 + WRAW_B + (unsigned)(WRAWI_FLOATS + tid) * 4u;
   const unsigned rdma0 = WRAW_B + (unsigned)wave * 1024u;
-  const unsigned rhdma0 = WRAW_B + (unsigned)(WCK * WNR * WTT) * 4u + (unsigned)wave * 256u;
+  const unsigned rhdma0 = WRAW_B + (unsigned)WRAWI_FLOATS * 4u + (unsigned)wave * 256u;
   const unsigned wdma0 = (unsigned)(WIN_FLOATS * 4) + (unsigned)wave * 1024u;
   const __amdgpu_buffer_rsrc_t rs_w = make_rsrc_e(reinterpret_cast<unsigned long long>(a.ww),
                                                    (unsigned)(a.ncg * nchunk) * WIMG_B);
@@ -194,11 +227,12 @@
     const int tge_ = tg_ + 4 <= Tp ? tg_ : Tp - 4;                                                    \
     Lfull = t0_ + WTT <= T;                                                                           \
     Lmask = (tg_ < T ? 1u : 0u) | (tg_ + 1 < T ? 2u : 0u) | (tg_ + 2 < T ? 4u : 0u) | (tg_ + 3 < T ? 8u : 0u); \
-    _Pragma("unroll") for (int i = 0; i < 5; ++i) {                                                   \
-      int fin = fin0_ + (scr + 16 * i) - sch[i] * WNR;                                                \
-      Lnr[i] = lds0 + ((fin >= 0 && fin < F) ? WNRM_B + (unsigned)(Lpar * WNRM_MAX + sch[i]) * 8u : WZERO_B); \
+    _Pragma("unroll") for (int i = 0; i < WNIT; ++i) {                                                \
+      int fin = fin0_ + (scr + WSCRN * i) - sch[i] * WNR;                                             \
+      Lnr[i] = lds0 + ((fin >= 0 && fin < F && sch[i] < WCK) ? WNRM_B + (unsigned)(Lpar * WNRM_MAX + sch[i]) * 8u : WZERO_B); \
       fin = fin < 0 ? 0 : (fin >= F ? F - 1 : fin);                                                   \
-      Lgoff[i] = (unsigned)sch[i] * plane_b + (unsigned)((fin * (int)row_e + tge_) * 4);              \
+       \
+      Lgoff[i] = (unsigned)(sch[i] < WCK ? sch[i] : 0) * plane_b + (unsigned)((fin * (int)row_e + tge_) * 4); \
     }                                                                                                 \
     {                                                                                                 \
       const int htg_ = hside ? t0_ + WTT : t0_ - 1;                                                   \
@@ -238,6 +272,9 @@
   __builtin_amdgcn_raw_ptr_buffer_load_lds(rs_l, MN_WLDS(smem_c + rhdma0 + lslot * (WRAW_FLOATS * 4)), 4, Lhoff, W_CB, 0, 0);
 #define W_ISSUE_W(J, ST, WSO)                                                                         \
   __builtin_amdgcn_raw_ptr_buffer_load_lds(rs_w, MN_WLDS(smem_c + (ST) * (WSTAGE_FLOATS * 4) + wdma0 + (G16 ? ((J) & 1) : (J)) * 4096), 16, wvo[J], WSO, 0, 0);
+#define W_ISSUE_WOP(J, ST, WSO)                                                                       \
+  if constexpr ((J) < 2 * NCG) __builtin_amdgcn_raw_ptr_buffer_load_lds(rs_w, MN_WLDS(smem_c + (ST) * (WSTAGE_FLOATS * 4) + wdma0 + (J) * 4096), 16, wvo[0], (WSO) + (unsigned)(J) * 4096u, 0, 0);
+#define W_VMCNT_N(N) asm volatile("s_waitcnt vmcnt(%0)" ::"n"(N) : "memory");
 #define W_WSO_L ((unsigned)(Lcg * nchunk + kl) * WIMG_B)
 #define W_VMCNT(N) asm volatile("s_waitcnt vmcnt(" #N ")" ::: "memory");
 #define W_NR(DST, I) DST = *W_LP(const wf2, Cnr[I]);
@@ -256,10 +293,10 @@
 #define W_DSW(ADDR, VAL, OFF) asm volatile("ds_write_b32 %0, %1 offset:%2" ::"v"(ADDR), "v"(VAL), "n"(OFF) : "memory");
 #define W_CW(CV, I)                                                                                   \
   {                                                                                                   \
-    W_DSW(cn, CV[0].x, (I) * (16 * WTW * 4))                                                          \
-    W_DSW(cn, CV[0].y, (I) * (16 * WTW * 4) + 4)                                                      \
-    W_DSW(cn, CV[1].x, (I) * (16 * WTW * 4) + 8)                                                      \
-    W_DSW(cn, CV[1].y, (I) * (16 * WTW * 4) + 12)                                                     \
+    W_DSW(cn, CV[0].x, (I) * (WSCRN * WTW * 4))                                                          \
+    W_DSW(cn, CV[0].y, (I) * (WSCRN * WTW * 4) + 4)                                                      \
+    W_DSW(cn, CV[1].x, (I) * (WSCRN * WTW * 4) + 8)                                                      \
+    W_DSW(cn, CV[1].y, (I) * (WSCRN * WTW * 4) + 12)                                                     \
   }
 #define W_CWH W_DSW(hn, chv, 0)
 #define W_BARRIER { asm volatile("s_waitcnt lgkmcnt(0)" ::: "memory"); __builtin_amdgcn_s_barrier(); asm volatile("" ::: "memory"); }
@@ -267,6 +304,7 @@
   wf2 dd16[2][4][2];
   wf2 vp16[2][4][2];
   wf2 dd[4][2];
+  wf4 uop[4][4];
   wf4 u[4];
   wf2 vp[4][2];
 #define W_FD(I0, DREG)                                                                                \
@@ -324,8 +362,8 @@
   W_TRANSFORM XG W_SB
 
   constexpr int W_NDMA_W = 4, W_NDMA_I = 6, W_NSTORE = 16;
-  static_assert(W_NDMA_W * 256 * 16 == WW_FLOATS * 4, "U image = 4 pieces of 256 threads x 16 bytes");
-  static_assert(5 * 256 * 16 == WCK * WNR * WTT * 4 && 2 * WCK * WNR <= 256, "raw input = 5 pieces of 256 x 16 bytes + one 4-byte halo piece");
+  static_assert(OP || W_NDMA_W * 256 * 16 == WW_FLOATS * 4, "U image = 4 pieces of 256 threads x 16 bytes");
+  static_assert(OP || (5 * 256 * 16 == WCK * WNR * WTT * 4 && 2 * WCK * WNR <= 256), "raw input = 5 pieces of 256 x 16 bytes + one 4-byte halo piece");
   static_assert(W_NDMA_W + W_NDMA_I == 10 && W_NDMA_I == 6 && 10 + W_NSTORE == 26 && 6 + W_NSTORE == 22,
                 "the s_waitcnt vmcnt immediates of W_CHUNK_ (10 / 26 in step 0, 6 / 22 in front of the barrier)");
 #define W_BK_S1  \
@@ -343,10 +381,10 @@
   const unsigned rsl_ = cslot ? (unsigned)(WRAW_FLOATS * 4) : 0u;
 #define W_BK_V                                                                                        \
   if (__builtin_expect(nxt0_, 0)) {                                                                   \
-    _Pragma("unroll") for (int i = 0; i < 6; ++i) Cnr[i] = Lnr[i];                                    \
+    _Pragma("unroll") for (int i = 0; i < 6; ++i) if (i < WNIT || i == 5) Cnr[i] = Lnr[i];            \
     Cmask = Lmask;                                                                                    \
   } else {                                                                                            \
-    _Pragma("unroll") for (int i = 0; i < 6; ++i) Cnr[i] += (unsigned)(WCK * 8);                      \
+    _Pragma("unroll") for (int i = 0; i < 6; ++i) if (i < WNIT || i == 5) Cnr[i] += (unsigned)(WCK * 8); \
   }                                                                                                   \
   d1 = d0n + STEP_B; d2 = d0n + 2 * STEP_B; d3 = d0n + 3 * STEP_B;                                    \
   uc = un;                                                                                            \
@@ -441,7 +479,70 @@
   W_S16(30, 1, W_BK_S1 W_BK_S2 W_BK_S3)                                                               \
   W_S16(31, 1)                                                                                        \
   W_TRANSFORM16(0) W_TRANSFORM16(1) W_BK_V W_SB
-#define W_BODY_ if constexpr (G16) { W_CHUNK16_ } else { W_CHUNK_ }
+  constexpr int OP_NW = 2 * NCG, OP_NI = WNIT + 1, OP_NS = 4 * NCG;
+  static_assert(!OP || (OP_NW + OP_NI + OP_NS <= 63 && OP_NW <= 8), "vmcnt is a 6-bit counter; W_ISSUE_WALL lists 8 pieces");
+#define W_FUOP(Q, UREG, S)                                                                            \
+  wfor<(NCG > 0 ? NCG : 1)>([&](auto cgc) __attribute__((always_inline)) {                           \
+    constexpr int cg_ = decltype(cgc)::value;                                                         \
+    uop[Q][cg_] = *W_LP(const wf4, UREG + (((S) * 4 + (Q)) * NCG + cg_) * 1024);                      \
+  });
+#define W_MFOP(P, CG, CS) wino_mfma16<(P) * NCG + (CG), (POST == 2 && (CS) == 0)>(uop[(P) >> 2][CG][(P) & 3], vp16[0][(P) >> 2][((P) & 3) >> 1][(P) & 1]);
+#define W_POS(P, CS, X0, X1, X2)                                                                      \
+  W_MFOP(P, 0, CS) X0 W_SB                                                                            \
+  W_MFOP(P, 1, CS) X1 W_SB                                                                            \
+  W_MFOP(P, 2, CS) X2 W_SB                                                                            \
+  if constexpr (NCG > 3) { W_MFOP(P, 3, CS) W_SB }
+#define W_CHUNKOP_                                                                                    \
+    \
+  W_POS(0, 0, W_FUOP(3, uc, 0), W_X(if (POST) { W_VMCNT_N(OP_NW + OP_NI + OP_NS) } else { W_VMCNT_N(OP_NW + OP_NI) } W_RR(rwa, 0)), W_X(W_RR(rwb, 1))) \
+  W_POS(1, 0, W_X(W_NR(nra, 0)), W_X(W_NR(nrb, 1)), W_NONE)                                           \
+  W_POS(2, 0, W_NONE, W_NONE, W_NONE)                                                                 \
+  W_POS(3, 0, W_NONE, W_NONE, W_X(W_CC(cva, rwa, nra) W_CC(cvb, rwb, nrb)))                           \
+  W_POS(4, 0, W_FUOP(0, uc, 1), W_X(W_CW(cva, 0)), W_X(W_CW(cvb, 1)))                                 \
+  W_POS(5, 0, W_FD16(0, 0, d1), W_FD16(0, 2, d1), W_X(W_RR(rwa, 2)))                                  \
+  W_POS(6, 0, W_X(W_RRH), W_X(W_NR(nra, 2)), W_X(W_NR(nrb, 5)))                                       \
+  W_POS(7, 0, W_NONE, W_NONE, W_NONE)                                                                 \
+  W_POS(8, 0, W_FUOP(1, uc, 1), W_NONE, W_NONE)                                                       \
+  W_POS(9, 0, W_NONE, W_NONE, W_X(W_CC(cva, rwa, nra) W_CCH(nrb)))                                    \
+  W_POS(10, 0, W_X(W_CW(cva, 2)), W_X(W_CWH), W_NONE)                                                 \
+  W_POS(11, 0, W_NONE, W_NONE, W_NONE)                                                                \
+  W_POS(12, 0, W_FUOP(2, uc, 1), W_NONE, W_NONE)                                                      \
+  W_POS(13, 0, W_NONE, W_NONE, W_NONE)                                                                \
+  W_POS(14, 0, W_NONE, W_NONE, W_NONE)                                                                \
+  W_POS(15, 0, W_NONE, W_NONE, W_NONE)                                                                \
+  W_TRANSFORM16(0) W_SB                                                                               \
+        \
+  W_POS(0, 1, W_FUOP(3, uc, 1), W_NONE, W_NONE)                                                       \
+  W_POS(1, 1, W_NONE, W_NONE, W_NONE)                                                                 \
+  W_XW(if (POST == 2) { W_VMCNT_N(OP_NI + OP_NS) } else { W_VMCNT_N(OP_NI) }) W_BARRIER               \
+  W_POS(2, 1, W_XW(W_ISSUE_WOP(0, stnn, Dwso)), W_XW(W_ISSUE_WOP(1, stnn, Dwso)), W_XW(W_ISSUE_WOP(2, stnn, Dwso))) \
+  W_POS(3, 1, W_XW(W_ISSUE_WOP(3, stnn, Dwso)), W_XW(W_ISSUE_WOP(4, stnn, Dwso)), W_XW(W_ISSUE_WOP(5, stnn, Dwso))) \
+  W_POS(4, 1, W_FUOP(0, un, 0), W_XW(W_ISSUE_WOP(6, stnn, Dwso)), W_XW(W_ISSUE_WOP(7, stnn, Dwso)))   \
+  W_POS(5, 1, W_FD16(0, 0, d0n), W_FD16(0, 2, d0n), W_XL(W_ISSUE_I(0)))                               \
+  W_POS(6, 1, W_XL(W_ISSUE_I(1)), W_XL(W_ISSUE_I(2)), W_XL(W_ISSUE_H))                                \
+  W_POS(7, 1, W_NONE, W_NONE, W_NONE)                                                                 \
+  W_POS(8, 1, W_FUOP(1, un, 0), W_NONE, W_NONE)                                                       \
+  W_POS(9, 1, W_NONE, W_NONE, W_NONE)                                                                 \
+  W_POS(10, 1, W_NONE, W_NONE, W_NONE)                                                                \
+  W_POS(11, 1, W_NONE, W_NONE, W_NONE)                                                                \
+  W_POS(12, 1, W_FUOP(2, un, 0), W_NONE, W_NONE)                                                      \
+  W_POS(13, 1, W_NONE, W_NONE, W_NONE)                                                                \
+  W_POS(14, 1, W_BK_S1 W_BK_S2 W_BK_S3, W_NONE, W_NONE)                                               \
+  W_POS(15, 1, W_NONE, W_NONE, W_NONE)                                                                \
+  W_TRANSFORM16(0) W_BK_V W_SB
+#define W_BODY_ if constexpr (OP) { W_CHUNKOP_ } else if constexpr (G16) { W_CHUNK16_ } else { W_CHUNK_ }
+
+#define W_ISSUE_WALL(ST)                                                                              \
+  if constexpr (OP) {                                                                                 \
+    W_ISSUE_WOP(0, ST, W_WSO_L) W_ISSUE_WOP(1, ST, W_WSO_L) W_ISSUE_WOP(2, ST, W_WSO_L) W_ISSUE_WOP(3, ST, W_WSO_L)  \
+    W_ISSUE_WOP(4, ST, W_WSO_L) W_ISSUE_WOP(5, ST, W_WSO_L) W_ISSUE_WOP(6, ST, W_WSO_L) W_ISSUE_WOP(7, ST, W_WSO_L)  \
+  } else {                                                                                            \
+    W_ISSUE_W(0, ST, W_WSO_L) W_ISSUE_W(1, ST, W_WSO_L) W_ISSUE_W(2, ST, W_WSO_L) W_ISSUE_W(3, ST, W_WSO_L)          \
+  }
+#define W_ISSUE_IALL                                                                                  \
+  W_ISSUE_I(0) W_ISSUE_I(1) W_ISSUE_I(2)                                                              \
+  if constexpr (!OP) { W_ISSUE_I(3) W_ISSUE_I(4) }                                                    \
+  W_ISSUE_H
 
   constexpr bool RAG = true;
   W_LOAD_SETUP(ql)
@@ -449,12 +550,10 @@
   for (int i = 0; i < 6; ++i) Cnr[i] = Lnr[i];
   Cmask = Lmask; Cfull = Lfull;
   __syncthreads();
-  W_ISSUE_W(0, 0, W_WSO_L) W_ISSUE_W(1, 0, W_WSO_L) W_ISSUE_W(2, 0, W_WSO_L) W_ISSUE_W(3, 0, W_WSO_L)
-  W_ISSUE_I(0) W_ISSUE_I(1) W_ISSUE_I(2) W_ISSUE_I(3) W_ISSUE_I(4) W_ISSUE_H
+  W_ISSUE_WALL(0) W_ISSUE_IALL
   W_LATCH
   W_ADVANCE
-  W_ISSUE_W(0, 1, W_WSO_L) W_ISSUE_W(1, 1, W_WSO_L) W_ISSUE_W(2, 1, W_WSO_L) W_ISSUE_W(3, 1, W_WSO_L)
-  W_ISSUE_I(0) W_ISSUE_I(1) W_ISSUE_I(2) W_ISSUE_I(3) W_ISSUE_I(4) W_ISSUE_H
+  W_ISSUE_WALL(1) W_ISSUE_IALL
   W_LATCH
   W_ADVANCE
   W_VMCNT(0)
@@ -463,22 +562,27 @@
   W_RR(rwa, 0) W_NR(nra, 0) W_CC(cva, rwa, nra) W_CW(cva, 0)
   W_RR(rwa, 1) W_NR(nra, 1) W_CC(cva, rwa, nra) W_CW(cva, 1)
   W_RR(rwa, 2) W_NR(nra, 2) W_CC(cva, rwa, nra) W_CW(cva, 2)
-  W_RR(rwa, 3) W_NR(nra, 3) W_CC(cva, rwa, nra) W_CW(cva, 3)
-  W_RR(rwa, 4) W_NR(nra, 4) W_CC(cva, rwa, nra) W_CW(cva, 4)
+  if constexpr (!OP) {
+    W_RR(rwa, 3) W_NR(nra, 3) W_CC(cva, rwa, nra) W_CW(cva, 3)
+    W_RR(rwa, 4) W_NR(nra, 4) W_CC(cva, rwa, nra) W_CW(cva, 4)
+  }
   W_RRH W_NR(nrb, 5) W_CCH(nrb) W_CWH
 #pragma unroll
   for (int i = 0; i < 6; ++i) Cnr[i] += (unsigned)(WCK * 8);
   cn += STAGE_B;
   if (hrole) hn += STAGE_B;
   asm volatile("s_waitcnt lgkmcnt(0)" ::: "memory");
-  W_ISSUE_I(0) W_ISSUE_I(1) W_ISSUE_I(2) W_ISSUE_I(3) W_ISSUE_I(4) W_ISSUE_H
+  W_ISSUE_IALL
   W_LATCH
   W_ADVANCE
   cslot = 1;
   rofs = rofs0 + WRAW_FLOATS * 4;
   rhofs = rhofs0 + WRAW_FLOATS * 4;
   W_BARRIER
-  if constexpr (G16) {
+  if constexpr (OP) {
+    W_FD16(0, 0, dbase) W_FD16(0, 2, dbase) W_FUOP(0, uc, 0) W_FUOP(1, uc, 0) W_FUOP(2, uc, 0)
+    W_TRANSFORM16(0)
+  } else if constexpr (G16) {
     W_FD16(0, 0, dbase) W_FD16(0, 2, dbase) W_FD16(1, 0, dbase) W_FD16(1, 2, dbase) W_FU16(0, uc, 0) W_FU16(1, uc, 0) W_FU16(2, uc, 0)
     W_TRANSFORM16(0) W_TRANSFORM16(1)
   } else {
@@ -551,7 +655,42 @@
       auto dummy_store = [&]() __attribute__((always_inline)) {
         if (!(DBG & 64)) __builtin_amdgcn_raw_buffer_store_b128(u32x4_t{0u, 0u, 0u, 0u}, rs_out, 0x80000000u, 0, 2);
       };
-      if constexpr (G16) {
+      if constexpr (OP) {
+        const bool ev = (nn & 1) == 0;
+        const unsigned tabop = launder(lds0 + WBIAS_B + (unsigned)(4 * kk) * 24u);
+        float s1g[4 * (NCG > 0 ? NCG : 1)], s2g[4 * (NCG > 0 ? NCG : 1)];
+        const int t = t0 + 2 * nn;
+        const bool c0ok = t < T, c1ok = t + 1 < T;
+        const unsigned vbase = (unsigned)(fa * Tp + t) * 4u + (unsigned)(4 * kk) * P4;
+        const unsigned vo_x = ev ? ((r0ok && c0ok) ? vbase : 0x80000000u)
+                                 : ((r1ok && t - 2 < T) ? vbase + (unsigned)Tp * 4u - 8u : 0x80000000u);
+        wf2 mt = {(r0ok && c0ok) ? 1.f : 0.f, (r0ok && c1ok) ? 1.f : 0.f}, mb = {(r1ok && c0ok) ? 1.f : 0.f, (r1ok && c1ok) ? 1.f : 0.f};
+        asm volatile("" : "+v"(mt), "+v"(mb));
+        wfor<(NCG > 0 ? NCG : 1)>([&](auto cgc) __attribute__((always_inline)) {
+          constexpr int cg_ = decltype(cgc)::value;
+          wfor<4>([&](auto rc) __attribute__((always_inline)) {
+            constexpr int r = decltype(rc)::value;
+            epi_item([&](auto xc, auto nc) __attribute__((always_inline)) { return agpr_get<((4 * decltype(xc)::value + decltype(nc)::value) * NCG + cg_) * 4 + r>(); },
+                     tabop + (16 * cg_ + r) * 24, vo_x + (unsigned)(16 * cg_ + r) * P4, ev, mt, mb, s1g[4 * cg_ + r], s2g[4 * cg_ + r]);
+          });
+        });
+        W_STAMP(11)
+        if (!(DBG & 128)) {
+          wfor<4 * (NCG > 0 ? NCG : 1)>([&](auto ic) __attribute__((always_inline)) {
+            constexpr int i = decltype(ic)::value;
+            float x1 = s1g[i], x2 = s2g[i];
+            x1 += dpp_get<0xB1>(x1); x2 += dpp_get<0xB1>(x2);
+            x1 += dpp_get<0x4E>(x1); x2 += dpp_get<0x4E>(x2);
+            x1 += dpp_get<0x141>(x1); x2 += dpp_get<0x141>(x2);
+            x1 += dpp_get<0x140>(x1); x2 += dpp_get<0x140>(x2);
+            if (nn == 0) {
+              const unsigned ra_ = red_a + (unsigned)((wave * Geo::RED_CO + 16 * (i >> 2) + 4 * kk + (i & 3)) * 2) * 4u;
+              lds_write_f32<0>(ra_, x1);
+              lds_write_f32<4>(ra_, x2);
+            }
+          });
+        }
+      } else if constexpr (G16) {
         const bool ev = (nn & 1) == 0;
         const unsigned tab16 = launder(lds0 + WBIAS_B + (unsigned)(cbase + 4 * kk) * 24u);
         float s1g[8], s2g[8];
@@ -630,14 +769,15 @@
       }
       if (!(DBG & 128)) {
         W_BARRIER
-        if (lane < 16) {
-          const int pr = wave * 16 + lane;
+        constexpr int TAILN = OP ? 8 * NCG : 16;
+        if (lane < TAILN) {
+          const int pr = wave * TAILN + lane;
           const int co_l = pr >> 1, which = pr & 1;
           const int co = cbase + co_l;
           if (co < a.Cout) {
             float tot = 0.f;
             for (int w = 0; w < 4; ++w)
-              if (f0 + 2 * w < F) tot += *W_LP(const float, red_a + (unsigned)((w * 32 + co_l) * 2 + which) * 4u);
+              if (f0 + 2 * w < F) tot += *W_LP(const float, red_a + (unsigned)((w * Geo::RED_CO + co_l) * 2 + which) * 4u);
             dstat_add(a.out_stats + (((long long)n * a.out_sstride + a.out_c0 + co) * 2 + which) * DS_NL, (double)tot);
           }
         }
@@ -660,6 +800,11 @@
   }
 }
 
+template <int DBG, bool G16 = false>
+__global__ __launch_bounds__(256, 1) void conv3x3_wino_f32(const ConvArgs a) { wino_body<DBG, G16, 0>(a); }
+template <int NCG>
+__global__ __launch_bounds__(256, 1) void conv3x3_wino_f32_onepass(const ConvArgs a) { wino_body<0, false, NCG>(a); }
+
 bool conv_wino_ok(const ConvShape& s) {
   return s.act && s.Cin >= 3 * WCK && s.Cout <= WCO_MAX && s.sf == 1 && s.padf == 1 && !s.tr2 && s.Fin == s.Fout && (s.Cin % WCK) == 0 && s.Cin <= WNRM_MAX && !s.in_oct &&
          !s.out_oct;
@@ -677,6 +822,9 @@
                                      (int)WINO_LDS);
   if (e == hipSuccess)
     e = hipFuncSetAttribute(reinterpret_cast<const void*>(&conv3x3_wino_f32<0, true>), hipFuncAttributeMaxDynamicSharedMemorySize, (int)WINO_LDS);
+  if (e == hipSuccess)
+    e = hipFuncSetAttribute(reinterpret_cast<const void*>(&conv3x3_wino_f32_onepass<WOP_NCG>), hipFuncAttributeMaxDynamicSharedMemorySize,
+                            (int)WGeo<WOP_NCG>::LDS);
 #ifdef MISONET_EXPERIMENTS
 #define W_ATTR(D) if (e == hipSuccess) e = hipFuncSetAttribute(reinterpret_cast<const void*>(&conv3x3_wino_f32<D>), hipFuncAttributeMaxDynamicSharedMemorySize, (int)WINO_LDS);
   W_ATTR(1) W_ATTR(2) W_ATTR(3) W_ATTR(4) W_ATTR(7) W_ATTR(10) W_ATTR(18) W_ATTR(34) W_ATTR(64) W_ATTR(128) W_ATTR(256) W_ATTR(448) W_ATTR(512)
@@ -687,8 +835,22 @@
 
 static hipError_t launch_wino_groups(ConvArgs a, int n_samples, hipStream_t s, bool g16);
 
+static hipError_t launch_wino_onepass(ConvArgs a, int n_samples, hipStream_t s) {
+  a.ww = a.wwop;
+  a.cop = 16 * WOP_NCG;
+  a.ncg = 1;
+  const int cus = device_cus();
+  if (cus <= 0) return hipErrorInvalidDevice;
+  (void)conv_grid(a, n_samples, WGeo<WOP_NCG>::TT, WFT, (n_samples % 8 == 0 && cus % 8 == 0) ? conv_xcd_env() : 0);
+  const long long tiles = (long long)n_samples * a.ntx * a.nty;
+  const unsigned grid = (unsigned)(tiles < cus ? tiles : cus);
+  hipLaunchKernelGGL((conv3x3_wino_f32_onepass<WOP_NCG>), dim3(a.xcd ? (unsigned)cus : grid), dim3(256), WGeo<WOP_NCG>::LDS, s, a);
+  return hipGetLastError();
+}
+
 hipError_t launch_conv_wino(const ConvArgs& a_in, int n_samples, hipStream_t s) {
   if (!conv_wino_ok(conv_shape(a_in)) || !a_in.ww) return hipErrorInvalidValue;
+  if (a_in.wwop != nullptr && conv_wino_onepass_ncg(a_in.Cout) == WOP_NCG) return launch_wino_onepass(a_in, n_samples, s);
   if ((a_in.Cout & 31) == 16 && a_in.ww16 != nullptr) {
     const int c32 = a_in.Cout - 16;
     if (c32 > 0) {
diff --git a/misonet_amd/csrc/kernels.hpp b/misonet_amd/csrc/kernels.hpp
--- a/misonet_amd/csrc/kernels.hpp
+++ b/misonet_amd/csrc/kernels.hpp
@@ -34,6 +34,7 @@
   const void* ww6;
   const float* wsm;
   const float* ww16;
+  const float* wwop;
   const float* w1d;
   const float* ww;
   long long in_bstride;
diff --git a/misonet_amd/csrc/net.hip b/misonet_amd/csrc/net.hip
--- a/misonet_amd/csrc/net.hip
+++ b/misonet_amd/csrc/net.hip
@@ -293,6 +293,9 @@
 static inline dstat_t* stats_base(void* ws) { return reinterpret_cast<dstat_t*>(reinterpret_cast<char*>(ws) + 256); }
 static inline dstat_t* stats_ptr(const Layout& L, void* ws, int b) { return stats_base(ws) + L.stats_off[b]; }
 
+static std::atomic<int> g_wino_op_state[MAX_DEV] = {};
+static bool wino_onepass_checked() { return g_wino_op_state[cur_dev()].load(std::memory_order_acquire) == 1; }
+
 static int run_conv(const misonet_net* n, const Layout& L, void* ws, const ConvL& c, hipStream_t s, int n0 = 0, int nb = -1) {
   const ConvKind kind = c.kind[n->precision];
   if (nb < 0) nb = L.N;
@@ -342,6 +345,7 @@
     case ConvKind::WINO: {
       a.ww = c.img(n->w_dev, kind);
       if ((c.Cout & 31) == 16) a.ww16 = a.ww + conv_wino_ww16_at(c.Cin, c.Cout);
+      if (conv_wino_onepass_ncg(c.Cout) && wino_onepass_checked()) a.wwop = a.ww + conv_wino_wwop_at(c.Cin, c.Cout);
       ProfScope ps(s, PK_CONV);
       e = launch_conv_wino(a, nb, s);
     } break;
@@ -463,7 +467,7 @@
   }
 }
 const char* misonet_last_error(void) { return g_err; }
-int misonet_version(void) { return 660; }
+int misonet_version(void) { return 670; }
 
 int misonet_net_create(const misonet_cfg* cfg, misonet_net** out) {
   if (!cfg || !out) return fail(MISONET_EINVAL, "null argument");
@@ -531,9 +535,9 @@
   bool ok = hipMalloc(reinterpret_cast<void**>(&dx), x.size() * 4) == hipSuccess && hipMalloc(reinterpret_cast<void**>(&dwd), wd.size() * 4) == hipSuccess &&
             hipMalloc(reinterpret_cast<void**>(&dww), ww.size() * 4) == hipSuccess &&
             hipMalloc(reinterpret_cast<void**>(&db), 128 * 4) == hipSuccess &&
-            hipMalloc(reinterpret_cast<void**>(&dy), 2 * out_n * 4) == hipSuccess && hipMalloc(reinterpret_cast<void**>(&dst), 2 * st_n * 8) == hipSuccess;
-  std::vector<float> y(2 * out_n);
-  std::vector<dstat_t> sv(2 * st_n);
+            hipMalloc(reinterpret_cast<void**>(&dy), 3 * out_n * 4) == hipSuccess && hipMalloc(reinterpret_cast<void**>(&dst), 3 * st_n * 8) == hipSuccess;
+  std::vector<float> y(3 * out_n);
+  std::vector<dstat_t> sv(3 * st_n);
   if (ok) {
     std::vector<float> b128(128, 0.f);
     std::copy(bias.begin(), bias.end(), b128.begin());
@@ -541,7 +545,7 @@
          hipMemcpy(dwd, wd.data(), wd.size() * 4, hipMemcpyHostToDevice) == hipSuccess &&
          hipMemcpy(dww, ww.data(), ww.size() * 4, hipMemcpyHostToDevice) == hipSuccess &&
          hipMemcpy(db, b128.data(), 128 * 4, hipMemcpyHostToDevice) == hipSuccess &&
-         hipMemset(dy, 0, 2 * out_n * 4) == hipSuccess && hipMemset(dst, 0, 2 * st_n * 8) == hipSuccess;
+         hipMemset(dy, 0, 3 * out_n * 4) == hipSuccess && hipMemset(dst, 0, 3 * st_n * 8) == hipSuccess;
   }
   if (ok) {
     ConvArgs a = {};
@@ -554,30 +558,43 @@
     a.wscale = a.descale = 1.f;
     a.out = dy; a.out_stats = dst;
     ok = launch_conv_wino(a, N, nullptr) == hipSuccess;
-    a.ww = nullptr; a.ww16 = nullptr; a.out = dy + out_n; a.out_stats = dst + st_n;
+    a.wwop = dww + conv_wino_wwop_at(Cin, Cout); a.out = dy + 2 * out_n; a.out_stats = dst + 2 * st_n;
+    ok = ok && launch_conv_wino(a, N, nullptr) == hipSuccess;
+    a.ww = nullptr; a.ww16 = nullptr; a.wwop = nullptr; a.out = dy + out_n; a.out_stats = dst + st_n;
     ok = ok && launch_conv(a, N, nullptr) == hipSuccess && hipDeviceSynchronize() == hipSuccess &&
-         hipMemcpy(y.data(), dy, 2 * out_n * 4, hipMemcpyDeviceToHost) == hipSuccess &&
-         hipMemcpy(sv.data(), dst, 2 * st_n * 8, hipMemcpyDeviceToHost) == hipSuccess;
+         hipMemcpy(y.data(), dy, 3 * out_n * 4, hipMemcpyDeviceToHost) == hipSuccess &&
+         hipMemcpy(sv.data(), dst, 3 * st_n * 8, hipMemcpyDeviceToHost) == hipSuccess;
   }
   release();
+  bool ok_op = ok;
   if (ok) {
+    auto same = [&](int which, double& worst, double& scale) {
+      worst = 0.0; scale = 0.0;
+      for (int nn = 0; nn < N; ++nn)
+        for (int c = 0; c < Cout; ++c)
+          for (int f = 0; f < F; ++f)
+            for (int t = 0; t < T; ++t) {
+              const size_t i = (((size_t)nn * Cout + c) * F + f) * Tp + t;
+              worst = std::max(worst, (double)fabsf(y[which * out_n + i] - y[out_n + i]));
+              scale = std::max(scale, (double)fabsf(y[out_n + i]));
+            }
+      bool r = std::isfinite(worst) && scale > 0.0 && worst <= 2e-5 * scale;
+      for (size_t i = 0; r && i < st_n / DS_NL; ++i) {
+        auto rd = [](const dstat_t* p) { long long L[DS_NL]; for (int k = 0; k < DS_NL; ++k) L[k] = (long long)p[k]; return dstat_combine(L); };
+        const double a1 = rd(sv.data() + which * st_n + i * DS_NL), a2 = rd(sv.data() + st_n + i * DS_NL);
+        r = std::isfinite(a1) && fabs(a1 - a2) <= 1e-4 * (fabs(a2) + 1.0);
+      }
+      return r;
+    };
     double worst = 0.0, scale = 0.0;
-    for (int nn = 0; nn < N; ++nn)
-      for (int c = 0; c < Cout; ++c)
-        for (int f = 0; f < F; ++f)
-          for (int t = 0; t < T; ++t) {
-            const size_t i = (((size_t)nn * Cout + c) * F + f) * Tp + t;
-            worst = std::max(worst, (double)fabsf(y[i] - y[out_n + i]));
-            scale = std::max(scale, (double)fabsf(y[out_n + i]));
-          }
-    ok = std::isfinite(worst) && scale > 0.0 && worst <= 2e-5 * scale;
-    for (size_t i = 0; ok && i < st_n / DS_NL; ++i) {
-      auto rd = [](const dstat_t* p) { long long L[DS_NL]; for (int k = 0; k < DS_NL; ++k) L[k] = (long long)p[k]; return dstat_combine(L); };
-      const double a1 = rd(sv.data() + i * DS_NL), a2 = rd(sv.data() + st_n + i * DS_NL);
-      ok = std::isfinite(a1) && fabs(a1 - a2) <= 1e-4 * (fabs(a2) + 1.0);
-    }
+    ok = same(0, worst, scale);
     if (!ok) fprintf(stderr, "[misonet] conv3x3_wino_f32 self-check FAILED on device %d (max |diff| %.3e of %.3e): mode f32w disabled\n", d, worst, scale);
-  }
+    ok_op = ok && same(2, worst, scale);
+    if (ok && !ok_op)
+      fprintf(stderr, "[misonet] conv3x3_wino_f32_onepass self-check FAILED on device %d (max |diff| %.3e of %.3e): 48-channel layers keep "
+                      "the two-launch dispatch\n", d, worst, scale);
+  }
+  g_wino_op_state[d].store(ok_op ? 1 : 2, std::memory_order_release);
   st = ok ? 1 : 2;
   g_wino_state[d].store(st, std::memory_order_release);
   return st;
@@ -701,6 +718,56 @@
   return k;
 }
 
+int misonet_conv_dense_layer(int path, int n_samples, int c_in, int c_out, int n_freq, int n_frames, const float* w_host,
+                             const float* bias_host, const float* x_dev, float* y_dev, unsigned long long* stats_dev, misonet_stream stream) {
+  if (!w_host || !bias_host || !x_dev || !y_dev || !stats_dev) return fail(MISONET_EINVAL, "null argument");
+  if (path < 0 || path > 2 || n_samples <= 0 || c_in <= 0 || c_out <= 0 || n_freq <= 0 || n_frames <= 0)
+    return fail(MISONET_EINVAL, "path must be 0, 1 or 2 and every size positive");
+  const int Tp = frames_pitch(n_frames);
+  ConvArgs a = {};
+  a.in = x_dev; a.in_stats = nullptr;
+  a.in_bstride = (long long)c_in * n_freq * Tp; a.out_bstride = (long long)c_out * n_freq * Tp;
+  a.in_sstride = c_in; a.out_sstride = c_out;
+  a.in_c0 = 0; a.Cin = c_in; a.Fin = n_freq; a.ident_c = c_in;
+  a.out_c0 = 0; a.Cout = c_out; a.Fout = n_freq; a.T = n_frames; a.Tp = Tp;
+  a.sf = 1; a.padf = 1; a.tr2 = 0; a.act = 1;
+  a.cop = c_out > 32 ? 64 : 32; a.ncg = (c_out + a.cop - 1) / a.cop;
+  a.wscale = a.descale = 1.f;
+  a.out = y_dev; a.out_stats = reinterpret_cast<dstat_t*>(stats_dev);
+  const bool wino = path != 0 && conv_wino_ok(conv_shape(a));
+  const ConvKind kind = wino ? ConvKind::WINO : ConvKind::DIRECT;
+  const ConvWeights cw = {w_host, c_in, c_out, false, a.cop, a.ncg};
+  std::vector<float> img((size_t)conv_image_floats(kind, cw)), b((size_t)a.ncg * a.cop + 64, 0.f);
+  conv_image_pack(kind, cw, img.data());
+  std::copy(bias_host, bias_host + c_out, b.begin());
+  hipStream_t s = reinterpret_cast<hipStream_t>(stream);
+  HIPCHK(conv_init());
+  HIPCHK(conv_wino_init());
+  if (wino && wino_selftest() != 1) return fail(MISONET_ESTATE, "the f32w kernel failed its self-check on this device (see stderr)");
+  float *dw = nullptr, *db = nullptr;
+  HIPCHK(hipMalloc(reinterpret_cast<void**>(&dw), img.size() * 4));
+  hipError_t e = hipMalloc(reinterpret_cast<void**>(&db), b.size() * 4);
+  if (e == hipSuccess) e = hipMemcpy(dw, img.data(), img.size() * 4, hipMemcpyHostToDevice);
+  if (e == hipSuccess) e = hipMemcpy(db, b.data(), b.size() * 4, hipMemcpyHostToDevice);
+  if (e == hipSuccess) e = hipMemsetAsync(stats_dev, 0, (size_t)n_samples * c_out * 2 * DS_NL * sizeof(dstat_t), s);
+  a.bias = db;
+  if (e == hipSuccess) {
+    if (wino) {
+      a.ww = dw;
+      if ((c_out & 31) == 16) a.ww16 = dw + conv_wino_ww16_at(c_in, c_out);
+      if (path == 2 && conv_wino_onepass_ncg(c_out) && wino_onepass_checked()) a.wwop = dw + conv_wino_wwop_at(c_in, c_out);
+      e = launch_conv_wino(a, n_samples, s);
+    } else {
+      a.w = dw;
+      e = launch_conv(a, n_samples, s);
+    }
+  }
+  if (e == hipSuccess) e = hipStreamSynchronize(s);
+  (void)hipFree(dw); (void)hipFree(db);
+  HIPCHK(e);
+  return wino ? (a.wwop ? 2 : 1) : 0;
+}
+
 int misonet_net_keep_activations(misonet_net* n, int keep) {
   if (!n) return fail(MISONET_EINVAL, "null argument");
   n->keep_taps = keep != 0;
```
